# HoangGiang93/mujoco_sim

Hardware: AMD Instinct MI355X
Metric: env-steps/sec (whole node) at 4096 envs, 24-DoF/30-contact scene; 1/2/4/8 GPUs (higher is better)
Workload: dtype f32

## Files before the change

mujoco_sim_amd/csrc/dev_convex.h:

```cpp
#pragma once
#include "dev_math.h"

#define MPR_TOL 1e-6f
#define MPR_ITER 50
#define MPR_EPS_LEN2 1e-10f
#define MPR_EPS_VOL 1e-7f

struct CvxGeom { int type; float pos[3], mat[9], size[3], pad; const float* vert; int nvert; };
struct MprPt { float v[3], s[3]; };

DEV void mpr_tri_normal(float* n, const MprPt& p1, const MprPt& p2, const MprPt& p3) {
  const float e1[3] = {p2.v[0]-p1.v[0], p2.v[1]-p1.v[1], p2.v[2]-p1.v[2]}, e2[3] = {p3.v[0]-p1.v[0], p3.v[1]-p1.v[1], p3.v[2]-p1.v[2]};
  cross3(n, e1, e2); normalize3(n);
}
DEV bool mpr_converged(const MprPt& p1, const MprPt& p2, const MprPt& p3, const MprPt& p4, const float* n) {
  const float d4 = dot3(p4.v, n);
  const float m = fminf(d4 - dot3(p1.v, n), fminf(d4 - dot3(p2.v, n), d4 - dot3(p3.v, n)));
  return m <= MPR_TOL;
}
DEV void mpr_take(MprPt& q, const MprPt& p, bool take) {
#pragma unroll
  for (int k = 0; k < 3; k++) { q.v[k] = take ? p.v[k] : q.v[k]; q.s[k] = take ? p.s[k] : q.s[k]; }
}
DEV void mpr_expand(const MprPt& p0, MprPt& p1, MprPt& p2, MprPt& p3, const MprPt& p4) {
  float c[3];
  cross3(c, p4.v, p0.v);
  const bool a = dot3(p1.v, c) > 0, b = dot3(p2.v, c) > 0, d = dot3(p3.v, c) > 0;
  const bool r1 = a ? b : !d, r2 = !a && d, r3 = a && !b;
  mpr_take(p1, p4, r1); mpr_take(p2, p4, r2); mpr_take(p3, p4, r3);
}
DEV void tri_closest_to_origin(const float* a, const float* b, const float* c, float* out) {
  const float ab[3] = {b[0]-a[0], b[1]-a[1], b[2]-a[2]}, ac[3] = {c[0]-a[0], c[1]-a[1], c[2]-a[2]};
  const float d1 = -dot3(ab, a), d2 = -dot3(ac, a);
  if (d1 <= 0 && d2 <= 0) { out[0] = a[0]; out[1] = a[1]; out[2] = a[2]; return; }
  const float d3 = -dot3(ab, b), d4 = -dot3(ac, b);
  if (d3 >= 0 && d4 <= d3) { out[0] = b[0]; out[1] = b[1]; out[2] = b[2]; return; }
  const float vc = d1*d4 - d3*d2;
  if (vc <= 0 && d1 >= 0 && d3 <= 0) { const float t = d1 / (d1 - d3); out[0] = a[0] + t*ab[0]; out[1] = a[1] + t*ab[1]; out[2] = a[2] + t*ab[2]; return; }
  const float d5 = -dot3(ab, c), d6 = -dot3(ac, c);
  if (d6 >= 0 && d5 <= d6) { out[0] = c[0]; out[1] = c[1]; out[2] = c[2]; return; }
  const float vb = d5*d2 - d1*d6;
  if (vb <= 0 && d2 >= 0 && d6 <= 0) { const float t = d2 / (d2 - d6); out[0] = a[0] + t*ac[0]; out[1] = a[1] + t*ac[1]; out[2] = a[2] + t*ac[2]; return; }
  const float va = d3*d6 - d5*d4;
  if (va <= 0 && (d4 - d3) >= 0 && (d5 - d6) >= 0) {
    const float t = (d4 - d3) / ((d4 - d3) + (d5 - d6));
    out[0] = b[0] + t*(c[0]-b[0]); out[1] = b[1] + t*(c[1]-b[1]); out[2] = b[2] + t*(c[2]-b[2]); return;
  }
  const float den = 1.0f / (va + vb + vc), v = vb * den, w = vc * den;
  out[0] = a[0] + v*ab[0] + w*ac[0]; out[1] = a[1] + v*ab[1] + w*ac[1]; out[2] = a[2] + v*ab[2] + w*ac[2];
}

DEV void cvx_support_local(const CvxGeom& g, const float* dl, float* pl) {
  const float* s = g.size;
  pl[0] = pl[1] = pl[2] = 0;
  if (g.type == MJH_GEOM_SPHERE) { pl[0] = s[0]*dl[0]; pl[1] = s[0]*dl[1]; pl[2] = s[0]*dl[2]; }
  else if (g.type == MJH_GEOM_CAPSULE) { pl[0] = s[0]*dl[0]; pl[1] = s[0]*dl[1]; pl[2] = s[0]*dl[2] + (dl[2] >= 0 ? s[1] : -s[1]); }
  else if (g.type == MJH_GEOM_CYLINDER) {
    const float r2 = dl[0]*dl[0] + dl[1]*dl[1];
    if (r2 > MPR_EPS_LEN2) { const float sc = s[0] * rsqrtf(r2); pl[0] = dl[0]*sc; pl[1] = dl[1]*sc; }
    pl[2] = dl[2] >= 0 ? s[1] : -s[1];
  } else if (g.type == MJH_GEOM_BOX) { pl[0] = dl[0] >= 0 ? s[0] : -s[0]; pl[1] = dl[1] >= 0 ? s[1] : -s[1]; pl[2] = dl[2] >= 0 ? s[2] : -s[2]; }
  else if (g.type == MJH_GEOM_ELLIPSOID) {
    const float w0 = s[0]*s[0]*dl[0], w1 = s[1]*s[1]*dl[1], w2 = s[2]*s[2]*dl[2];
    const float den = sqrtf(w0*dl[0] + w1*dl[1] + w2*dl[2]);
    if (den > MJ_MINVAL) { const float inv = 1.0f / den; pl[0] = w0*inv; pl[1] = w1*inv; pl[2] = w2*inv; }
  }
}
DEV void mesh_support_wave(const bool want, const float* vert, const int nvert, const float* dl, float* pl, const int lane) {
  unsigned long long req = __ballot(want);
  const unsigned long long va = (unsigned long long)vert;
  const int valo = (int)(unsigned)va, vahi = (int)(unsigned)(va >> 32);
  while (req) {
    constexpr int NB = 4;
    int L[NB], nv[NB]; const float* vp[NB]; float d0[NB], d1[NB], d2[NB]; bool on[NB];
#pragma unroll
    for (int u = 0; u < NB; u++) {
      on[u] = req != 0;
      L[u] = on[u] ? __ffsll((long long)req) - 1 : 0;
      if (on[u]) req &= req - 1;
      const unsigned lo = (unsigned)__builtin_amdgcn_readlane(valo, L[u]), hi = (unsigned)__builtin_amdgcn_readlane(vahi, L[u]);
      vp[u] = (const float*)(((unsigned long long)hi << 32) | lo);
      nv[u] = on[u] ? __builtin_amdgcn_readlane(nvert, L[u]) : 0;
      d0[u] = readlane_f(dl[0], L[u]); d1[u] = readlane_f(dl[1], L[u]); d2[u] = readlane_f(dl[2], L[u]);
    }
    float bx[NB], by[NB], bz[NB], bd[NB]; int bi[NB];
#pragma unroll
    for (int u = 0; u < NB; u++) {
      bd[u] = -3.0e38f; bi[u] = 0x7fffffff; bx[u] = by[u] = bz[u] = 0;
      if (on[u]) { const int i = min(lane, nv[u] - 1); bx[u] = vp[u][3*i]; by[u] = vp[u][3*i+1]; bz[u] = vp[u][3*i+2]; }
    }
#pragma unroll
    for (int u = 0; u < NB; u++) {
      if (!on[u]) continue;
      if (lane < nv[u]) { bd[u] = bx[u]*d0[u] + by[u]*d1[u] + bz[u]*d2[u]; bi[u] = lane; }
      for (int i = lane + 64; i < nv[u]; i += 64) {
        const float x = vp[u][3*i], y = vp[u][3*i+1], z = vp[u][3*i+2], dp = x*d0[u] + y*d1[u] + z*d2[u];
        if (dp > bd[u]) { bd[u] = dp; bi[u] = i; bx[u] = x; by[u] = y; bz[u] = z; }
      }
      const float gmax = wave_max_f(bd[u]);
      const bool cand = bd[u] == gmax && bi[u] != 0x7fffffff;
      unsigned long long m = __ballot(cand);
      if (__popcll(m) > 1) { const int wi = wave_min_i(cand ? bi[u] : 0x7fffffff); m = __ballot(cand && bi[u] == wi); }
      const int wl = m ? __ffsll((long long)m) - 1 : 0;
      const float wx = readlane_f(bx[u], wl), wy = readlane_f(by[u], wl), wz = readlane_f(bz[u], wl);
      if (lane == L[u]) { pl[0] = wx; pl[1] = wy; pl[2] = wz; }
    }
  }
}
struct HfPrism { float x[3], y[3], top[3], bot; };
DEV void prism_support_local(const HfPrism& h, const float* dl, float* pl) {
  const bool up = dl[2] >= 0;
  float bd = -3.0e38f;
  pl[0] = h.x[0]; pl[1] = h.y[0]; pl[2] = up ? h.top[0] : h.bot;
#pragma unroll
  for (int i = 0; i < 3; i++) {
    const float z = up ? h.top[i] : h.bot, d = h.x[i]*dl[0] + h.y[i]*dl[1] + z*dl[2];
    const bool take = d > bd;
    bd = take ? d : bd; pl[0] = take ? h.x[i] : pl[0]; pl[1] = take ? h.y[i] : pl[1]; pl[2] = take ? z : pl[2];
  }
}
DEV void mesh_support_lane(const float* vert, const int nvert, const float* dl, float* pl) {
  float bd = -3.0e38f;
  for (int i = 0; i < nvert; i++) {
    const float x = vert[3*i], y = vert[3*i+1], z = vert[3*i+2], dp = x*dl[0] + y*dl[1] + z*dl[2];
    if (dp > bd) { bd = dp; pl[0] = x; pl[1] = y; pl[2] = z; }
  }
}
template <bool PRISM = false>
DEV void mpr_support_wave(const CvxGeom& g1, const CvxGeom& g2, const float* dir, MprPt& p, const bool act, const int lane, const HfPrism* h = nullptr) {
  const float nd[3] = {-dir[0], -dir[1], -dir[2]};
  float dl1[3], dl2[3], pl1[3], pl2[3], a[3], b[3];
  rotvecT(dl1, g1.mat, dir); rotvecT(dl2, g2.mat, nd);
  if constexpr (PRISM) prism_support_local(*h, dl1, pl1); else cvx_support_local(g1, dl1, pl1);
  cvx_support_local(g2, dl2, pl2);
  if constexpr (!PRISM) mesh_support_wave(act && g1.type == MJH_GEOM_MESH, g1.vert, g1.nvert, dl1, pl1, lane);
  if constexpr (PRISM) { if (g2.type == MJH_GEOM_MESH) mesh_support_lane(g2.vert, g2.nvert, dl2, pl2); }
  else mesh_support_wave(act && g2.type == MJH_GEOM_MESH, g2.vert, g2.nvert, dl2, pl2, lane);
  rotvec(a, g1.mat, pl1); rotvec(b, g2.mat, pl2);
#pragma unroll
  for (int k = 0; k < 3; k++) {
    a[k] += g1.pos[k] + g1.pad*dir[k]; b[k] += g2.pos[k] + g2.pad*nd[k];
    p.v[k] = a[k] - b[k]; p.s[k] = a[k] + b[k];
  }
}

template <bool PRISM = false>
DEV int c_convex_wave(CvxGeom& g1, CvxGeom& g2, float margin, float* st, const bool act, const int lane, const HfPrism* h = nullptr) {
  g1.pad = g2.pad = 0.5f * margin;
  MprPt p0, p1, p2, p3, p4;
  float n[3], c[3];
#pragma unroll
  for (int k = 0; k < 3; k++) { p0.v[k] = g1.pos[k] - g2.pos[k]; p0.s[k] = g1.pos[k] + g2.pos[k]; p1.v[k] = p2.v[k] = p3.v[k] = 0; p1.s[k] = p2.s[k] = p3.s[k] = 0; }
  if (dot3(p0.v, p0.v) < MPR_EPS_LEN2) p0.v[0] += 1e-4f;
  n[0] = -p0.v[0]; n[1] = -p0.v[1]; n[2] = -p0.v[2];
  normalize3(n);
  enum { PH_FIRST, PH_SECOND, PH_DISCOVER, PH_REFINE, PH_PUSH };
  int phase = PH_FIRST, it = 0;
  bool live = act;
  int res = 0;
  while (__ballot(live) != 0) {
    mpr_support_wave<PRISM>(g1, g2, n, p4, live, lane, h);
    if (live) {
    const float d4 = dot3(p4.v, n);
    if (phase == PH_FIRST) {
      if (d4 <= 0) live = false;
      else {
      p1 = p4;
      cross3(n, p0.v, p1.v);
      if (dot3(n, n) < 1e-12f * dot3(p0.v, p0.v) * dot3(p1.v, p1.v)) {
        const float depth = norm3(p1.v);
        float dir[3] = {p1.v[0], p1.v[1], p1.v[2]}; normalize3(dir);
        const float pos[3] = {0.5f * p1.s[0], 0.5f * p1.s[1], 0.5f * p1.s[2]};
        raw_emit(st, 0, margin - depth, pos, dir);
        res = 1; live = false;
      } else {
      normalize3(n);
      phase = PH_SECOND;
      } }
    } else if (phase == PH_SECOND) {
      if (d4 <= 0) live = false;
      else {
      p2 = p4;
      const float e1[3] = {p1.v[0]-p0.v[0], p1.v[1]-p0.v[1], p1.v[2]-p0.v[2]}, e2[3] = {p2.v[0]-p0.v[0], p2.v[1]-p0.v[1], p2.v[2]-p0.v[2]};
      cross3(n, e1, e2); normalize3(n);
      const bool sw = dot3(n, p0.v) > 0;
      const MprPt t = p1;
      mpr_take(p1, p2, sw); mpr_take(p2, t, sw);
      n[0] = sw ? -n[0] : n[0]; n[1] = sw ? -n[1] : n[1]; n[2] = sw ? -n[2] : n[2];
      phase = PH_DISCOVER; it = 0;
      }
    } else if (phase == PH_DISCOVER) {
      if (d4 <= 0 || it > MPR_ITER) live = false;
      else {
      it++;
      cross3(c, p1.v, p4.v);
      const bool t2 = dot3(c, p0.v) < -MPR_EPS_VOL;
      cross3(c, p4.v, p2.v);
      const bool t1 = !t2 && dot3(c, p0.v) < -MPR_EPS_VOL;
      if (t1 || t2) {
        mpr_take(p2, p4, t2); mpr_take(p1, p4, t1);
        const float e1[3] = {p1.v[0]-p0.v[0], p1.v[1]-p0.v[1], p1.v[2]-p0.v[2]}, e2[3] = {p2.v[0]-p0.v[0], p2.v[1]-p0.v[1], p2.v[2]-p0.v[2]};
        cross3(n, e1, e2); normalize3(n);
      } else {
        p3 = p4;
        mpr_tri_normal(n, p1, p2, p3);
        phase = dot3(n, p1.v) >= -MPR_EPS_VOL ? PH_PUSH : PH_REFINE; it = 0;
      }
      }
    } else if (phase == PH_REFINE) {
      if (d4 < -MPR_EPS_VOL || mpr_converged(p1, p2, p3, p4, n) || it > MPR_ITER) live = false;
      else {
      it++;
      mpr_expand(p0, p1, p2, p3, p4);
      mpr_tri_normal(n, p1, p2, p3);
      if (dot3(n, p1.v) >= -MPR_EPS_VOL) { phase = PH_PUSH; it = 0; }
      }
    } else {
      if (mpr_converged(p1, p2, p3, p4, n) || it > MPR_ITER) { res = 2; live = false; }
      else {
      it++;
      mpr_expand(p0, p1, p2, p3, p4);
      mpr_tri_normal(n, p1, p2, p3);
      }
    }
    }
  }
  if (res != 2) return res;
  float depth, dir[3], pos[3];
  tri_closest_to_origin(p1.v, p2.v, p3.v, c);
  depth = norm3(c);
  if (depth < 1e-7f) { dir[0] = n[0]; dir[1] = n[1]; dir[2] = n[2]; } else { const float inv = 1.0f / depth; dir[0] = c[0]*inv; dir[1] = c[1]*inv; dir[2] = c[2]*inv; }
  float b0, b1, b2, b3, x[3];
  cross3(x, p1.v, p2.v); b0 = dot3(x, p3.v);
  cross3(x, p3.v, p2.v); b1 = dot3(x, p0.v);
  cross3(x, p0.v, p1.v); b2 = dot3(x, p3.v);
  cross3(x, p2.v, p1.v); b3 = dot3(x, p0.v);
  float sum = b0 + b1 + b2 + b3;
  if (sum <= 0) {
    b0 = 0;
    cross3(x, p2.v, p3.v); b1 = dot3(x, n);
    cross3(x, p3.v, p1.v); b2 = dot3(x, n);
    cross3(x, p1.v, p2.v); b3 = dot3(x, n);
    sum = b1 + b2 + b3;
  }
// ... 14 lines not shown
```

mujoco_sim_amd/csrc/dev_math.h:

```cpp
#pragma once
#include <hip/hip_runtime.h>

#define DEV __device__ __forceinline__
#define HDEV __host__ __device__ __forceinline__
#if !defined(__HIP_DEVICE_COMPILE__)
static inline float rsqrtf(float x) { return 1.0f / sqrtf(x); }
#endif
#define MJ_MINVAL 1e-15f
#define MJ_MAXVAL 1e10f

HDEV float dot3(const float* a, const float* b) { return a[0]*b[0] + a[1]*b[1] + a[2]*b[2]; }
HDEV void cross3(float* r, const float* a, const float* b) {
  float x = a[1]*b[2] - a[2]*b[1], y = a[2]*b[0] - a[0]*b[2], z = a[0]*b[1] - a[1]*b[0];
  r[0] = x; r[1] = y; r[2] = z;
}
HDEV float norm3(const float* a) { return sqrtf(dot3(a, a)); }
DEV float normalize3(float* a) {
  float n = norm3(a);
  if (n < MJ_MINVAL) { a[0] = 1; a[1] = 0; a[2] = 0; } else { float s = 1.0f / n; a[0] *= s; a[1] *= s; a[2] *= s; }
  return n;
}
DEV void normalize4(float* q) {
  const float n2 = q[0]*q[0] + q[1]*q[1] + q[2]*q[2] + q[3]*q[3];
  if (fabsf(n2 - 1.0f) <= 4.8e-7f) return;
  const float n = sqrtf(n2);
  if (n < MJ_MINVAL) { q[0] = 1; q[1] = q[2] = q[3] = 0; } else { float s = 1.0f / n; q[0] *= s; q[1] *= s; q[2] *= s; q[3] *= s; }
}
DEV void mulquat(float* r, const float* a, const float* b) {
  float w = a[0]*b[0] - a[1]*b[1] - a[2]*b[2] - a[3]*b[3];
  float x = a[0]*b[1] + a[1]*b[0] + a[2]*b[3] - a[3]*b[2];
  float y = a[0]*b[2] - a[1]*b[3] + a[2]*b[0] + a[3]*b[1];
  float z = a[0]*b[3] + a[1]*b[2] - a[2]*b[1] + a[3]*b[0];
  r[0] = w; r[1] = x; r[2] = y; r[3] = z;
}
DEV void quat2mat(float* m, const float* q) {
  float w = q[0], x = q[1], y = q[2], z = q[3];
  m[0] = w*w + x*x - y*y - z*z; m[1] = 2*(x*y - w*z);         m[2] = 2*(x*z + w*y);
  m[3] = 2*(x*y + w*z);         m[4] = w*w - x*x + y*y - z*z; m[5] = 2*(y*z - w*x);
  m[6] = 2*(x*z - w*y);         m[7] = 2*(y*z + w*x);         m[8] = w*w - x*x - y*y + z*z;
}
HDEV void rotvec(float* r, const float* m, const float* v) {
  float x = m[0]*v[0] + m[1]*v[1] + m[2]*v[2], y = m[3]*v[0] + m[4]*v[1] + m[5]*v[2], z = m[6]*v[0] + m[7]*v[1] + m[8]*v[2];
  r[0] = x; r[1] = y; r[2] = z;
}
HDEV void rotvecT(float* r, const float* m, const float* v) {
  float x = m[0]*v[0] + m[3]*v[1] + m[6]*v[2], y = m[1]*v[0] + m[4]*v[1] + m[7]*v[2], z = m[2]*v[0] + m[5]*v[1] + m[8]*v[2];
  r[0] = x; r[1] = y; r[2] = z;
}
DEV void axisangle2quat(float* q, const float* axis, float angle) {
  float s, c; __sincosf(0.5f * angle, &s, &c);
  q[0] = c; q[1] = axis[0]*s; q[2] = axis[1]*s; q[3] = axis[2]*s;
}
DEV void quat_integrate(float* q, const float* w, float h) {
  float ax[3] = {w[0], w[1], w[2]};
  float n = norm3(ax);
  if (n < MJ_MINVAL) { normalize4(q); return; }
  float inv = 1.0f / n; ax[0] *= inv; ax[1] *= inv; ax[2] *= inv;
  float dq[4], r[4];
  float s = sinf(0.5f * h * n), c = cosf(0.5f * h * n);
  dq[0] = c; dq[1] = ax[0]*s; dq[2] = ax[1]*s; dq[3] = ax[2]*s;
  normalize4(q); mulquat(r, q, dq); normalize4(r);
  q[0] = r[0]; q[1] = r[1]; q[2] = r[2]; q[3] = r[3];
}
DEV void cross_motion(float* r, const float* v, const float* x) {
  float a[3], b[3], c[3];
  cross3(a, v, x); cross3(b, v, x + 3); cross3(c, v + 3, x);
  r[0] = a[0]; r[1] = a[1]; r[2] = a[2]; r[3] = b[0] + c[0]; r[4] = b[1] + c[1]; r[5] = b[2] + c[2];
}
DEV void cross_force(float* r, const float* v, const float* f) {
  float a[3], b[3], c[3];
  cross3(a, v, f); cross3(b, v + 3, f + 3); cross3(c, v, f + 3);
  r[0] = a[0] + b[0]; r[1] = a[1] + b[1]; r[2] = a[2] + b[2]; r[3] = c[0]; r[4] = c[1]; r[5] = c[2];
}
DEV void inert_com(float* res, const float* diagI, const float* mat, const float* off, float mass) {
  float I[9];
#pragma unroll
  for (int r = 0; r < 3; r++)
#pragma unroll
    for (int c = 0; c < 3; c++) I[3*r+c] = mat[3*r]*diagI[0]*mat[3*c] + mat[3*r+1]*diagI[1]*mat[3*c+1] + mat[3*r+2]*diagI[2]*mat[3*c+2];
  float d2 = dot3(off, off);
  res[0] = I[0] + mass * (d2 - off[0]*off[0]); res[1] = I[4] + mass * (d2 - off[1]*off[1]); res[2] = I[8] + mass * (d2 - off[2]*off[2]);
  res[3] = I[1] - mass * off[0]*off[1]; res[4] = I[2] - mass * off[0]*off[2]; res[5] = I[5] - mass * off[1]*off[2];
  res[6] = mass * off[0]; res[7] = mass * off[1]; res[8] = mass * off[2]; res[9] = mass;
}
DEV void mul_inert_vec(float* res, const float* i, const float* v) {
  float r0 = i[0]*v[0] + i[3]*v[1] + i[4]*v[2] - i[8]*v[4] + i[7]*v[5];
// ... 104 lines not shown
```

mujoco_sim_amd/csrc/dev_types.h:

```cpp
#pragma once

#define MJH_INT_TABLES(X)                                                                          \
  X(body_parentid) X(body_rootid) X(body_jntadr) X(body_jntnum) X(body_dofadr) X(body_dofnum)      \
  X(body_level) X(body_subtreesize) X(body_treeid) X(body_lastdof) X(jnt_type) X(jnt_qposadr)      \
  X(jnt_dofadr) X(jnt_bodyid) X(jnt_limited) X(dof_bodyid) X(dof_jntid) X(dof_parentid)            \
  X(dof_Madr) X(dof_treeid) X(tree_dofadr) X(tree_dofnum) X(geom_type) X(geom_bodyid)              \
  X(geom_condim) X(pair_geom1) X(pair_geom2) X(pair_stageadr) X(eq_obj1id) X(eq_obj2id)            \
  X(eq_active) X(fl_dof) X(gc_body) X(controlled) X(odom)

#define MJH_FLT_TABLES(X)                                                                          \
  X(body_pos) X(body_quat) X(body_ipos) X(body_iquat) X(body_mass) X(body_inertia)                 \
  X(body_gravcomp) X(body_invweight0) X(jnt_pos) X(jnt_axis) X(jnt_stiffness) X(jnt_range)         \
  X(jnt_margin) X(jnt_solref) X(jnt_solimp) X(qpos0) X(qpos_spring) X(dof_armature)                \
  X(dof_damping) X(dof_frictionloss) X(dof_invweight0) X(dof_solref) X(dof_solimp) X(geom_pos)     \
  X(geom_quat) X(geom_size) X(geom_rbound) X(geom_friction) X(geom_solmix) X(geom_solref)          \
  X(geom_solimp) X(geom_margin) X(geom_gap) X(eq_data) X(eq_solref) X(eq_solimp)

struct DModel {
  const int* I;
  const float* F;
#define X(n) int o_##n;
  MJH_INT_TABLES(X)
  MJH_FLT_TABLES(X)
#undef X
  int nq, nv, nbody, njnt, ngeom, neq, npair, nM, ntree, maxcon, maxefc;
  int nqp, nvp;
  int maxlevel, nfl, ngc, rowW, nstage, has_damping, has_limits, diagM, maxblk, maxbrow, has_dim4, big, k1_floats, has_convex;
  int iterations, disableflags;
  float timestep, gravity[3], tolerance, impratio, meaninertia;
  int o_geom_dataid, o_mesh_vertadr, o_mesh_vertnum, o_mesh_vert;
  int noslip_iterations; float noslip_tolerance;
  double timestep_d;
  int nsite, nsensor, nmocap, has_weld;
  int group_max;
  int scratch_off;
  int o_site_bodyid, o_site_pos, o_site_quat, o_sensor_type, o_sensor_objid, o_body_mocapid, o_eq_type;
  int patch, pool, pool_floats, pdesc, pslot;
  int window, win_nvt, win_maxw, win_jsz;
  int pgs_row_order;
  int dense, dense_cap, dense_nvs;
  int dense_min_iter;
};

#ifdef MJH_COLLIDE_PROBE
#define PROF_STRIDE 24
#else
#define PROF_STRIDE 20
#endif
struct DState {
  float *qpos, *qvel, *qacc, *qacc_ws, *qvel_ref, *qfrc_applied, *ddq, *dq, *qfrc_inverse;
  double* time;
  float *initial_qpos, *odom_vel;
  int* stats;
  const int* env_order;
  unsigned* slot_mask;
  float *x_xpos, *x_xquat, *x_gpos, *x_gmat;
  float *x_bias, *x_passive, *x_smooth, *x_constraint, *x_energy;
  float *x_contacts;
  float *x_vec, *x_res;
  long long* x_prof;
  const float *p_geom_size, *p_geom_rbound, *p_body_mass, *p_body_inertia, *p_body_invweight0, *p_dof_invweight0;
  int p_stride;
  float *xfrc_applied, *mocap, *sensordata; int xfrc_stride;
  const float* pd_target; float pd_kp, pd_kd;
  float* gscratch; long long gstride;
  int win32;
  int win64;
  int probe_slices;
  float* wbuf; long long wstride; long long wj_off;
};

#define MJH_LDS_SMALL(X)                                                                           \
  X(qpos) X(qvel) X(qvref) X(ws) X(qacc) X(smooth) X(asmooth) X(passive) X(bias) X(applied)        \
  X(tmpv) X(tmpv2) X(xpos) X(xquat) X(xmat) X(xipos) X(ximat) X(com) X(cinert) X(crb) X(cvel)      \
  X(cacc) X(cfrc) X(cfrcsub) X(xanchor) X(xaxis) X(cdof) X(cdofdot) X(qM) X(qLD) X(qLDinv)          \
  X(gpos) X(gmat) X(zero) X(dofpar) X(dofMadr) X(anc) X(p_gsize) X(p_rbound) X(p_mass) X(p_inertia) X(site) X(fext)
#define MJH_LDS_POOLS(X) X(con) X(blki) X(blkf) X(blkq) X(bv) X(phi) X(sched) X(order) X(J) X(B) X(ext)
#define MJH_LDS_ARRAYS(X) MJH_LDS_SMALL(X) MJH_LDS_POOLS(X)

struct Lay {
#define X(n) int n;
  MJH_LDS_ARRAYS(X)
#undef X
  int total;
  int g_a0, g_minv, g_qvel, g_smooth, g_qacc, g_meta, g_qM;
  int g_qLD, g_anc;
  int g_dense;
};

struct DHField { int has_hfield, o_hfield_nrow, o_hfield_ncol, o_hfield_adr, o_hfield_size, o_hfield_data; };

struct DWpre { int slim, J; };

#define CREP_STRIDE 20
#define CREP_FORCE 13
#define CREP_GEOM1 17
#define CREP_GEOM2 18
#define CREP_DIM 19
struct DReport { int on, maxcon; int* ncon; float* rec; float* cfrc; };

struct DConst { DModel M; Lay L; DHField H; DWpre W; DReport R; };

enum { PH_STEP1 = 1, PH_INV = 2, PH_STEP2 = 4, PH_NOINT = 8, PH_FKONLY = 16, PH_MULM = 32, PH_RESET = 64,
       PH_PRE = 128, PH_POST = 256 };
enum { XF_BODY = 1, XF_GEOM = 2, XF_CON = 4, XF_FORCE = 8, XF_PROF = 16,
       XF_NOSTORE = 32,
       XF_DENSE = 64,
       XF_SPLIT2 = 256,
       XF_WSTRAIGHT = 512,
       XF_DEFER = 128 };

#define CON_STRIDE 16
#define CON_GEOMS 13
#define CON_MARGIN 14
#define CON_G1(c) (__float_as_int((c)[CON_GEOMS]) & 0xfff)
#define CON_G2(c) ((__float_as_int((c)[CON_GEOMS]) >> 12) & 0xfff)
#define CON_DIM(c) (__float_as_int((c)[CON_GEOMS]) >> 24)
#define BLKI_STRIDE 4
#define BLKF_STRIDE 16
#define BLKQ_STRIDE 16
#define BF_AREF 4
#define BF_F 8
#define BF_LO 14
enum { BK_SINGLE = 0, BK_PYR3 = 3, BK_PYR4 = 4 };
enum { RT_EQ = 0, RT_FL = 1, RT_LIMIT = 2, RT_CONTACT = 3, RT_WELD = 4 };
```

mujoco_sim_amd/csrc/engine.hip:

```cpp
#include <hip/hip_runtime.h>

#include <algorithm>
#include <cmath>
#include <cstddef>
#include <cstdio>
#include <cstdlib>
#include <cstring>
#include <string>
#include <vector>

#include "../../include/mjhip.h"
#include "step_kernel.h"
#include "dev_ray.h"
#include "dev_depth.h"
#include "dev_scan.h"
#include "dev_heightscan.h"
#include "dev_contact.h"
#include "dev_frame.h"
#include "dev_render.h"
#include "dev_light.h"
#include "dev_texture.h"
#include "ray_tables.h"

void mjh_set_error(const std::string& s);
hipError_t mjh_launch_window(hipStream_t st, int nvt, int grid, size_t lds, const DConst* dC, const DState& S, int env0, int n, int nl, int wxf, int n32, int n64);
hipError_t mjh_dense_attributes(size_t build_lds, size_t solve_lds);
hipError_t mjh_launch_step_hf(hipStream_t st, int nr, bool diag, int wpre, int grid, size_t lds, const DConst* dC, const DState& S,
                              int env0, int nsteps, int ph, int xflags);
hipError_t mjh_step_hf_attributes(size_t lds);
hipError_t mjh_launch_dense(hipStream_t st, int n, size_t build_lds, size_t solve_lds, const DConst* dC, const DState& S, int env0);
#define DN_CAP_MAX 256

#define HIPCHK(call)                                                                             \
  do {                                                                                           \
    hipError_t e_ = (call);                                                                      \
    if (e_ != hipSuccess) {                                                                      \
      mjh_set_error(std::string(#call) + ": " + hipGetErrorString(e_));                          \
      return MJH_ERR_NO_DEVICE;                                                                  \
    }                                                                                            \
  } while (0)

struct StateGuard {
  DState* where; DState saved;
  explicit StateGuard(DState* w) : where(w), saved(*w) {}
  ~StateGuard() { *where = saved; }
  StateGuard(const StateGuard&) = delete; StateGuard& operator=(const StateGuard&) = delete;
};
struct DevBuf {
  void* p = nullptr;
  ~DevBuf() { if (p) (void)hipFree(p); }
};

#define MJH_MAX_COHORTS 8
#define MJH_IO_SLOTS 8
#define MJH_IO_PUT_FLOATS 4096
#define MJH_IO_GET_FLOATS 16384
__attribute__((constructor)) static void mjh_library_init() { setenv("GPU_MAX_HW_QUEUES", "8", 0); }
struct mjh_engine {
  const mjh_model* model = nullptr;
  int nenv = 0, device = 0;
  hipStream_t stream = nullptr;
  DModel M{};
  DState S{};
  Lay L{};
  int lds_bytes = 0, lds_bytes_pre = 0;
  DHField H{};
  bool report = false; DReport R{};
  int2* csel_tab = nullptr; int2* csel_host = nullptr; int csel_cap = 0; hipEvent_t csel_up = nullptr; std::vector<int> csel_have; float* csel_io = nullptr; size_t csel_io_words = 0;
  DWpre W{};
  size_t dense_lds = 0, dense_solve_lds = 0;
  float* h_io = nullptr; float* d_io = nullptr; hipEvent_t io_ev[MJH_IO_SLOTS] = {}; bool io_used[MJH_IO_SLOTS] = {}; unsigned io_next = 0;
  int win_lean = -1;
  bool win_straight = true;
  int* h_wn = nullptr; int* d_wn = nullptr; int cur_cohort = -1;
  int* h_dense = nullptr; int* d_dense = nullptr; hipEvent_t ev_dense[MJH_MAX_COHORTS][4] = {}; unsigned dense_epoch[MJH_MAX_COHORTS] = {}; bool dense_now[MJH_MAX_COHORTS];
  int* dI = nullptr; float* dF = nullptr; DConst* dC = nullptr;
  std::vector<int> hI;
  int o_controlled = 0, o_odom = 0;
  std::vector<void*> allocs;
  float* scratch = nullptr; size_t scratch_floats = 0;
  float* p_tables[MJH_EP_COUNT] = {nullptr};
  int* d_order = nullptr;
  bool lpt = true;
  bool split3 = true;
  bool order_valid = false;
  struct ChainGraph { hipGraphExec_t exec = nullptr; unsigned char S[sizeof(DState)]; int g0 = -1, n = -1, key = -1; bool nocap = false; };
  int last_launches = 0;
  ChainGraph cgraph[MJH_MAX_COHORTS][8];
  int steps_per_launch = 8;
  long order_age = 0; int order_G = 0; int last_chunk = 1;
  int ncohort = 1;
  hipStream_t cstream[MJH_MAX_COHORTS] = {nullptr};
  hipEvent_t ev_fork = nullptr, ev_join[MJH_MAX_COHORTS] = {nullptr};
  bool forked = false;
  bool timing = false; int timing_stride = 1; long timing_count = 0;
  std::vector<std::pair<hipEvent_t, hipEvent_t>> tev; size_t tev_used = 0;
  bool step1_done = false;
  bool handover = false;
  bool step1_pending = false;
  float pd_kp = 0, pd_kd = 0; float* pd_target = nullptr; bool pd_on = false;
  int4* ray_ginfo = nullptr; RayHField* ray_hf = nullptr; float* ray_hfdata = nullptr; bool ray_ready = false;
  int ray_mesh_mode = 0; int4* ray_ginfo_mesh = nullptr; RayMesh* ray_mesh = nullptr; float4* ray_planes = nullptr;
  int ray_mesh_surface = 0; bool ray_tri_ready = false; std::vector<int4> ray_gi_mesh_host;
  int4* ray_ginfo_tri = nullptr; RayTriMesh* ray_trimesh = nullptr; RayNode* ray_nodes = nullptr; float4* ray_tris = nullptr;
  float* ray_io = nullptr; size_t ray_io_floats = 0;
  float4* ray_color = nullptr; float* render_io = nullptr; size_t render_io_floats = 0;
  int light_mode = 0; mjh_light_options light_opt = {1, 1, 1e-3f};
  bool lights_ready = false; int nlight = 0; LightRec lights[MJH_MAXLIGHT]; int light_on[MJH_MAXLIGHT];
  int tex_mode = 0; TexRec* tex_rec = nullptr; unsigned* tex_data = nullptr; float* tex_io = nullptr; size_t tex_io_floats = 0;
  float* scan_tab = nullptr; size_t scan_tab_floats = 0; float* scan_host = nullptr; size_t scan_host_floats = 0; hipEvent_t scan_up = nullptr;
  bool scan_have = false; int scan_w = 0, scan_h = 0; double scan_az[2] = {0, 0}, scan_el[2] = {0, 0}; bool scan_table = false; std::vector<double> scan_elev;
  int* hscan_root = nullptr;
  bool frame_ready = false; FrameModel frame_model{};
  FrameRec* frame_tab = nullptr; FrameRec* frame_host = nullptr; int frame_cap = 0; hipEvent_t frame_up = nullptr; std::vector<int> frame_have;
  float* frame_io = nullptr; size_t frame_io_floats = 0;
};

static int pad32(int n) { return ((n + 31) / 32) * 32; }

template <class T> static int dev_alloc(mjh_engine* e, T** p, size_t n, bool zero = true) {
  void* q = nullptr;
  HIPCHK(hipMalloc(&q, std::max<size_t>(n, 1) * sizeof(T)));
  if (zero) HIPCHK(hipMemsetAsync(q, 0, std::max<size_t>(n, 1) * sizeof(T), e->stream));
  e->allocs.push_back(q);
  *p = (T*)q;
  return MJH_OK;
}

static int g_chain_graph = getenv("MJH_CHAIN_GRAPH") ? atoi(getenv("MJH_CHAIN_GRAPH")) : 1;
extern "C" void mjh_set_chain_graph(int mode) { g_chain_graph = mode < 0 ? 0 : (mode > 2 ? 2 : mode); }

static int ensure_scratch(mjh_engine* e, size_t floats) {
  if (floats <= e->scratch_floats) return MJH_OK;
  if (e->scratch) { HIPCHK(hipStreamSynchronize(e->stream)); HIPCHK(hipFree(e->scratch)); }
  HIPCHK(hipMalloc((void**)&e->scratch, floats * sizeof(float)));
  e->scratch_floats = floats;
  return MJH_OK;
}

static bool extra_instance(const DModel& M) { return M.has_convex || M.noslip_iterations > 0 || M.nsensor > 0 || M.nmocap > 0 || M.has_weld; }

static int window_tier(const mjh_engine* e) {
  static const int nl_env = getenv("MJH_WN_NL") ? atoi(getenv("MJH_WN_NL")) : -1;
  const int nwreg = e->M.win_nvt == 24 ? WN_NW24 : WN_NW32;
  const int seen = (e->h_wn && e->cur_cohort >= 0) ? *(volatile int*)(e->h_wn + e->cur_cohort) : (1 << 20);
  const int nl_full = std::min(WN_MAXW, (int)((40 * 1024 - 1024) / (4 * WN_XREC(e->M.win_nvt) * 16 * sizeof(float))));
  const bool sec32 = e->S.win32 > 0 && e->M.win_nvt == 24 && e->S.win32 <= 16 * nwreg;
  const bool tier = sec32 ? seen > 32 * WN32_NW : seen + 16 > 16 * nwreg;
  if (nl_env < 0 && e->win_lean >= 0 && e->M.win_maxw <= 16) return e->win_lean ? 0 : nl_full;
// ... 5 lines not shown
  const bool window = snap || (e->M.window && e->S.wbuf && (ph & PH_STEP2) && !(ph & (PH_NOINT | PH_PRE | PH_POST)) && !(xflags & ~(XF_FORCE | XF_DEFER | (wmode == 1 ? XF_PROF : 0))));
  if (window && !snap) ph |= PH_PRE;
  if (wmode && !window) { mjh_set_error("internal: window-chain launch mode on a launch that is not one"); return MJH_ERR_STATE; }
  if (wmode == 1) xflags |= XF_DEFER;
  if (wmode != 2) {
#define MJH_LAUNCH2(NR, DG, CX) do { if (e->H.has_hfield) HIPCHK(mjh_launch_step_hf(st, NR, DG, 0, n, (size_t)e->lds_bytes, e->dC, e->S, env0, nsteps, ph, xflags)); \
                                   else hipLaunchKernelGGL((mjh_step_kernel<NR, DG, CX>), dim3(n), dim3(64), (size_t)e->lds_bytes, st, e->dC, e->S, env0, nsteps, ph, xflags); } while (0)
#define MJH_LAUNCH(NR, DG) do { if (extra_instance(e->M) || e->S.xfrc_applied || e->report) MJH_LAUNCH2(NR, DG, true); else MJH_LAUNCH2(NR, DG, false); } while (0)
  const int nr = e->M.big ? 8 : (e->M.nv <= 16 ? 1 : (e->M.nv <= 32 ? 2 : 4));
  static const bool slim = !(getenv("MJH_WINDOW_SLIM") && atoi(getenv("MJH_WINDOW_SLIM")) == 0);
  if (window && slim) {
    const bool cx = extra_instance(e->M) || e->S.xfrc_applied || e->report;
    static const bool slim_lds = !(getenv("MJH_WINDOW_SLIM_LDS") && atoi(getenv("MJH_WINDOW_SLIM_LDS")) == 0);
    static const int wpad = getenv("MJH_WPRE_LDS_PAD") ? std::max(0, atoi(getenv("MJH_WPRE_LDS_PAD"))) : 0;
    const size_t wlds = (size_t)((slim_lds && e->lds_bytes_pre > 0) ? e->lds_bytes_pre : e->lds_bytes) + (size_t)wpad;
#define MJH_LAUNCHW(NR, CX, GJ) do { if (e->H.has_hfield) HIPCHK(mjh_launch_step_hf(st, NR, true, GJ, n, wlds, e->dC, e->S, env0, nsteps, ph, xflags)); \
                                   else hipLaunchKernelGGL((mjh_step_kernel<NR, true, CX, GJ>), dim3(n), dim3(64), wlds, st, e->dC, e->S, env0, nsteps, ph, xflags); } while (0)
#define MJH_LAUNCHW2(NR, CX) do { if (e->M.patch) MJH_LAUNCHW(NR, CX, 1); else MJH_LAUNCHW(NR, CX, 2); } while (0)
    if (nr == 1) { if (cx) MJH_LAUNCHW2(1, true); else MJH_LAUNCHW2(1, false); } else { if (cx) MJH_LAUNCHW2(2, true); else MJH_LAUNCHW2(2, false); }
#undef MJH_LAUNCHW2
#undef MJH_LAUNCHW
  } else
  if (e->M.diagM) { if (nr == 1) MJH_LAUNCH(1, true); else if (nr == 2) MJH_LAUNCH(2, true); else if (nr == 4) MJH_LAUNCH(4, true); else MJH_LAUNCH(8, true); }
  else { if (nr == 1) MJH_LAUNCH(1, false); else if (nr == 2) MJH_LAUNCH(2, false); else if (nr == 4) MJH_LAUNCH(4, false); else MJH_LAUNCH(8, false); }
#undef MJH_LAUNCH2
#undef MJH_LAUNCH
  HIPCHK(hipGetLastError());
  }
  if (window && wmode != 1 && wmode != 3) {
    const int nl = tier_nl >= 0 ? tier_nl : window_tier(e);
    const size_t lds = (size_t)4 * nl * WN_XREC(e->M.win_nvt) * 16 * sizeof(float);
    const int n32 = (e->S.win32 && e->M.win_nvt == 24) ? (n + 1) / 2 : 0;
    const int wxf = (xflags & ~XF_DEFER) | ((ph & PH_STEP1) ? 0 : XF_SPLIT2) | (e->win_straight ? XF_WSTRAIGHT : 0);
    const int n64 = (e->S.win64 && e->M.win_nvt == 24 && e->S.win64 < 16 * e->M.win_maxw) ? n : 0;
    HIPCHK(mjh_launch_window(st, e->M.win_nvt, n64 + (e->M.win_nvt == 24 ? n32 : 0) + (n + 3) / 4, lds, e->dC, e->S, env0, n, nl, wxf, n32, n64));
  }
  return MJH_OK;
}

static int launch(mjh_engine* e, int env0, int n, int nsteps, int ph, int xflags, int wmode = 0) { return launch_on(e, e->stream, env0, n, nsteps, ph, xflags, wmode); }

static int fork_cohorts(mjh_engine* e) {
  if (e->forked || e->ncohort <= 1) return MJH_OK;
  HIPCHK(hipEventRecord(e->ev_fork, e->stream));
  for (int g = 0; g < e->ncohort; g++) HIPCHK(hipStreamWaitEvent(e->cstream[g], e->ev_fork, 0));
  e->forked = true;
  return MJH_OK;
}
static int join_cohorts(mjh_engine* e) {
  if (!e->forked) return MJH_OK;
  for (int g = 0; g < e->ncohort; g++) {
    HIPCHK(hipEventRecord(e->ev_join[g], e->cstream[g]));
    HIPCHK(hipStreamWaitEvent(e->stream, e->ev_join[g], 0));
  }
  e->forked = false;
  return MJH_OK;
}
static int set_cohorts(mjh_engine* e, int n) {
  n = std::max(1, std::min(n, MJH_MAX_COHORTS));
  int rc = join_cohorts(e);
  if (rc) return rc;
  if (n > 1) {
    if (!e->ev_fork) HIPCHK(hipEventCreateWithFlags(&e->ev_fork, hipEventDisableTiming));
    for (int g = 0; g < n; g++) {
      if (!e->cstream[g]) HIPCHK(hipStreamCreateWithFlags(&e->cstream[g], hipStreamNonBlocking));
      if (!e->ev_join[g]) HIPCHK(hipEventCreateWithFlags(&e->ev_join[g], hipEventDisableTiming));
    }
  }
  e->ncohort = n;
  return MJH_OK;
}

static int pair_cap(int t1, int t2) {
  if (t1 > t2) std::swap(t1, t2);
  if (t1 == MJH_GEOM_PLANE && t2 == MJH_GEOM_BOX) return 4;
  if (t1 == MJH_GEOM_PLANE && t2 == MJH_GEOM_CAPSULE) return 2;
  if (t1 == MJH_GEOM_PLANE && t2 == MJH_GEOM_CYLINDER) return 4;
  if (t1 == MJH_GEOM_PLANE && t2 == MJH_GEOM_MESH) return 4;
  if (t1 == MJH_GEOM_BOX && t2 == MJH_GEOM_BOX) return 8;
  if (t1 == MJH_GEOM_HFIELD) return MJH_HFIELD_MAXCON;
  return 1;
}

struct HostPack { DModel M{}; Lay L{}; DHField H{}; DWpre W{}; bool report = false; std::vector<int> I; std::vector<float> F; int o_controlled = 0, o_odom = 0, lds_bytes = 0, lds_bytes_pre = 0, lds_bytes_wpre = 0; long long gstride = 0; };
#define MJH_WINDOW_MAXCON 128
static int g_window_solver = getenv("MJH_WINDOW") ? (atoi(getenv("MJH_WINDOW")) != 0) : 1;
extern "C" void mjh_set_window_solver(int on) { g_window_solver = on ? 1 : 0; }
static int g_pgs_row_order = 1;
static int g_contact_report = getenv("MJH_CONTACT_REPORT") ? (atoi(getenv("MJH_CONTACT_REPORT")) != 0) : 0;
extern "C" void mjh_set_contact_report(int on) { g_contact_report = on ? 1 : 0; }
extern "C" void mjh_set_pgs_row_order(int mode) { g_pgs_row_order = mode < 0 || mode > 2 ? 1 : mode; }
static void derive_device_model(const mjh_model* m, HostPack& hp, bool force_big = false, bool allow_patch = true) {
  DModel& M = hp.M; std::vector<int>& I = hp.I; std::vector<float>& F = hp.F;
  const bool report = g_contact_report != 0;
  hp.report = report;
  const int nb = m->nbody, nv = m->nv, nj = m->njnt, ng = m->ngeom;
  std::vector<int> subtreesize(nb, 1), lastdof(nb, -1), stageadr(m->npair, 0), fl_dof, gc_body, controlled(std::max(nv, 1), 0), odom(10, -1);
  odom[9] = 0;
  for (int b = nb - 1; b > 0; b--) subtreesize[m->body_parentid[b]] += subtreesize[b];
  for (int b = 1; b < nb; b++) lastdof[b] = m->body_dofnum[b] ? m->body_dofadr[b] + m->body_dofnum[b] - 1 : lastdof[m->body_parentid[b]];
  int nstage = 0, maxlevel = 0, rowW = 1;
  for (int b = 0; b < nb; b++) maxlevel = std::max(maxlevel, m->body_level[b]);
  auto treenum = [&](int b) { int t = m->body_treeid[b]; return t >= 0 ? m->tree_dofnum[t] : 0; };
  for (int i = 0; i < m->npair; i++) {
    int g1 = m->pair_geom1[i], g2 = m->pair_geom2[i];
    stageadr[i] = nstage; nstage += pair_cap(m->geom_type[g1], m->geom_type[g2]);
    int b1 = m->geom_bodyid[g1], b2 = m->geom_bodyid[g2];
    int w = treenum(b1) + ((m->body_treeid[b1] != m->body_treeid[b2]) ? treenum(b2) : 0);
    rowW = std::max(rowW, w);
  }
  for (int t = 0; t < m->ntree; t++) rowW = std::max(rowW, m->tree_dofnum[t]);
  int neqrow = 0; bool has_weld = false;
  for (int q = 0; q < m->neq; q++) {
    if (m->eq_type[q] != MJH_EQ_JOINT) {
      has_weld = true; neqrow += m->eq_type[q] == MJH_EQ_WELD ? 6 : 3;
      rowW = std::max(rowW, treenum(m->eq_obj1id[q]) + ((m->body_treeid[m->eq_obj1id[q]] != m->body_treeid[m->eq_obj2id[q]]) ? treenum(m->eq_obj2id[q]) : 0));
      continue;
    }
    neqrow++;
    int j1 = m->eq_obj1id[q], j2 = m->eq_obj2id[q];
    int t1 = m->dof_treeid[m->jnt_dofadr[j1]], w = m->tree_dofnum[t1];
    if (j2 >= 0) { int t2 = m->dof_treeid[m->jnt_dofadr[j2]]; if (t2 != t1) w += m->tree_dofnum[t2]; }
    rowW = std::max(rowW, w);
  }
  rowW = ((rowW + 3) / 4) * 4;
  bool diagM = m->ntree > 0 && m->neq == 0 && m->nsensor == 0 && m->nmocap == 0 && !report;
  for (int t = 0; t < m->ntree && diagM; t++) {
    const int b = m->tree_bodyid[t];
    diagM = m->tree_dofnum[t] == 6 && m->body_jntnum[b] == 1 && m->jnt_type[m->body_jntadr[b]] == MJH_JNT_FREE && subtreesize[b] == 1 &&
            m->body_ipos[3*b] == 0 && m->body_ipos[3*b+1] == 0 && m->body_ipos[3*b+2] == 0 && m->body_iquat[4*b] == 1;
  }
  bool has_damping = false, has_limits = false;
  for (int d = 0; d < nv; d++) { if (m->dof_frictionloss[d] > 0) { fl_dof.push_back(d); diagM = false; } if (m->dof_damping[d] > 0) has_damping = true; }
  for (int j = 0; j < nj; j++) if (m->jnt_limited[j]) has_limits = true;
  for (int b = 1; b < nb; b++) if (m->body_gravcomp[b] != 0) gc_body.push_back(b);

  auto addI = [&](const int* p, size_t n) { int o = (int)I.size(); I.insert(I.end(), p, p + n); while (I.size() % 4) I.push_back(0); return o; };
  auto addF = [&](const double* p, size_t n) { int o = (int)F.size(); for (size_t i = 0; i < n; i++) F.push_back((float)p[i]); while (F.size() % 4) F.push_back(0); return o; };
#define PI(name, n) M.o_##name = addI(m->name, (size_t)(n))
#define PF(name, n) M.o_##name = addF(m->name, (size_t)(n))
  PI(body_parentid, nb); PI(body_rootid, nb); PI(body_jntadr, nb); PI(body_jntnum, nb); PI(body_dofadr, nb); PI(body_dofnum, nb);
  PI(body_level, nb); M.o_body_subtreesize = addI(subtreesize.data(), nb); PI(body_treeid, nb); M.o_body_lastdof = addI(lastdof.data(), nb);
  PI(jnt_type, nj); PI(jnt_qposadr, nj); PI(jnt_dofadr, nj); PI(jnt_bodyid, nj); PI(jnt_limited, nj);
  PI(dof_bodyid, nv); PI(dof_jntid, nv); PI(dof_parentid, nv); PI(dof_Madr, nv); PI(dof_treeid, nv);
  PI(tree_dofadr, m->ntree); PI(tree_dofnum, m->ntree);
  PI(geom_type, ng); PI(geom_bodyid, ng); PI(geom_condim, ng);
  PI(pair_geom1, m->npair); PI(pair_geom2, m->npair); M.o_pair_stageadr = addI(stageadr.data(), m->npair);
  PI(eq_obj1id, m->neq); PI(eq_obj2id, m->neq); PI(eq_active, m->neq);
  M.o_fl_dof = addI(fl_dof.data(), fl_dof.size()); M.o_gc_body = addI(gc_body.data(), gc_body.size());
  M.o_controlled = hp.o_controlled = addI(controlled.data(), controlled.size());
  M.o_odom = hp.o_odom = addI(odom.data(), odom.size());
  PF(body_pos, 3*nb); PF(body_quat, 4*nb); PF(body_ipos, 3*nb); PF(body_iquat, 4*nb); PF(body_mass, nb); PF(body_inertia, 3*nb);
  PF(body_gravcomp, nb); PF(body_invweight0, 2*nb);
  PF(jnt_pos, 3*nj); PF(jnt_axis, 3*nj); PF(jnt_stiffness, nj); PF(jnt_range, 2*nj); PF(jnt_margin, nj); PF(jnt_solref, 2*nj); PF(jnt_solimp, 5*nj);
  PF(qpos0, m->nq); PF(qpos_spring, m->nq);
  PF(dof_armature, nv); PF(dof_damping, nv); PF(dof_frictionloss, nv); PF(dof_invweight0, nv); PF(dof_solref, 2*nv); PF(dof_solimp, 5*nv);
  PF(geom_pos, 3*ng); PF(geom_quat, 4*ng); PF(geom_size, 3*ng); PF(geom_rbound, ng); PF(geom_friction, 3*ng); PF(geom_solmix, ng);
  PF(geom_solref, 2*ng); PF(geom_solimp, 5*ng); PF(geom_margin, ng); PF(geom_gap, ng);
  PF(eq_data, 11*m->neq); PF(eq_solref, 2*m->neq); PF(eq_solimp, 5*m->neq);
  PI(geom_dataid, ng); PI(mesh_vertadr, m->nmesh); PI(mesh_vertnum, m->nmesh); PF(mesh_vert, 3 * (size_t)m->nmeshvert);
  PI(eq_type, m->neq);
  if (m->nsite > 0) { PI(site_bodyid, m->nsite); PF(site_pos, 3 * (size_t)m->nsite); PF(site_quat, 4 * (size_t)m->nsite); }
  if (m->nsensor > 0) { PI(sensor_type, m->nsensor); PI(sensor_objid, m->nsensor); }
  {
    std::vector<int> mocapid(nb, -1);
    if (m->body_mocapid) for (int b = 0; b < nb; b++) mocapid[b] = m->body_mocapid[b];
    M.o_body_mocapid = addI(mocapid.data(), nb);
  }
  M.nsite = m->nsite; M.nsensor = m->nsensor; M.nmocap = m->nmocap; M.has_weld = has_weld ? 1 : 0;
  {
    DHField& H = hp.H;
    H.has_hfield = 0;
    for (int i = 0; i < m->npair; i++) if (m->geom_type[m->pair_geom1[i]] == MJH_GEOM_HFIELD) H.has_hfield = 1;
    if (H.has_hfield) {
      H.o_hfield_nrow = addI(m->hfield_nrow, m->nhfield); H.o_hfield_ncol = addI(m->hfield_ncol, m->nhfield); H.o_hfield_adr = addI(m->hfield_adr, m->nhfield);
      H.o_hfield_size = addF(m->hfield_size, 4 * (size_t)m->nhfield); H.o_hfield_data = addF(m->hfield_data, (size_t)m->nhfielddata);
    }
  }
  M.group_max = m->ntree <= 64 ? 16 : 4;
  for (int t = 0; t < m->ntree; t++) if (m->tree_dofnum[t] > 8) M.group_max = 4;
#undef PI
#undef PF
  M.nq = m->nq; M.nv = nv; M.nbody = nb; M.njnt = nj; M.ngeom = ng; M.neq = m->neq; M.npair = m->npair; M.nM = m->nM; M.ntree = m->ntree;
  M.maxcon = std::max(m->maxcon, 1); M.maxefc = std::max(m->maxefc, 1);
  M.nqp = M.nvp = pad32(m->nq + 4 * std::max(nv, 1));
  M.maxlevel = maxlevel; M.nfl = (int)fl_dof.size(); M.ngc = (int)gc_body.size(); M.rowW = rowW; M.nstage = nstage;
  M.has_damping = has_damping; M.has_limits = has_limits; M.diagM = diagM;
  M.has_dim4 = 0;
  for (int g = 0; g < ng; g++) if (m->geom_condim[g] == 4) M.has_dim4 = 1;
  M.has_convex = 0;
  for (int i = 0; i < m->npair; i++) {
    const int t1 = m->geom_type[m->pair_geom1[i]], t2 = m->geom_type[m->pair_geom2[i]];
    if (t2 == MJH_GEOM_MESH) M.has_convex = 1;
    if (t1 != MJH_GEOM_PLANE && (t1 == MJH_GEOM_ELLIPSOID || t2 == MJH_GEOM_ELLIPSOID || t1 == MJH_GEOM_CYLINDER || t2 == MJH_GEOM_CYLINDER ||
                                 t2 == MJH_GEOM_MESH || (t1 == MJH_GEOM_CAPSULE && t2 == MJH_GEOM_BOX))) M.has_convex = 1;
  }
  {
    int nlim = 0; for (int j = 0; j < nj; j++) if (m->jnt_limited[j]) nlim += (m->jnt_range[2*j+1] - m->jnt_range[2*j] <= 2 * m->jnt_margin[j]) ? 2 : 1;
    const int nfix = neqrow + (int)fl_dof.size() + nlim;
    M.maxblk = nfix + M.maxcon; M.maxbrow = nfix + 4 * M.maxcon;
  }
  M.iterations = m->opt.iterations; M.disableflags = m->opt.disableflags;
  M.timestep = (float)m->opt.timestep; M.timestep_d = m->opt.timestep; for (int k = 0; k < 3; k++) M.gravity[k] = (float)m->opt.gravity[k];
  M.tolerance = (float)m->opt.tolerance; M.impratio = (float)m->opt.impratio; M.meaninertia = (float)m->meaninertia;
  M.noslip_iterations = m->opt.noslip_iterations; M.noslip_tolerance = (float)m->opt.noslip_tolerance;
  {
    Lay& L = hp.L; int off = 0; long long goff = 0;
    auto put = [&](int n) { int o = off; off += ((std::max(n, 1) + 3) / 4) * 4; return o; };
    const bool big = force_big || nv > 64;
    M.big = big;
    const bool keep = m->nsensor > 0 || report;
    auto gput = [&](long long n) { long long o = goff; goff += ((std::max<long long>(n, 1) + 3) / 4) * 4; return (int)(-1 - o); };
    const int nblkcap = std::max(M.maxblk, 1);
    long long jsz = std::max<long long>((long long)(M.maxblk - M.maxcon) * rowW + (long long)M.maxcon * rowW * 4, 4);
    const long long need = (long long)nstage * RAW_STRIDE;
    if ((diagM ? 1 : 2) * jsz < need) jsz = diagM ? need : (need + 1) / 2;
    M.pgs_row_order = g_pgs_row_order;
    if (!M.pgs_row_order && nv > 32) for (int t = 0; t < m->ntree; t++) if (m->tree_dofnum[t] > 16) M.pgs_row_order = 1;
    const bool small_free = allow_patch && diagM && !big && nv <= 32 && M.noslip_iterations == 0 && !keep;
    const bool patch = small_free && M.maxcon <= 64;
    M.patch = patch ? 1 : 0;
    M.window = (small_free && M.maxcon <= MJH_WINDOW_MAXCON && M.pgs_row_order != 0 && g_window_solver && nv <= 32 && m->njnt <= 16 && m->nq <= 40) ? 1 : 0;
    M.win_nvt = nv <= 24 ? 24 : 32;
    M.win_maxw = std::max(1, std::min(WN_MAXW, (M.maxefc + 15) / 16));
    if (const char* v = getenv("MJH_WINDOW_MAXW")) M.win_maxw = std::max(1, std::min(M.win_maxw, atoi(v)));
    L.qpos = put(m->nq);
    L.qvel = put(nv); L.qvref = put(nv); L.ws = put(nv); L.qacc = put(nv); L.smooth = put(nv); L.asmooth = put(nv); L.passive = put(nv);
    L.bias = put(nv); L.applied = put(nv); L.tmpv = put(nv); L.tmpv2 = put(nv);
    if (patch) {
      L.qM = put(m->nM); L.qLD = L.qM; L.qLDinv = put(nv); L.dofpar = 0; L.dofMadr = 0; L.anc = 0;
      L.p_gsize = put(3*ng); L.p_rbound = put(ng); L.p_mass = put(nb); L.p_inertia = put(3*nb);
      L.zero = put(PP_ZERO);
    }
    const int k1 = off;
    const int unused = diagM ? put(4) : 0;
    L.xpos = put(3*nb); L.xquat = put(4*nb); L.xmat = put(9*nb); L.ximat = put(9*nb); L.crb = diagM ? unused : put(10*nb);
    L.xanchor = put(3*nj); L.xaxis = put(3*nj); L.gpos = put(3*ng); L.gmat = put(9*ng);
    const int k1_size = off - k1;
    M.k1_floats = k1_size;
    M.scratch_off = (big && keep) ? put(k1_size) : k1;
    L.xipos = put(3*nb); L.com = put(3*nb); L.cinert = diagM ? unused : put(10*nb); L.cdof = diagM ? unused : put(6*nv);
    const int k2_size = off - k1;
    if (!patch) {
      L.qM = put(m->nM); L.qLD = (diagM || big) ? L.qM : put(m->nM); L.qLDinv = put(nv);
      if (diagM) { L.dofpar = 0; L.dofMadr = 0; L.anc = 0; }
      else { L.dofpar = put(nv); L.dofMadr = put(nv); L.anc = put(m->nM); }
      const bool nopairs = m->npair == 0;
      L.p_gsize = nopairs ? L.gpos : put(3*ng); L.p_rbound = nopairs ? L.gmat : put(ng); L.p_mass = put(nb); L.p_inertia = put(3*nb);
    }
    {
      const int a4 = [](int n) { return ((std::max(n, 1) + 3) / 4) * 4; }(6*nb);
      const int velsz = diagM ? 4 : 4 * a4 + ((6*nv + 3) / 4) * 4;
      int vel;
      if (big) { L.con = gput((long long)M.maxcon * CON_STRIDE); L.blkq = gput((long long)nblkcap * BLKQ_STRIDE); vel = (!keep && !diagM && velsz <= k1_size) ? k1 : put(velsz); }
      else if (keep) { L.con = put(M.maxcon * CON_STRIDE); L.blkq = put(nblkcap * BLKQ_STRIDE); vel = put(velsz); }
      else {
        L.con = put(std::max(std::max(M.maxcon * CON_STRIDE, velsz), nblkcap * BLKQ_STRIDE));
        L.blkq = L.con; vel = L.con;
      }
      if (diagM) { L.cvel = unused; L.cacc = unused; L.cfrc = unused; L.cfrcsub = unused; L.cdofdot = unused; }
      else { L.cvel = vel; L.cacc = vel + a4; L.cfrc = vel + 2*a4; L.cfrcsub = vel + 3*a4; L.cdofdot = vel + 4*a4; }
// ... 42 lines not shown
      L.g_a0 = graw(nv); L.g_minv = graw(nv); L.g_qvel = graw(nv); L.g_smooth = graw(nv); L.g_qacc = graw(nv); L.g_meta = graw(8); L.g_qM = graw(m->nM);
      const bool dense_on = !(getenv("MJH_DENSE") && atoi(getenv("MJH_DENSE")) == 0);
      M.dense = (dense_on && !diagM && M.noslip_iterations == 0 && nv <= 128 && nv >= 1) ? 1 : 0;
      M.dense_cap = std::min(256, ((std::max(M.maxefc, 1) + 63) / 64) * 64); M.dense_nvs = ((nv + 15) / 16) * 16;
      if (const char* dc = getenv("MJH_DENSE_CAP")) M.dense_cap = std::max(64, std::min(M.dense_cap, (atoi(dc) / 64) * 64));
      M.dense_min_iter = getenv("MJH_DENSE_MIN_ITER") ? std::max(0, atoi(getenv("MJH_DENSE_MIN_ITER"))) : 32;
      L.g_dense = 0; L.g_qLD = 0; L.g_anc = 0;
      if (M.dense) { L.g_qLD = graw(m->nM); L.g_anc = graw(m->nM); }
      if (M.dense) { long long o = goff; goff += (long long)M.dense_cap * M.dense_cap + (long long)M.dense_cap * M.dense_nvs + 6LL * M.dense_cap; L.g_dense = (int)o; }
    }
    hp.gstride = goff;
    if (const char* pad = getenv("MJH_LDS_PAD")) off += std::max(0, atoi(pad));
    L.total = off;
    hp.lds_bytes = off * (int)sizeof(float);
  }
}

#define MJH_LDS_RESIDENT_MAX (24 * 1024)
#define MJH_ORDER_EVERY 32
static int order_every_of(const mjh_engine* e);
static int g_layout_policy = 0;
extern "C" void mjh_set_layout_policy(int policy) { g_layout_policy = policy < 0 || policy > 2 ? 0 : policy; }
static int order_every_of(const mjh_engine* e) {
  static const int env = getenv("MJH_ORDER_EVERY") ? std::max(1, atoi(getenv("MJH_ORDER_EVERY"))) : 0;
  return env ? env : ((e->M.window && e->M.win_maxw > 16) ? 16 : MJH_ORDER_EVERY);
}
static void derive_fitting(const mjh_model* m, HostPack& hp) {
  derive_device_model(m, hp);
  int policy = g_layout_policy;
  if (const char* fb = getenv("MJH_FORCE_BIG")) policy = atoi(fb) ? 2 : 1;
  const int limit = policy == 1 ? 160 * 1024 : (policy == 2 ? 0 : MJH_LDS_RESIDENT_MAX);
  if ((hp.M.patch || hp.M.window) && policy == 0 && hp.lds_bytes <= 64 * 1024) return;
  if (hp.M.patch && hp.lds_bytes > 64 * 1024 && hp.lds_bytes <= limit) { HostPack np; derive_device_model(m, np, false, false); hp = np; }
  if ((hp.lds_bytes > 160 * 1024 || hp.lds_bytes > limit) && !hp.M.big && hp.M.rowW <= 64) { HostPack big; derive_device_model(m, big, true); hp = big; }
}

extern "C" int mjh_query_lds_bytes(const mjh_model* m) {
  if (!m) return MJH_ERR_ARG;
  HostPack hp; derive_fitting(m, hp);
  return hp.lds_bytes;
}
extern "C" int mjh_debug_lds_layout(const mjh_model* m, char* out, int cap) {
  if (!m || !out || cap <= 0) return MJH_ERR_ARG;
  HostPack hp; derive_fitting(m, hp);
  std::string t;
#define X(n) t += std::string(#n) + " " + std::to_string(hp.L.n) + "\n";
  MJH_LDS_ARRAYS(X)
#undef X
  t += "total " + std::to_string(hp.L.total) + "\nlds_bytes " + std::to_string(hp.lds_bytes) + "\nlds_bytes_pre " + std::to_string(hp.lds_bytes_pre) +
       "\nk1_floats " + std::to_string(hp.M.k1_floats) + "\nmaxcon " + std::to_string(hp.M.maxcon) + "\nmaxblk " + std::to_string(hp.M.maxblk) +
       "\nrowW " + std::to_string(hp.M.rowW) + "\nnstage " + std::to_string(hp.M.nstage) + "\nbig " + std::to_string((int)hp.M.big) +
       "\nlds_bytes_wpre " + std::to_string(hp.M.window ? hp.lds_bytes_wpre : 0) + "\n";
  const int n = std::min((int)t.size(), cap - 1);
  std::memcpy(out, t.data(), (size_t)n); out[n] = 0;
  return n;
}
extern "C" int mjh_query_lds_bytes_assemble(const mjh_model* m) {
  if (!m) return MJH_ERR_ARG;
  HostPack hp; derive_fitting(m, hp);
  return hp.M.window ? hp.lds_bytes_pre : 0;
}

extern "C" int mjh_create(const mjh_model* m, int nenv, int device, void* stream, mjh_engine** out) {
  if (!m || nenv <= 0 || !out) { mjh_set_error("mjh_create: bad argument"); return MJH_ERR_ARG; }
  int ndev = 0;
  if (hipGetDeviceCount(&ndev) != hipSuccess || ndev <= 0) {
    mjh_set_error("mjh_create: no HIP device visible (this engine has no CPU fallback)");
    return MJH_ERR_NO_DEVICE;
  }
  if (device < 0 || device >= ndev) { mjh_set_error("mjh_create: bad device index"); return MJH_ERR_ARG; }

  if (m->ngeom > 4095) { mjh_set_error("mjh_create: more than 4095 geoms (contact records pack the geom ids in 12 bits)"); return MJH_ERR_CAPACITY; }
  for (int g = 0; g < m->ngeom; g++) if (m->geom_condim[g] != 1 && m->geom_condim[g] != 3 && m->geom_condim[g] != 4) {
    mjh_set_error("mjh_create: condim must be 1, 3 or 4 (rolling friction, condim 6, is not implemented)"); return MJH_ERR_UNSUPPORTED; }
  HIPCHK(hipSetDevice(device));
  mjh_engine* e = new mjh_engine();
#undef HIPCHK
#define HIPCHK(call) do { hipError_t e_ = (call); if (e_ != hipSuccess) { mjh_set_error(std::string(#call) + ": " + hipGetErrorString(e_)); mjh_destroy(e); return MJH_ERR_NO_DEVICE; } } while (0)
  if (const char* v = getenv("MJH_LPT")) e->lpt = atoi(v) != 0;
  if (const char* v = getenv("MJH_SPLIT3")) e->split3 = atoi(v) != 0;
  e->model = m; e->nenv = nenv; e->device = device; e->stream = (hipStream_t)stream;

  HostPack hp; derive_fitting(m, hp);
  e->M = hp.M; e->L = hp.L; e->H = hp.H; e->W = hp.W; e->report = hp.report; e->lds_bytes = hp.lds_bytes; e->lds_bytes_pre = hp.lds_bytes_wpre; e->o_controlled = hp.o_controlled; e->o_odom = hp.o_odom;
  DModel& M = e->M; std::vector<int>& I = hp.I; std::vector<float>& F = hp.F;
  e->hI = I;
  if (dev_alloc(e, &e->dI, I.size(), false) || dev_alloc(e, &e->dF, F.size(), false)) { mjh_destroy(e); return MJH_ERR_NO_DEVICE; }
  HIPCHK(hipMemcpyAsync(e->dI, I.data(), I.size() * sizeof(int), hipMemcpyHostToDevice, e->stream));
  HIPCHK(hipMemcpyAsync(e->dF, F.data(), F.size() * sizeof(float), hipMemcpyHostToDevice, e->stream));
  HIPCHK(hipStreamSynchronize(e->stream));
  M.I = e->dI; M.F = e->dF;

  if (e->report) {
    DReport& R = e->R;
    R.on = 1; R.maxcon = e->M.maxcon; e->split3 = false;
    if (dev_alloc(e, &R.ncon, (size_t)nenv) || dev_alloc(e, &R.rec, (size_t)nenv * R.maxcon * CREP_STRIDE) || dev_alloc(e, &R.cfrc, (size_t)nenv * 6 * e->M.nbody)) { mjh_destroy(e); return MJH_ERR_NO_DEVICE; }
  }
  {
    DConst hc; hc.M = e->M; hc.L = e->L; hc.H = e->H; hc.W = e->W; hc.R = e->R;
    if (dev_alloc(e, &e->dC, 1, false)) { mjh_destroy(e); return MJH_ERR_NO_DEVICE; }
    HIPCHK(hipMemcpyAsync(e->dC, &hc, sizeof hc, hipMemcpyHostToDevice, e->stream));
    HIPCHK(hipStreamSynchronize(e->stream));
  }
  if ((long long)(e->M.maxblk - e->M.maxcon) * e->M.rowW + (long long)e->M.maxcon * e->M.rowW * 4 >= 4LL * 65536) {
    mjh_set_error("mjh_create: Jacobian pool too large for the 16-bit block offsets (lower the contact capacity)");
    mjh_destroy(e); return MJH_ERR_CAPACITY;
  }
  if (e->M.big && e->M.rowW > 64) {
    mjh_set_error("mjh_create: nv > 64 needs every constraint to touch at most 64 dofs (this model: " + std::to_string(e->M.rowW) + "); the solver maps one dof of a block per lane");
    mjh_destroy(e); return MJH_ERR_CAPACITY;
  }
  if (e->lds_bytes > 160 * 1024) {
    mjh_set_error("mjh_create: per-env working set exceeds the 160 KiB LDS of one CU (" + std::to_string(e->lds_bytes) + " B)");
    mjh_destroy(e); return MJH_ERR_CAPACITY;
  }
#define MJH_ATTR(NR, DG) do { HIPCHK(hipFuncSetAttribute((const void*)mjh_step_kernel<NR, DG, false>, hipFuncAttributeMaxDynamicSharedMemorySize, e->lds_bytes)); \
                              HIPCHK(hipFuncSetAttribute((const void*)mjh_step_kernel<NR, DG, true>, hipFuncAttributeMaxDynamicSharedMemorySize, e->lds_bytes)); } while (0)
  if (e->M.dense) {
    e->dense_lds = ((size_t)e->M.dense_nvs + 5 * (size_t)e->M.dense_cap + (size_t)std::max(e->M.maxblk, 1) + 8) * sizeof(float);
    e->dense_solve_lds = (DN_CAP_MAX + 128 + 2 * (size_t)e->M.nM) * sizeof(float);
    if (e->dense_lds > 160 * 1024 || e->dense_solve_lds > 160 * 1024) { e->M.dense = 0; }
    else {
      HIPCHK(mjh_dense_attributes(e->dense_lds, e->dense_solve_lds));
    }
  }
  MJH_ATTR(1, true); MJH_ATTR(2, true); MJH_ATTR(4, true); MJH_ATTR(8, true); MJH_ATTR(1, false); MJH_ATTR(2, false); MJH_ATTR(4, false); MJH_ATTR(8, false);
#undef MJH_ATTR
  if (e->H.has_hfield) HIPCHK(mjh_step_hf_attributes((size_t)e->lds_bytes));
  if (e->M.window) {
#define MJH_ATTRW(NR, CX, GJ) HIPCHK(hipFuncSetAttribute((const void*)mjh_step_kernel<NR, true, CX, GJ>, hipFuncAttributeMaxDynamicSharedMemorySize, e->lds_bytes))
    MJH_ATTRW(1, false, 1); MJH_ATTRW(1, true, 1); MJH_ATTRW(2, false, 1); MJH_ATTRW(2, true, 1);
    MJH_ATTRW(1, false, 2); MJH_ATTRW(1, true, 2); MJH_ATTRW(2, false, 2); MJH_ATTRW(2, true, 2);
#undef MJH_ATTRW
  }

  DState& S = e->S;
  const size_t nq_all = (size_t)nenv * M.nqp, nv_all = (size_t)nenv * M.nvp;
  int rc = 0;
  rc |= dev_alloc(e, &S.qpos, nq_all); rc |= dev_alloc(e, &S.initial_qpos, nq_all);
  {
    const int nvc = std::max(M.nv, 1);
    S.qvel = S.qpos + M.nq; S.qacc_ws = S.qvel + nvc; S.ddq = S.qacc_ws + nvc; S.dq = S.ddq + nvc;
  }
  S.qacc = S.qacc_ws;
  rc |= dev_alloc(e, &S.qvel_ref, nv_all); rc |= dev_alloc(e, &S.qfrc_applied, nv_all);
  rc |= dev_alloc(e, &S.qfrc_inverse, nv_all);
  S.gscratch = nullptr; S.gstride = hp.gstride;
  if (M.big) rc |= dev_alloc(e, &S.gscratch, (size_t)nenv * (size_t)hp.gstride, false);
  S.wbuf = nullptr; S.wstride = 0;
  S.win32 = getenv("MJH_WINDOW32") ? std::max(0, atoi(getenv("MJH_WINDOW32"))) : (M.win_maxw > 16 ? 0 : WN32_MIN_ROWS);
  S.win64 = getenv("MJH_WINDOW64") ? std::max(0, atoi(getenv("MJH_WINDOW64"))) : (M.win_maxw > 16 ? WN64_MIN_ROWS : WN32_MIN_ROWS);
  if (S.win64 > 0 && S.win64 < S.win32) S.win64 = S.win32;
  if (getenv("MJH_WN_NL") && atoi(getenv("MJH_WN_NL")) < 3) S.win64 = 0;
  if (M.window) {
    S.wj_off = ((WN_ROWS + M.win_maxw * WN_NK * 16 + M.win_maxw * WN_XREC(M.win_nvt) * 16 + (M.win_maxw / 2 + 1) * WN_XPAIR * 16 + 63) / 64) * 64;
    S.wstride = S.wj_off + ((M.win_jsz + 63) / 64) * 64;
    if (((S.wstride / 64) & 1) == 0) S.wstride += 64;
    rc |= dev_alloc(e, &S.wbuf, (size_t)nenv * (size_t)S.wstride, true);
  }
  if (const char* v = getenv("MJH_WINDOW_LEAN")) e->win_lean = atoi(v) != 0;
  if (const char* v = getenv("MJH_WINDOW_STRAIGHT")) e->win_straight = atoi(v) != 0;
  if (M.window && e->lpt && nenv >= 1024) {
    HIPCHK(hipHostMalloc((void**)&e->h_wn, MJH_MAX_COHORTS * sizeof(int), hipHostMallocMapped));
    for (int g = 0; g < MJH_MAX_COHORTS; g++) e->h_wn[g] = 1 << 20;
    HIPCHK(hipHostGetDevicePointer((void**)&e->d_wn, e->h_wn, 0));
  }
  if (M.big && M.dense && e->lpt && nenv >= 1024) {
    HIPCHK(hipHostMalloc((void**)&e->h_dense, MJH_MAX_COHORTS * 4 * sizeof(int), hipHostMallocMapped));
    for (int g = 0; g < MJH_MAX_COHORTS * 4; g++) e->h_dense[g] = 1;
    for (int g = 0; g < MJH_MAX_COHORTS; g++) e->dense_now[g] = true;
    HIPCHK(hipHostGetDevicePointer((void**)&e->d_dense, e->h_dense, 0));
    for (int g = 0; g < MJH_MAX_COHORTS; g++) for (int k = 0; k < 4; k++) HIPCHK(hipEventCreateWithFlags(&e->ev_dense[g][k], hipEventDisableTiming));
  }
  rc |= dev_alloc(e, &S.time, (size_t)nenv); rc |= dev_alloc(e, &S.odom_vel, (size_t)nenv * 6); rc |= dev_alloc(e, &S.stats, (size_t)nenv * 4);
  rc |= dev_alloc(e, &S.x_bias, nv_all); rc |= dev_alloc(e, &S.x_passive, nv_all); rc |= dev_alloc(e, &S.x_smooth, nv_all);
  rc |= dev_alloc(e, &S.x_constraint, nv_all); rc |= dev_alloc(e, &S.x_energy, (size_t)nenv * 2);
  if (M.nsensor > 0) { rc |= dev_alloc(e, &S.sensordata, (size_t)nenv * 3 * M.nsensor); e->split3 = false; }
  if (M.nmocap > 0) rc |= dev_alloc(e, &S.mocap, (size_t)nenv * 7 * M.nmocap, false);
  if (rc) { mjh_destroy(e); return MJH_ERR_NO_DEVICE; }
  if (M.nmocap > 0) {
    std::vector<float> mp((size_t)nenv * 7 * M.nmocap);
    for (int b = 0; b < m->nbody; b++) if (m->body_mocapid && m->body_mocapid[b] >= 0)
// ... 1857 lines not shown
```

mujoco_sim_amd/csrc/step_kernel.h:

```cpp
#pragma once
#include "dev_collide.h"
#include "dev_convex.h"
#include "dev_types.h"

#define WSYNC() __syncthreads()
#define PROF(k) do { if ((xflags & XF_PROF) && lane == 0) S.x_prof[(size_t)blockIdx.x * PROF_STRIDE + (k)] = (long long)__builtin_amdgcn_s_memtime(); \
                     if (((xflags >> 8) & 15) == (k) && (k) > 0) return; } while (0)
#ifdef MJH_ASM_PROBE
#define ASM_PROBE_BEGIN() const long long asm_probe_t0 = (long long)__builtin_amdgcn_s_memrealtime()
#define ASM_PROBE_STORE() do { if (WPRE != 0 && lane == 0) { \
    const int hw = (int)__builtin_amdgcn_s_getreg(63492), xcc = (int)__builtin_amdgcn_s_getreg(63508) & 7; \
    const long long dt = (long long)__builtin_amdgcn_s_memrealtime() - asm_probe_t0; \
    S.stats[4*env] = (int)(asm_probe_t0 & 0x7fffffff); \
    S.stats[4*env+2] = ((hw >> 4) & 3) | (((hw >> 8) & 0xff) << 2) | (xcc << 10) | ((int)(dt < 0 ? 0 : (dt > 0x3ffff ? 0x3ffff : dt)) << 13); } } while (0)
#else
#define ASM_PROBE_BEGIN() do {} while (0)
#define ASM_PROBE_STORE() do {} while (0)
#endif
#ifdef MJH_COLLIDE_PROBE
#define CPROF(k) do { if ((xflags & XF_PROF) && lane == 0) S.x_prof[(size_t)blockIdx.x * PROF_STRIDE + 20 + (k)] = (long long)__builtin_amdgcn_s_memtime(); } while (0)
#else
#define CPROF(k) do {} while (0)
#endif
#define MINIMP 0.0001f
#define MAXIMP 0.9999f

DEV float get_impedance(const float* si, float pos, float margin) {
  float s0 = fminf(MAXIMP, fmaxf(MINIMP, si[0])), s1 = fminf(MAXIMP, fmaxf(MINIMP, si[1]));
  float s2 = fmaxf(0.0f, si[2]), s3 = fminf(MAXIMP, fmaxf(MINIMP, si[3])), s4 = fmaxf(1.0f, si[4]);
  if (s0 == s1 || s2 <= MJ_MINVAL) return 0.5f * (s0 + s1);
  float x = fabsf((pos - margin) / s2);
  if (x >= 1) return s1;
  if (x <= 0) return s0;
  float y;
  if (s4 == 1) y = x;
  else if (x <= s3) y = powf(x, s4) / powf(s3, s4 - 1);
  else y = 1 - powf(1 - x, s4) / powf(1 - s3, s4 - 1);
  return s0 + y * (s1 - s0);
}

template <class T> struct Tab {
  const T* base; int off;
  DEV T operator[](int i) const { return base[off + i]; }
  DEV const T* operator+(int k) const { return base + off + k; }
};
template <bool LAZY, class T, int DModel::*OFF> struct XTab {
  const DModel* m; const T* base; int off;
  DEV explicit XTab(const DModel& M) : m(&M), base(nullptr), off(0) { if constexpr (!LAZY) { base = tb(); off = M.*OFF; } }
  DEV const T* tb() const { if constexpr (T(1.5) == T(1)) return (const T*)m->I; else return (const T*)m->F; }
#ifdef MJH_TAB_PROBE_L2
  DEV T operator[](int i) const { if constexpr (LAZY) return *(volatile const T*)(tb() + (m->*OFF + i)); else return base[off + i]; }
#else
  DEV T operator[](int i) const { if constexpr (LAZY) return tb()[m->*OFF + i]; else return base[off + i]; }
#endif
  DEV const T* operator+(int k) const { if constexpr (LAZY) return tb() + (m->*OFF + k); else return base + off + k; }
};

template <bool LAZY, int Lay::*OFF> struct XArr {
  float* p; const Lay* l; float* b;
  DEV XArr(float* lds, const Lay& L) : p(nullptr), l(&L), b(lds) { if constexpr (!LAZY) p = lds + L.*OFF; }
  DEV float* get() const { if constexpr (LAZY) return b + l->*OFF; else return p; }
  DEV operator float*() const { return get(); }
  template <class U> DEV explicit operator U*() const { return (U*)get(); }
};

DEV void solve_tree(float* x, const float* qLD, const float* qLDinv, const int* dof_parentid, const int* dof_Madr, int adr, int num, const int STRIDE = 1) {
  for (int k = adr + num - 1; k >= adr; k--) {
    float xk = x[k * STRIDE];
    if (xk == 0) continue;
    int a = dof_Madr[k] + 1;
    for (int i = dof_parentid[k]; i >= 0; i = dof_parentid[i]) x[i * STRIDE] -= qLD[a++] * xk;
  }
  for (int k = adr; k < adr + num; k++) x[k * STRIDE] *= qLDinv[k];
  for (int k = adr; k < adr + num; k++) {
    int a = dof_Madr[k] + 1; float xk = x[k * STRIDE];
    for (int i = dof_parentid[k]; i >= 0; i = dof_parentid[i]) xk -= qLD[a++] * x[i * STRIDE];
    x[k * STRIDE] = xk;
  }
}
DEV void solve_tree_lt(float* x, const float* qLD, const int* dof_parentid, const int* dof_Madr, int adr, int num, const int STRIDE = 1) {
  for (int k = adr + num - 1; k >= adr; k--) {
    float xk = x[k * STRIDE];
    if (xk == 0) continue;
    int a = dof_Madr[k] + 1;
    for (int i = dof_parentid[k]; i >= 0; i = dof_parentid[i]) x[i * STRIDE] -= qLD[a++] * xk;
  }
}
DEV void factor_tree(float* qLD, float* qLDinv, const int* dof_parentid, const int* dof_Madr, int adr, int num) {
  for (int k = adr + num - 1; k >= adr; k--) {
    int Mkk_a = dof_Madr[k], Mki = Mkk_a + 1;
    float Mkk = qLD[Mkk_a];
    float inv = 1.0f / Mkk;
    for (int i = dof_parentid[k]; i >= 0; i = dof_parentid[i]) {
      float tmp = qLD[Mki] * inv;
      int cnt = 0, ai = dof_Madr[i];
      for (int j = i; j >= 0; j = dof_parentid[j]) { qLD[ai + cnt] -= tmp * qLD[Mki + cnt]; cnt++; }
      qLD[Mki] = tmp;
      Mki++;
    }
    qLDinv[k] = inv;
  }
}

#define MJH_WAVE_TREE_MIN 12
#define ANC_DOF(w) ((w) & 0xffff)
#define ANC_MADR(w) ((int)((unsigned)(w) >> 16))
template <int NP, int NQ>
DEV void factor_dof_pairs(float* qLD, float* qLDinv, const int* anc, const int Mk, const int d, const int k, const int lane) {
  const int q = 1 + (lane & 15), pr = lane >> 4;
  const float dk = qLD[Mk];
  float aq[NQ], ap[NP], tg[NP][NQ]; int am[NP];
#pragma unroll
  for (int c = 0; c < NQ; c++) aq[c] = qLD[Mk + min(q + 16 * c, d)];
#pragma unroll
  for (int it = 0; it < NP; it++) { const int pp = min(1 + 4 * it + pr, d); ap[it] = qLD[Mk + pp]; am[it] = ANC_MADR(anc[Mk + pp]); }
  const float inv = 1.0f / dk;
#pragma unroll
  for (int it = 0; it < NP; it++)
#pragma unroll
    for (int c = 0; c < NQ; c++) {
      tg[it][c] = 0.0f;
      if (16 * c + 16 > 4 * it) {
        const int pp = 1 + 4 * it + pr, qq = q + 16 * c; const bool v = pp <= d && qq >= pp && qq <= d;
        tg[it][c] = qLD[v ? am[it] + (qq - pp) : Mk];
      }
    }
#pragma unroll
  for (int it = 0; it < NP; it++)
#pragma unroll
    for (int c = 0; c < NQ; c++)
      if (16 * c + 16 > 4 * it) {
        const int pp = 1 + 4 * it + pr, qq = q + 16 * c; const bool v = pp <= d && qq >= pp && qq <= d;
        if (v) qLD[am[it] + (qq - pp)] = tg[it][c] - ap[it] * inv * aq[c];
      }
#pragma unroll
  for (int c = 0; c < NQ; c++) if (pr == 0 && q + 16 * c <= d) qLD[Mk + q + 16 * c] = aq[c] * inv;
  if (lane == 0) qLDinv[k] = inv;
}
// ... 638 lines not shown
      while (true) {
        o2 = nextFetch(); processQ(o0, impl); stepDone(); if (done) break;
        o0 = nextFetch(); processQ(o1, impl); stepDone(); if (done) break;
        o1 = nextFetch(); processQ(o2, impl); stepDone(); if (done) break;
      }
    } else {
      QOp o0 = nextFetch(), o1;
      while (true) {
        o1 = nextFetch(); processQ(o0, impl); stepDone(); if (done) break;
        o0 = nextFetch(); processQ(o1, impl); stepDone(); if (done) break;
      }
    }
  } else
  if (c.nblk < 3) {
    for (int it = 0; it < itmax; it++) {
      float improvement = 0;
      for (int k = 0; k < c.nblk; k++) { MOp op = fetch8(blockAt(k)); process8(op, improvement); if (!solo) __syncthreads(); }
      niter = it + 1;
      if (improvement * c.scale < tol) break;
    }
  } else {
    MOp opA = fetch8(blockAt(0)), opB;
    for (int it = 0; it < itmax; it++) {
      float improvement = 0;
      for (int k = 0; k < c.nblk; k += 2) {
        opB = fetch8(blockAt(k + 1 < c.nblk ? k + 1 : 0));
        process8(opA, improvement);
        if (k + 1 < c.nblk) {
          opA = fetch8(blockAt(k + 2 < c.nblk ? k + 2 : 0));
          process8(opB, improvement);
        } else opA = opB;
      }
      niter = it + 1;
      if (improvement * c.scale < tol) break;
    }
  }
  }
  return niter + nmain;
}

DEV void contact_frame_force(const int hd0, const float* f, const float mu1, const float mu3, float cf[4]) {
  float ph[4] = {0, 0, 0, 0};
  const int kind = hd0 & 15, nr = (hd0 >> 4) & 15;
  for (int r = 0; r < nr; r++) {
    const float fr = f[r];
    ph[0] += fr;
    if (kind != BK_SINGLE) { const int kk = 1 + (r >> 1); ph[kk] += (r & 1) ? -fr : fr; }
  }
  cf[0] = ph[0]; cf[1] = mu1 * ph[1]; cf[2] = mu1 * ph[2]; cf[3] = mu3 * ph[3];
}

#include "patch_pgs.h"
#include "window_pgs.h"

template <int NROW, bool DIAGM, bool EXTRA, int WPRE = 0, bool HF = false>
#ifndef MJH_STEP_WAVES
#define MJH_STEP_WAVES ((!DIAGM && NROW <= 4) ? 3 : 2)
#endif
#ifndef MJH_WPRE_WAVES
#define MJH_WPRE_WAVES 2
#endif
#define MJH_STEP_WAVES_T (WPRE ? MJH_WPRE_WAVES : MJH_STEP_WAVES)
__global__ __launch_bounds__(64, MJH_STEP_WAVES_T) void mjh_step_kernel(const DConst* __restrict__ C, const DState S_arg, int env0, int nsteps, int ph, int xflags) {
#ifndef MJH_LAZY_STATE
#define MJH_LAZY_STATE true
#endif
  static_assert(alignof(DState) <= alignof(const DConst*), "the descriptor follows the first argument in the kernel-argument segment without padding");
  const DState& S = MJH_LAZY_STATE ? *(const DState*)((const char*)__builtin_amdgcn_kernarg_segment_ptr() + sizeof(const DConst*)) : S_arg;
  ASM_PROBE_BEGIN();
#ifdef MJH_WPRE_PRIO
  if constexpr (WPRE != 0) __builtin_amdgcn_s_setprio(MJH_WPRE_PRIO);
#endif
  const DModel& M = C->M;
  const Lay& L = C->L;
  extern __shared__ float lds[];
  const int lane = threadIdx.x;
  const int env = S.env_order ? S.env_order[env0 + blockIdx.x] : env0 + (int)blockIdx.x;
  const int xrow = env - env0;
  const int nq = M.nq, nv = M.nv, nbody = M.nbody, njnt = M.njnt, ngeom = M.ngeom;

#ifndef MJH_LAZY_TABLES
#define MJH_LAZY_TABLES (WPRE != 0 || (!DIAGM && NROW <= 4 && EXTRA))
#endif
#define IT(n) const XTab<MJH_LAZY_TABLES, int, &DModel::o_##n> n(M);
  MJH_INT_TABLES(IT)
#undef IT
#define FT(n) const XTab<MJH_LAZY_TABLES, float, &DModel::o_##n> n(M);
  MJH_FLT_TABLES(FT)
#undef FT
  float* const gs = NROW == 8 ? S.gscratch + (size_t)env * (size_t)S.gstride : nullptr;
#ifndef MJH_LAZY_LDS
#define MJH_LAZY_LDS (WPRE != 0)
#endif
#ifndef MJH_COLLIDE_LANES
#define MJH_COLLIDE_LANES 1
#endif
  constexpr bool COLLIDE_LANES = MJH_COLLIDE_LANES != 0 && WPRE != 0;
  constexpr bool REPORT = EXTRA && !DIAGM && WPRE == 0;
#define LA(n) const XArr<MJH_LAZY_LDS, &Lay::n> s_##n(lds, L);
  MJH_LDS_SMALL(LA)
#undef LA
#define LA(n) float* s_##n = NROW == 8 ? gs + (-1 - L.n) : lds + L.n;
  MJH_LDS_POOLS(LA)
#undef LA
  int* s_blki_i = (int*)s_blki; int* s_sched_i = (int*)s_sched; int* s_order_i = (int*)s_order; 
  const int* s_dofpar_i = DIAGM ? (dof_parentid + 0) : (const int*)s_dofpar; const int* s_dofMadr_i = DIAGM ? (dof_Madr + 0) : (const int*)s_dofMadr;
  int* s_anc_i = (int*)s_anc;
  const bool level_solves = !DIAGM && nv <= 128;
  const bool short_rows = level_solves && M.ntree <= 4;
  const float* qM_ro = (NROW == 8 && !DIAGM) ? gs + L.g_qM : s_qM;
  if constexpr (WPRE == 2) { s_J = S.wbuf + (size_t)env * (size_t)S.wstride + S.wj_off; s_B = s_J; }
  if constexpr (WPRE == 2) if (8 * max(M.maxblk, 1) <= M.maxcon * CON_STRIDE) { s_bv = s_con; s_phi = s_con + 4 * max(M.maxblk, 1); }
  if constexpr (WPRE == 1) if (C->W.slim) { s_bv = s_con; s_phi = s_con + 4 * max(M.maxblk, 1); s_J = lds + C->W.J; s_B = s_J; }
  float* s_stage = s_J;
  const int rowW = M.rowW;

  const size_t qrow = (size_t)env * M.nqp, vrow = (size_t)env * M.nvp;
  const float h = M.timestep;
  const float grav[3] = {(M.disableflags & MJH_DSBL_GRAVITY) ? 0.0f : M.gravity[0], (M.disableflags & MJH_DSBL_GRAVITY) ? 0.0f : M.gravity[1],
                         (M.disableflags & MJH_DSBL_GRAVITY) ? 0.0f : M.gravity[2]};

  if (ph & PH_RESET) {
    for (int i = lane; i < nq; i += 64) S.qpos[qrow + i] = S.initial_qpos[qrow + i];
    for (int i = lane; i < nv; i += 64) { S.qvel[vrow+i] = 0; S.qacc_ws[vrow+i] = 0; S.qvel_ref[vrow+i] = 0; S.qfrc_applied[vrow+i] = 0; S.ddq[vrow+i] = 0; S.dq[vrow+i] = 0; }
    if (lane == 0) { S.time[env] = 0; S.stats[4*env] = 0; S.stats[4*env+1] = 0; S.stats[4*env+2] = 0; S.stats[4*env+3] = 0; }
    if constexpr (REPORT) if (C->R.on) {
      const DReport& R = C->R;
      float* const rec = R.rec + (size_t)env * (size_t)R.maxcon * CREP_STRIDE;
      for (int i = lane; i < R.maxcon * CREP_STRIDE; i += 64) rec[i] = 0;
      for (int i = lane; i < 6 * nbody; i += 64) R.cfrc[(size_t)env * (size_t)(6 * nbody) + i] = 0;
      if (lane == 0) R.ncon[env] = 0;
    }
    return;
  }
  for (int i = lane; i < nq; i += 64) s_qpos[i] = S.qpos[qrow + i];
  for (int i = lane; i < nv; i += 64) {
    s_qvel[i] = S.qvel[vrow + i]; s_ws[i] = S.qacc_ws[vrow + i];
    s_qacc[i] = ((ph & PH_INV) || !(ph & PH_STEP2)) ? S.qacc[vrow + i] : 0.0f;
    if (!(ph & PH_STEP1)) { s_qvref[i] = S.qvel_ref[vrow + i]; s_applied[i] = S.qfrc_applied[vrow + i]; }
  }
  if (lane < (M.patch ? PP_ZERO : 4)) s_zero[lane] = 0;
  if (!DIAGM) {
    for (int i = lane; i < nv; i += 64) { ((int*)s_dofpar)[i] = dof_parentid[i]; ((int*)s_dofMadr)[i] = dof_Madr[i]; }
    WSYNC();
    for (int i = lane; i < nv; i += 64) {
      int a = s_dofMadr_i[i]; s_anc_i[a] = i | (a << 16);
      for (int j = s_dofpar_i[i]; j >= 0; j = s_dofpar_i[j]) s_anc_i[++a] = j | (s_dofMadr_i[j] << 16);
    }
  }
  for (int i = lane; i < 3 * ngeom; i += 64) s_p_gsize[i] = S.p_geom_size ? S.p_geom_size[(size_t)env * S.p_stride + i] : geom_size[i];
  for (int i = lane; i < ngeom; i += 64) s_p_rbound[i] = S.p_geom_rbound ? S.p_geom_rbound[(size_t)env * S.p_stride + i] : geom_rbound[i];
  for (int i = lane; i < nbody; i += 64) s_p_mass[i] = S.p_body_mass ? S.p_body_mass[(size_t)env * S.p_stride + i] : body_mass[i];
  for (int i = lane; i < 3 * nbody; i += 64) s_p_inertia[i] = S.p_body_inertia ? S.p_body_inertia[(size_t)env * S.p_stride + i] : body_inertia[i];
  const bool pre = NROW == 8 && (ph & PH_PRE), post = NROW == 8 && (ph & PH_POST);
  bool wpre = false;
  if constexpr (DIAGM && NROW <= 2) wpre = M.window != 0 && (ph & PH_PRE) && S.wbuf != nullptr;
  if (wpre && lane == 0) { int* wh0 = (int*)(S.wbuf + (size_t)env * (size_t)S.wstride); wh0[0] = 0; wh0[4] = 0; wh0[5] = 0; }
  if (post) for (int i = lane; i < nv; i += 64) s_qvel[i] = gs[L.g_qvel + i];
  double time = S.time[env];
  const unsigned slotmask = S.slot_mask ? (unsigned)__builtin_amdgcn_readfirstlane((int)S.slot_mask[env]) : 0u;
  const int sbase = nbody > 32 ? nbody - 32 : 0;
  int flags = 0, ncon = 0, nefc = 0, niter = 0, cost_hint = 0;
  PROF(0);
  if ((xflags & XF_PROF) && lane == 0) {
    S.x_prof[(size_t)blockIdx.x * PROF_STRIDE + 16] = (long long)__builtin_amdgcn_s_memrealtime();
    S.x_prof[(size_t)blockIdx.x * PROF_STRIDE + 19] = env;
    S.x_prof[(size_t)blockIdx.x * PROF_STRIDE + 18] = (long long)__builtin_amdgcn_s_getreg(63492) | ((long long)__builtin_amdgcn_s_getreg(63508) << 32);
  }
  WSYNC();
  PROF(1);

  constexpr bool LOOP = !DIAGM && NROW <= 4;
  int step = 0;
step_again:
  {
    int lane_it = (int)threadIdx.x;
    if constexpr (LOOP) asm volatile("" : "+v"(lane_it));
    const int lane = lane_it;
    cost_hint = 0;
    {
      bool badv = false;
      for (int i = lane; i < nq; i += 64) { float x = s_qpos[i]; badv |= !(x == x) || fabsf(x) > MJ_MAXVAL; }
      for (int i = lane; i < nv; i += 64) { float x = s_qvel[i], y = s_qacc[i]; badv |= !(x == x) || fabsf(x) > MJ_MAXVAL || !(y == y) || fabsf(y) > MJ_MAXVAL; }
      if (wave_any(badv)) {
        for (int i = lane; i < nq; i += 64) s_qpos[i] = S.initial_qpos[qrow + i];
        for (int i = lane; i < nv; i += 64) { s_qvel[i] = 0; s_qacc[i] = 0; s_ws[i] = 0; s_applied[i] = 0; }
        flags |= 4;
        WSYNC();
      }
    }
    if (post) {
      for (int j = lane; j < njnt; j += 64) {
        const int jt = jnt_type[j], qa = jnt_qposadr[j] + (jt == MJH_JNT_FREE ? 3 : 0);
        if (jt == MJH_JNT_FREE || jt == MJH_JNT_BALL) {
          float q[4] = {s_qpos[qa], s_qpos[qa+1], s_qpos[qa+2], s_qpos[qa+3]};
          normalize4(q);
          s_qpos[qa] = q[0]; s_qpos[qa+1] = q[1]; s_qpos[qa+2] = q[2]; s_qpos[qa+3] = q[3];
        }
      }
      for (int i = lane; i < M.nM; i += 64) s_qM[i] = gs[L.g_qM + i];
      WSYNC();
    } else {
    if (lane == 0) {
      s_xpos[0] = s_xpos[1] = s_xpos[2] = 0; s_xquat[0] = 1; s_xquat[1] = s_xquat[2] = s_xquat[3] = 0;
      for (int k = 0; k < 9; k++) { s_xmat[k] = (k % 4 == 0) ? 1.0f : 0.0f; s_ximat[k] = s_xmat[k]; }
      s_xipos[0] = s_xipos[1] = s_xipos[2] = 0;
    }
    WSYNC();
    for (int lev = 1; lev <= M.maxlevel; lev++) {
      for (int b = lane; b < nbody; b += 64) {
        if (body_level[b] != lev) continue;
        float xpos[3], xquat[4], mat[9];
        const int jn = body_jntnum[b], ja = body_jntadr[b];
        if (jn == 1 && jnt_type[ja] == MJH_JNT_FREE) {
          const int qa = jnt_qposadr[ja];
          xpos[0] = s_qpos[qa]; xpos[1] = s_qpos[qa+1]; xpos[2] = s_qpos[qa+2];
          xquat[0] = s_qpos[qa+3]; xquat[1] = s_qpos[qa+4]; xquat[2] = s_qpos[qa+5]; xquat[3] = s_qpos[qa+6];
          normalize4(xquat);
          s_qpos[qa+3] = xquat[0]; s_qpos[qa+4] = xquat[1]; s_qpos[qa+5] = xquat[2]; s_qpos[qa+6] = xquat[3];
          s_xanchor[3*ja] = xpos[0]; s_xanchor[3*ja+1] = xpos[1]; s_xanchor[3*ja+2] = xpos[2];
          s_xaxis[3*ja] = 0; s_xaxis[3*ja+1] = 0; s_xaxis[3*ja+2] = 1;
        } else if (EXTRA && M.nmocap > 0 && M.I[M.o_body_mocapid + b] >= 0) {
          const float* mp = S.mocap + ((size_t)env * M.nmocap + M.I[M.o_body_mocapid + b]) * 7;
          xpos[0] = mp[0]; xpos[1] = mp[1]; xpos[2] = mp[2]; xquat[0] = mp[3]; xquat[1] = mp[4]; xquat[2] = mp[5]; xquat[3] = mp[6];
        } else {
          const int p = body_parentid[b];
          float t[3]; rotvec(t, s_xmat + 9*p, body_pos + 3*b);
          xpos[0] = s_xpos[3*p] + t[0]; xpos[1] = s_xpos[3*p+1] + t[1]; xpos[2] = s_xpos[3*p+2] + t[2];
          mulquat(xquat, s_xquat + 4*p, body_quat + 4*b);
          for (int j = ja; j < ja + jn; j++) {
            const int qa = jnt_qposadr[j], jt = jnt_type[j];
            float vec[3], anchor[3], axis[3];
            quat2mat(mat, xquat);
            rotvec(vec, mat, jnt_pos + 3*j);
            anchor[0] = xpos[0] + vec[0]; anchor[1] = xpos[1] + vec[1]; anchor[2] = xpos[2] + vec[2];
            rotvec(axis, mat, jnt_axis + 3*j);
            if (jt == MJH_JNT_SLIDE) {
              float dq = s_qpos[qa] - qpos0[qa];
              xpos[0] += axis[0]*dq; xpos[1] += axis[1]*dq; xpos[2] += axis[2]*dq;
            } else if (jt == MJH_JNT_BALL || jt == MJH_JNT_HINGE) {
              float ql[4], r[4];
              if (jt == MJH_JNT_BALL) {
                ql[0] = s_qpos[qa]; ql[1] = s_qpos[qa+1]; ql[2] = s_qpos[qa+2]; ql[3] = s_qpos[qa+3];
                normalize4(ql);
                s_qpos[qa] = ql[0]; s_qpos[qa+1] = ql[1]; s_qpos[qa+2] = ql[2]; s_qpos[qa+3] = ql[3];
              } else axisangle2quat(ql, jnt_axis + 3*j, s_qpos[qa] - qpos0[qa]);
              mulquat(r, xquat, ql);
              xquat[0] = r[0]; xquat[1] = r[1]; xquat[2] = r[2]; xquat[3] = r[3];
              quat2mat(mat, xquat); rotvec(vec, mat, jnt_pos + 3*j);
              xpos[0] = anchor[0] - vec[0]; xpos[1] = anchor[1] - vec[1]; xpos[2] = anchor[2] - vec[2];
            }
            s_xanchor[3*j] = anchor[0]; s_xanchor[3*j+1] = anchor[1]; s_xanchor[3*j+2] = anchor[2];
            s_xaxis[3*j] = axis[0]; s_xaxis[3*j+1] = axis[1]; s_xaxis[3*j+2] = axis[2];
          }
        }
        normalize4(xquat);
        quat2mat(mat, xquat);
        float t[3], qi[4], imat[9];
        rotvec(t, mat, body_ipos + 3*b);
        mulquat(qi, xquat, body_iquat + 4*b); quat2mat(imat, qi);
#pragma unroll
        for (int k = 0; k < 3; k++) { s_xpos[3*b+k] = xpos[k]; s_xipos[3*b+k] = xpos[k] + t[k]; }
#pragma unroll
        for (int k = 0; k < 4; k++) s_xquat[4*b+k] = xquat[k];
#pragma unroll
        for (int k = 0; k < 9; k++) { s_xmat[9*b+k] = mat[k]; s_ximat[9*b+k] = imat[k]; }
      }
      WSYNC();
    }
    for (int g = lane; g < ngeom; g += 64) {
      const int b = geom_bodyid[g];
      float t[3], q[4], mat[9];
      rotvec(t, s_xmat + 9*b, geom_pos + 3*g);
      mulquat(q, s_xquat + 4*b, geom_quat + 4*g); quat2mat(mat, q);
#pragma unroll
      for (int k = 0; k < 3; k++) s_gpos[3*g+k] = s_xpos[3*b+k] + t[k];
#pragma unroll
      for (int k = 0; k < 9; k++) s_gmat[9*g+k] = mat[k];
    }
    if (EXTRA && M.nsite > 0) {
      for (int si = lane; si < M.nsite; si += 64) {
        const int b = M.I[M.o_site_bodyid + si];
        float t[3], q[4], mat[9];
        rotvec(t, s_xmat + 9*b, M.F + M.o_site_pos + 3*si);
        mulquat(q, s_xquat + 4*b, M.F + M.o_site_quat + 4*si); quat2mat(mat, q);
#pragma unroll
        for (int k = 0; k < 3; k++) s_site[12*si+k] = s_xpos[3*b+k] + t[k];
#pragma unroll
        for (int k = 0; k < 9; k++) s_site[12*si+3+k] = mat[k];
      }
    }
    if (xflags & (XF_BODY | XF_GEOM)) {
      WSYNC();
      const size_t e = xrow;
      if (S.x_xpos) for (int i = lane; i < 3*nbody; i += 64) S.x_xpos[e*3*nbody + i] = s_xpos[i];
      if (S.x_xquat) for (int i = lane; i < 4*nbody; i += 64) S.x_xquat[e*4*nbody + i] = s_xquat[i];
      if (S.x_gpos) for (int i = lane; i < 3*ngeom; i += 64) S.x_gpos[e*3*ngeom + i] = s_gpos[i];
      if (S.x_gmat) for (int i = lane; i < 9*ngeom; i += 64) S.x_gmat[e*9*ngeom + i] = s_gmat[i];
    }
    if (ph & PH_FKONLY) return;
    PROF(2);

    for (int r = lane; r < nbody; r += 64) {
      if (r == 0 || body_parentid[r] != 0) continue;
      float sm = 0, c[3] = {0, 0, 0};
      for (int b = r; b < r + body_subtreesize[r]; b++) {
        float m = s_p_mass[b]; sm += m;
        c[0] += m * s_xipos[3*b]; c[1] += m * s_xipos[3*b+1]; c[2] += m * s_xipos[3*b+2];
      }
      if (sm < MJ_MINVAL) { c[0] = s_xipos[3*r]; c[1] = s_xipos[3*r+1]; c[2] = s_xipos[3*r+2]; }
      else { float inv = 1.0f / sm; c[0] *= inv; c[1] *= inv; c[2] *= inv; }
      s_com[3*r] = c[0]; s_com[3*r+1] = c[1]; s_com[3*r+2] = c[2];
    }
    WSYNC();
    if constexpr (DIAGM) {
      for (int i = lane; i < M.nM; i += 64) { s_qM[i] = 0; }
      WSYNC();
      for (int d = lane; d < nv; d += 64) {
        const int b = dof_bodyid[d], k = d - body_dofadr[b];
        s_qM[s_dofMadr_i[d]] = (k < 3 ? s_p_mass[b] : s_p_inertia[3*b + k - 3]) + dof_armature[d];
      }
      WSYNC();
    } else {
    for (int b = lane; b < nbody; b += 64) {
      float ci[10];
      if (b == 0) { for (int k = 0; k < 10; k++) ci[k] = 0; }
      else {
        const float* com = s_com + 3*body_rootid[b];
        float off[3] = {s_xipos[3*b] - com[0], s_xipos[3*b+1] - com[1], s_xipos[3*b+2] - com[2]};
        inert_com(ci, s_p_inertia + 3*b, s_ximat + 9*b, off, s_p_mass[b]);
      }
#pragma unroll
      for (int k = 0; k < 10; k++) s_cinert[10*b+k] = ci[k];
    }
    for (int d = lane; d < nv; d += 64) {
      const int j = dof_jntid[d], b = dof_bodyid[d], jt = jnt_type[j];
      int k = d - jnt_dofadr[j];
      const float* com = s_com + 3*body_rootid[b];
      float off[3] = {com[0] - s_xanchor[3*j], com[1] - s_xanchor[3*j+1], com[2] - s_xanchor[3*j+2]};
      float cd[6];
      if (jt == MJH_JNT_FREE && k < 3) { cd[0] = cd[1] = cd[2] = 0; cd[3] = (k == 0); cd[4] = (k == 1); cd[5] = (k == 2); }
      else if (jt == MJH_JNT_FREE || jt == MJH_JNT_BALL) {
        if (jt == MJH_JNT_FREE) k -= 3;
        float ax[3] = {s_xmat[9*b + k], s_xmat[9*b + 3 + k], s_xmat[9*b + 6 + k]};
        cd[0] = ax[0]; cd[1] = ax[1]; cd[2] = ax[2]; cross3(cd + 3, ax, off);
      } else if (jt == MJH_JNT_SLIDE) { cd[0] = cd[1] = cd[2] = 0; cd[3] = s_xaxis[3*j]; cd[4] = s_xaxis[3*j+1]; cd[5] = s_xaxis[3*j+2]; }
      else { float ax[3] = {s_xaxis[3*j], s_xaxis[3*j+1], s_xaxis[3*j+2]}; cd[0] = ax[0]; cd[1] = ax[1]; cd[2] = ax[2]; cross3(cd + 3, ax, off); }
#pragma unroll
      for (int q = 0; q < 6; q++) s_cdof[6*d+q] = cd[q];
    }
    WSYNC();
    for (int b = lane; b < nbody; b += 64) {
      float acc[10];
#pragma unroll
      for (int k = 0; k < 10; k++) acc[k] = 0;
      if (b > 0) for (int c = b; c < b + body_subtreesize[b]; c++)
#pragma unroll
        for (int k = 0; k < 10; k++) acc[k] += s_cinert[10*c+k];
#pragma unroll
      for (int k = 0; k < 10; k++) s_crb[10*b+k] = acc[k];
    }
    WSYNC();
    for (int i = lane; i < nv; i += 64) {
      float buf[6], cd[6];
#pragma unroll
      for (int q = 0; q < 6; q++) cd[q] = s_cdof[6*i+q];
      mul_inert_vec(buf, s_crb + 10*dof_bodyid[i], cd);
      int adr = s_dofMadr_i[i];
      for (int j = i; j >= 0; j = s_dofpar_i[j]) {
        float v = 0;
#pragma unroll
        for (int q = 0; q < 6; q++) v += s_cdof[6*j+q] * buf[q];
        if (j == i) v += dof_armature[i];
        s_qM[adr] = v; s_qLD[adr] = v;
        if (NROW == 8) gs[L.g_qM + adr] = v;
        adr++;
      }
    }
    WSYNC();
    }
    if (ph & PH_MULM) {
      for (int i = lane; i < nv; i += 64) { s_tmpv[i] = S.x_vec[(size_t)blockIdx.x * M.nvp + i]; s_tmpv2[i] = 0; }
      WSYNC();
      for (int i = lane; i < nv; i += 64) {
        int adr = s_dofMadr_i[i]; float vi = s_tmpv[i], acc = s_qM[adr] * vi; int k = 1;
        for (int j = s_dofpar_i[i]; j >= 0; j = s_dofpar_i[j]) { float mij = s_qM[adr + k]; acc += mij * s_tmpv[j]; atomicAdd(&s_tmpv2[j], mij * vi); k++; }
        atomicAdd(&s_tmpv2[i], acc);
      }
      WSYNC();
      for (int i = lane; i < nv; i += 64) S.x_res[(size_t)blockIdx.x * M.nvp + i] = s_tmpv2[i];
      return;
    }
    PROF(3);
    if (DIAGM) { for (int d = lane; d < nv; d += 64) s_qLDinv[d] = 1.0f / s_qM[s_dofMadr_i[d]]; }
    else {
      for (int t = 0; t < M.ntree; t++) if (tree_dofnum[t] >= MJH_WAVE_TREE_MIN) factor_tree_wave(s_qLD, s_qLDinv, s_anc_i, s_dofMadr_i, tree_dofadr[t], tree_dofnum[t], M.nM, nv, lane);
      if (short_rows) factor_trees_short(s_qLD, s_qLDinv, s_anc_i, s_dofMadr_i, tree_dofadr, tree_dofnum, M.ntree, M.nM, nv, lane);
      else for (int t = lane; t < M.ntree; t += 64) if (tree_dofnum[t] < MJH_WAVE_TREE_MIN) factor_tree(s_qLD, s_qLDinv, s_dofpar_i, s_dofMadr_i, tree_dofadr[t], tree_dofnum[t]);
    }
    WSYNC();
    }

    PROF(4);
    ncon = 0;
    if (!post && !(M.disableflags & (MJH_DSBL_CONTACT | MJH_DSBL_CONSTRAINT))) {
      int conbase = 0;
      auto hfield_pair = [&](const auto ipu) __attribute__((always_inline)) {
        const Tab<int> geom_dataid{M.I, M.o_geom_dataid}, mesh_vertadr{M.I, M.o_mesh_vertadr}, mesh_vertnum{M.I, M.o_mesh_vertnum};
        const DHField& H = C->H;
        const int g1 = pair_geom1[ipu], g2 = pair_geom2[ipu], t2 = geom_type[g2];
        float* const stp = s_stage + pair_stageadr[ipu] * RAW_STRIDE;
        const int hid = geom_dataid[g1];
        const int hnr = M.I[H.o_hfield_nrow + hid], hnc = M.I[H.o_hfield_ncol + hid];
        const float* const hdat = M.F + H.o_hfield_data + M.I[H.o_hfield_adr + hid];
        const float hsx = M.F[H.o_hfield_size + 4*hid], hsy = M.F[H.o_hfield_size + 4*hid + 1], hsz = M.F[H.o_hfield_size + 4*hid + 2], hsb = M.F[H.o_hfield_size + 4*hid + 3];
        const float hmargin = fmaxf(geom_margin[g1], geom_margin[g2]);
        CvxGeom P1, P2;
        P1.type = MJH_GEOM_HFIELD; P1.vert = nullptr; P1.nvert = 0; P1.pad = P2.pad = 0;
        P2.type = t2; P2.vert = nullptr; P2.nvert = 0;
        if (t2 == MJH_GEOM_MESH) { const int id = geom_dataid[g2]; P2.vert = M.F + M.o_mesh_vert + 3 * mesh_vertadr[id]; P2.nvert = mesh_vertnum[id]; }
        float lp[3];
#pragma unroll
        for (int k = 0; k < 9; k++) { P1.mat[k] = s_gmat[9*g1+k]; P2.mat[k] = s_gmat[9*g2+k]; }
#pragma unroll
        for (int k = 0; k < 3; k++) { P1.size[k] = 0; P2.pos[k] = s_gpos[3*g2+k]; P2.size[k] = s_p_gsize[3*g2+k]; lp[k] = P2.pos[k] - s_gpos[3*g1+k]; }
        { float t[3]; rotvecT(t, P1.mat, lp); lp[0] = t[0]; lp[1] = t[1]; lp[2] = t[2]; }
        const float rb2 = s_p_rbound[g2], R = rb2 + hmargin;
        const float dxc = 2.0f * hsx / (float)(hnc - 1), dyc = 2.0f * hsy / (float)(hnr - 1);
        const bool outside = lp[0] + R < -hsx || lp[0] - R > hsx || lp[1] + R < -hsy || lp[1] - R > hsy || lp[2] - R > hsz || lp[2] + R < -hsb;
        const int c0 = (int)fminf(fmaxf(floorf((lp[0] - R + hsx) / dxc), 0.0f), (float)(hnc - 2)), c1 = (int)fminf(fmaxf(floorf((lp[0] + R + hsx) / dxc), 0.0f), (float)(hnc - 2));
        const int r0 = (int)fminf(fmaxf(floorf((lp[1] - R + hsy) / dyc), 0.0f), (float)(hnr - 2)), r1 = (int)fminf(fmaxf(floorf((lp[1] + R + hsy) / dyc), 0.0f), (float)(hnr - 2));
        const int ncell = c1 - c0 + 1, nprism = outside ? 0 : 2 * ncell * (r1 - r0 + 1);
        const float low = lp[2] - rb2 - hmargin;
        int cnt = 0;
        for (int base = 0; base < nprism && cnt < MJH_HFIELD_MAXCON; base += 64) {
          const int k = min(base + lane, nprism - 1), cell = k >> 1, r = r0 + cell / ncell, c = c0 + cell % ncell;
          const int rc = (k & 1) ? r + 1 : r, cc = (k & 1) ? c : c + 1;
          const float xa = -hsx + dxc * (float)c, xb = -hsx + dxc * (float)(c + 1), xc = -hsx + dxc * (float)cc;
          const float ya = -hsy + dyc * (float)r, yb = -hsy + dyc * (float)(r + 1), yc = -hsy + dyc * (float)rc;
          const float ta = hdat[r * hnc + c] * hsz, tb = hdat[(r + 1) * hnc + c + 1] * hsz, tcc = hdat[rc * hnc + cc] * hsz;
          const bool act = base + lane < nprism && fmaxf(ta, fmaxf(tb, tcc)) >= low;
          const float cx = (xa + xb + xc) * (1.0f / 3.0f), cy = (ya + yb + yc) * (1.0f / 3.0f), cz = (ta + tb + tcc - 3.0f * hsb) * (1.0f / 6.0f);
          HfPrism hp;
          hp.x[0] = xa - cx; hp.x[1] = xb - cx; hp.x[2] = xc - cx; hp.y[0] = ya - cy; hp.y[1] = yb - cy; hp.y[2] = yc - cy;
          hp.top[0] = ta - cz; hp.top[1] = tb - cz; hp.top[2] = tcc - cz; hp.bot = -hsb - cz;
          { const float cl[3] = {cx, cy, cz}; float cw[3]; rotvec(cw, P1.mat, cl);
#pragma unroll
            for (int q = 0; q < 3; q++) P1.pos[q] = s_gpos[3*g1+q] + cw[q]; }
          float rbuf[RAW_STRIDE];
#pragma unroll
          for (int q = 0; q < RAW_STRIDE; q++) rbuf[q] = 0;
          bool got = false;
          if (wave_any(act)) got = c_convex_wave<true>(P1, P2, hmargin, rbuf, act, lane, &hp) != 0 && act;
          const unsigned long long gm = __ballot(got);
          const int idx = cnt + __popcll(gm & ((1ull << lane) - 1ull));
          if (got && idx < MJH_HFIELD_MAXCON) {
#pragma unroll
            for (int q = 0; q < RAW_STRIDE; q++) stp[idx * RAW_STRIDE + q] = rbuf[q];
          }
          cnt += __popcll(gm);
        }
        return min(cnt, MJH_HFIELD_MAXCON);
      };
      auto collide_round = [&](const int ip) __attribute__((always_inline)) {
        int n = 0, g1 = 0, g2 = 0; float margin = 0, gap = 0;
        float* st = s_stage;
        CvxGeom G1, G2; bool cvx = false, hf = false;
        G1.type = G2.type = 0; G1.vert = G2.vert = nullptr; G1.nvert = G2.nvert = 0; G1.pad = G2.pad = 0;
#pragma unroll
        for (int k = 0; k < 9; k++) { G1.mat[k] = G2.mat[k] = 0; if (k < 3) { G1.pos[k] = G2.pos[k] = 0; G1.size[k] = G2.size[k] = 0; } }
        if (ip >= 0) {
          g1 = pair_geom1[ip]; g2 = pair_geom2[ip];
          st = s_stage + pair_stageadr[ip] * RAW_STRIDE;
          const int t1 = geom_type[g1], t2 = geom_type[g2];
          margin = fmaxf(geom_margin[g1], geom_margin[g2]); gap = fmaxf(geom_gap[g1], geom_gap[g2]);
          float p1[3], p2[3], m1[9], m2[9], z1[3], z2[3];
#pragma unroll
          for (int k = 0; k < 3; k++) { p1[k] = s_gpos[3*g1+k]; p2[k] = s_gpos[3*g2+k]; z1[k] = s_p_gsize[3*g1+k]; z2[k] = s_p_gsize[3*g2+k]; }
#pragma unroll
          for (int k = 0; k < 9; k++) { m1[k] = s_gmat[9*g1+k]; m2[k] = s_gmat[9*g2+k]; }
          bool cull;
          const int sb1 = geom_bodyid[g1], sb2 = geom_bodyid[g2];
          const unsigned r1 = (unsigned)(sb1 - sbase), r2 = (unsigned)(sb2 - sbase);
          const bool parked = ((r1 < 32u && ((slotmask >> r1) & 1u)) || (r2 < 32u && ((slotmask >> r2) & 1u)));
          float tt[3] = {p2[0]-p1[0], p2[1]-p1[1], p2[2]-p1[2]};
          if (t1 == MJH_GEOM_PLANE) { float nn[3] = {m1[2], m1[5], m1[8]}; cull = dot3(tt, nn) > s_p_rbound[g2] + margin; }
          else { float bound = s_p_rbound[g1] + s_p_rbound[g2] + margin; cull = dot3(tt, tt) > bound * bound; }
          if (!cull && !parked) {
            if (t1 == MJH_GEOM_PLANE && t2 == MJH_GEOM_BOX) n = c_plane_box(p1, m1, p2, m2, z2, margin, st);
            else if (t1 == MJH_GEOM_BOX && t2 == MJH_GEOM_BOX) n = c_box_box(p1, m1, z1, p2, m2, z2, margin, st);
            else if (t1 == MJH_GEOM_PLANE && t2 == MJH_GEOM_SPHERE) n = c_plane_sphere(p1, m1, p2, z2[0], margin, st, 0);
            else if (t1 == MJH_GEOM_PLANE && t2 == MJH_GEOM_CAPSULE) n = c_plane_capsule(p1, m1, p2, m2, z2, margin, st);
            else if (t1 == MJH_GEOM_PLANE && t2 == MJH_GEOM_CYLINDER) n = c_plane_cylinder(p1, m1, p2, m2, z2, margin, st);
            else if (t1 == MJH_GEOM_SPHERE && t2 == MJH_GEOM_SPHERE) n = c_sphere_sphere(p1, z1[0], p2, z2[0], margin, st);
            else if (t1 == MJH_GEOM_SPHERE && t2 == MJH_GEOM_CAPSULE) n = c_sphere_capsule(p1, z1[0], p2, m2, z2, margin, st);
            else if (t1 == MJH_GEOM_CAPSULE && t2 == MJH_GEOM_CAPSULE) n = c_capsule_capsule(p1, m1, z1, p2, m2, z2, margin, st);
            else if (t1 == MJH_GEOM_SPHERE && t2 == MJH_GEOM_BOX) n = c_sphere_box(p1, z1[0], p2, m2, z2, margin, st);
            else if (t1 == MJH_GEOM_PLANE && t2 == MJH_GEOM_ELLIPSOID) n = c_plane_ellipsoid(p1, m1, p2, m2, z2, margin, st);
            else if (EXTRA && t2 == MJH_GEOM_MESH && t1 == MJH_GEOM_PLANE) {
              const Tab<int> geom_dataid{M.I, M.o_geom_dataid}, mesh_vertadr{M.I, M.o_mesh_vertadr}, mesh_vertnum{M.I, M.o_mesh_vertnum};
              const Tab<float> mesh_vert{M.F, M.o_mesh_vert};
              const int id = geom_dataid[g2];
              n = c_plane_mesh(p1, m1, p2, m2, mesh_vert + 3 * mesh_vertadr[id], mesh_vertnum[id], margin, st);
            } else if (EXTRA && pair_is_convex(t1, t2)) {
              const Tab<int> geom_dataid{M.I, M.o_geom_dataid}, mesh_vertadr{M.I, M.o_mesh_vertadr}, mesh_vertnum{M.I, M.o_mesh_vertnum};
              const Tab<float> mesh_vert{M.F, M.o_mesh_vert};
              cvx = true;
              G1.type = t1; G2.type = t2; G1.vert = G2.vert = nullptr; G1.nvert = G2.nvert = 0;
              if (t1 == MJH_GEOM_MESH) { const int id = geom_dataid[g1]; G1.vert = mesh_vert + 3 * mesh_vertadr[id]; G1.nvert = mesh_vertnum[id]; }
              if (t2 == MJH_GEOM_MESH) { const int id = geom_dataid[g2]; G2.vert = mesh_vert + 3 * mesh_vertadr[id]; G2.nvert = mesh_vertnum[id]; }
#pragma unroll
              for (int k = 0; k < 3; k++) { G1.pos[k] = p1[k]; G2.pos[k] = p2[k]; G1.size[k] = z1[k]; G2.size[k] = z2[k]; }
#pragma unroll
              for (int k = 0; k < 9; k++) { G1.mat[k] = m1[k]; G2.mat[k] = m2[k]; }
            } else if (HF && t1 == MJH_GEOM_HFIELD) hf = true;
          }
        }
        if constexpr (EXTRA) { if (wave_any(cvx)) { const int nc = c_convex_wave(G1, G2, margin, st, cvx, lane); if (cvx) n = nc; } }
        if constexpr (HF) {
          unsigned long long req = __ballot(hf);
          while (req) {
            const int owner = __ffsll((long long)req) - 1; req &= req - 1;
            const int nh = hfield_pair(__builtin_amdgcn_readlane(ip, owner));
            if (lane == owner) n = nh;
          }
          WSYNC();
        }
        CPROF(0);
        const int incl = wave_incl_scan_i(n, lane);
        const int total = wave_last_i(incl);
        const int first = conbase + incl - n;
        CPROF(1);
        if constexpr (COLLIDE_LANES) {
          const int exst = (incl - n) | ((int)(st - s_stage) << 10);
          const int gw = g1 | (g2 << 12) | (max(geom_condim[g1], geom_condim[g2]) << 24);
          const float mg = margin - gap;
          WSYNC();
          for (int c0 = 0; c0 < total; c0 += 64) {
            const int c = min(c0 + lane, total - 1), idx = conbase + c;
            const bool live = c0 + lane < total && idx < M.maxcon;
            int pl = 0;
#pragma unroll
            for (int stp = 32; stp > 0; stp >>= 1) { if (__builtin_amdgcn_ds_bpermute((pl + stp - 1) << 2, incl) <= c) pl += stp; }
            const int es = __builtin_amdgcn_ds_bpermute(pl << 2, exst);
            const float* r = s_stage + (es >> 10) + (c - (es & 1023)) * RAW_STRIDE;
            float* cc = s_con + min(idx, M.maxcon - 1) * CON_STRIDE;
            float fr[9]; fr[0] = r[4]; fr[1] = r[5]; fr[2] = r[6];
            const float r0 = r[0], r1 = r[1], r2 = r[2], r3 = r[3];
            if (live) { cc[0] = r0; cc[1] = r1; cc[2] = r2; cc[3] = r3; }
            make_frame(fr);
            if (live) {
#pragma unroll
              for (int k = 0; k < 9; k++) cc[4+k] = fr[k];
            }
            const int gwp = __builtin_amdgcn_ds_bpermute(pl << 2, gw);
            if (live) cc[CON_GEOMS] = __int_as_float(gwp);
            const int mgp = __builtin_amdgcn_ds_bpermute(pl << 2, __builtin_bit_cast(int, mg));
            if (live) cc[CON_MARGIN] = __int_as_float(mgp);
          }
        } else
        for (int q = 0; q < n; q++) {
          const int idx = first + q;
          if (idx >= M.maxcon) break;
          const float* r = st + q * RAW_STRIDE;
          float fr[9]; fr[0] = r[4]; fr[1] = r[5]; fr[2] = r[6];
          make_frame(fr);
          float* c = s_con + idx * CON_STRIDE;
          c[0] = r[0]; c[1] = r[1]; c[2] = r[2]; c[3] = r[3];
#pragma unroll
          for (int k = 0; k < 9; k++) c[4+k] = fr[k];
          c[CON_GEOMS] = __int_as_float(g1 | (g2 << 12) | (max(geom_condim[g1], geom_condim[g2]) << 24)); c[CON_MARGIN] = margin - gap;
        }
        CPROF(2);
        conbase += total;
      };
      auto survives = [&](const int ip) __attribute__((always_inline)) {
        const int g1 = pair_geom1[ip], g2 = pair_geom2[ip];
        const float margin = fmaxf(geom_margin[g1], geom_margin[g2]);
        const int sb1 = geom_bodyid[g1], sb2 = geom_bodyid[g2];
        const unsigned r1 = (unsigned)(sb1 - sbase), r2 = (unsigned)(sb2 - sbase);
        const bool parked = (r1 < 32u && ((slotmask >> (r1 & 31u)) & 1u)) | (r2 < 32u && ((slotmask >> (r2 & 31u)) & 1u));
        const float tt[3] = {s_gpos[3*g2] - s_gpos[3*g1], s_gpos[3*g2+1] - s_gpos[3*g1+1], s_gpos[3*g2+2] - s_gpos[3*g1+2]};
        const float nn[3] = {s_gmat[9*g1+2], s_gmat[9*g1+5], s_gmat[9*g1+8]};
        const float rb2 = s_p_rbound[g2], bound = s_p_rbound[g1] + rb2 + margin;
        const bool far_plane = dot3(tt, nn) > rb2 + margin, far_sphere = dot3(tt, tt) > bound * bound;
        return !parked & !(geom_type[g1] == MJH_GEOM_PLANE ? far_plane : far_sphere);
      };
      const int poolcap = NROW == 8 ? (max(M.maxblk, 1) * BLKQ_STRIDE) & ~63 : 0;
      const bool pool_list = NROW == 8 && poolcap >= M.npair;
      const int listcap = pool_list ? poolcap : (4 * (((nv + 3) / 4) * 4)) & ~63;
      if (M.npair > 64 && listcap >= 64) {
        int* list = pool_list ? (int*)s_blkq : (int*)s_smooth;
        for (int c0 = 0; c0 < M.npair; c0 += listcap) {
          const int c1 = min(c0 + listcap, M.npair);
          int cnt = 0;
          for (int base = c0; base < c1; base += 256) {
            bool sv[4];
#pragma unroll
            for (int u = 0; u < 4; u++) { const int ip = base + 64 * u + lane; sv[u] = survives(min(ip, c1 - 1)) & (ip < c1); }
#pragma unroll
            for (int u = 0; u < 4; u++) {
              const unsigned long long mk = __ballot(sv[u]);
              if (sv[u]) list[cnt + __popcll(mk & ((1ull << lane) - 1ull))] = base + 64 * u + lane;
              cnt += __popcll(mk);
            }
          }
          WSYNC();
          for (int b2 = 0; b2 < cnt; b2 += 64) collide_round(b2 + lane < cnt ? list[b2 + lane] : -1);
          WSYNC();
        }
      } else {
        for (int base = 0; base < M.npair; base += 64) collide_round(base + lane < M.npair ? base + lane : -1);
      }
      if (conbase > M.maxcon) { flags |= 1; conbase = M.maxcon; }
      ncon = __builtin_amdgcn_readfirstlane(conbase);
    }
    WSYNC();
    if ((xflags & XF_CON) && S.x_contacts) {
      float* o = S.x_contacts + (size_t)blockIdx.x * ((size_t)M.maxcon * CON_STRIDE + 4);
      for (int i = lane; i < ncon * CON_STRIDE; i += 64) o[i] = s_con[i];
      if (lane == 0) { o[(size_t)M.maxcon * CON_STRIDE] = __int_as_float(ncon); o[(size_t)M.maxcon * CON_STRIDE + 1] = __int_as_float(flags); }
      if (xflags & XF_NOSTORE) return;
      WSYNC();
    }

    PROF(5);
    nefc = 0;
    int nblk = 0, nbrow = 0, nfixblk = 0;
    if (!post && !(M.disableflags & MJH_DSBL_CONSTRAINT)) {
      auto put_block = [&](int b, int kind, int nrows, int nb, int clamp, int joff4, int id, int rtype, int side) __attribute__((always_inline)) {
        int* hd = s_blki_i + b * BLKI_STRIDE;
        hd[0] = kind | (nrows << 4) | (nb << 8) | (clamp << 12) | (joff4 << 16); hd[1] = id | (rtype << 24) | (side << 28);
      };
      const int w4 = rowW >> 2;
      if (!(M.disableflags & MJH_DSBL_EQUALITY))
        for (int e = 0; e < M.neq; e++) if (eq_active[e]) {
          const int et = (EXTRA && M.has_weld) ? M.I[M.o_eq_type + e] : MJH_EQ_JOINT;
          const int nr = et == MJH_EQ_WELD ? 6 : (et == MJH_EQ_CONNECT ? 3 : 1);
          if (lane < nr) put_block(nblk + lane, BK_SINGLE, 1, 1, 0, (nblk + lane) * w4, et == MJH_EQ_JOINT ? e : (e | (lane << 16)), et == MJH_EQ_JOINT ? RT_EQ : RT_WELD, 0);
          nblk += nr; nbrow += nr; nefc += nr;
        }
      if (!(M.disableflags & MJH_DSBL_FRICTIONLOSS)) {
        for (int f = lane; f < M.nfl; f += 64) put_block(nblk + f, BK_SINGLE, 1, 1, 2, (nblk + f) * w4, fl_dof[f], RT_FL, 0);
        nblk += M.nfl; nbrow += M.nfl; nefc += M.nfl;
      }
      if (M.has_limits && !(M.disableflags & MJH_DSBL_LIMIT)) {
        for (int base = 0; base < njnt; base += 64) {
          const int j = base + lane; int lo = 0, hi = 0;
          if (j < njnt && jnt_limited[j] && (jnt_type[j] == MJH_JNT_HINGE || jnt_type[j] == MJH_JNT_SLIDE)) {
            float val = s_qpos[jnt_qposadr[j]], mg = jnt_margin[j];
            lo = (val - jnt_range[2*j]) < mg; hi = (jnt_range[2*j+1] - val) < mg;
          }
          const int n = lo + hi, incl = wave_incl_scan_i(n, lane);
          int r = incl - n;
          if (lo) { put_block(nblk + r, BK_SINGLE, 1, 1, 1, (nblk + r) * w4, j, RT_LIMIT, 0); r++; }
          if (hi) put_block(nblk + r, BK_SINGLE, 1, 1, 1, (nblk + r) * w4, j, RT_LIMIT, 1);
          const int tot = wave_last_i(incl);
          nblk += tot; nbrow += tot; nefc += tot;
        }
      }
      const int nfix = nblk; nfixblk = nblk;
      bool stop = false;
      for (int base = 0; base < ncon && !stop; base += 64) {
        const int ic = base + lane; int nr = 0, nb = 0, dim = 0;
        if (ic < ncon) {
          const float* c = s_con + ic * CON_STRIDE;
          dim = CON_DIM(c);
          if (c[0] < c[CON_MARGIN]) { nr = dim == 1 ? 1 : 2 * (dim - 1); nb = dim == 1 ? 1 : (dim == 3 ? 3 : 4); }
        }
        const int inc = nr > 0;
        const int sr = wave_incl_scan_i(nr, lane), sb = wave_incl_scan_i(nb, lane), sc = wave_incl_scan_i(inc, lane);
        const unsigned long long over = __ballot(inc && nefc + sr > M.maxefc);
        const int firstover = over ? __ffsll((long long)over) - 1 : 64;
        if (inc && lane < firstover)
          put_block(nblk + sc - 1, dim == 1 ? BK_SINGLE : (dim == 3 ? BK_PYR3 : BK_PYR4), nr, nb, 1, (nfix + 4 * (nblk + sc - 1 - nfix)) * w4, ic, RT_CONTACT, 0);
        int last = 63;
        if (over) { flags |= 2; stop = true; last = firstover - 1; }
        if (last >= 0) { const int ul = __builtin_amdgcn_readfirstlane(last); nefc += __builtin_amdgcn_readlane(sr, ul); nbrow += __builtin_amdgcn_readlane(sb, ul); nblk += __builtin_amdgcn_readlane(sc, ul); }
      }
    }
    nefc = __builtin_amdgcn_readfirstlane(nefc); nblk = __builtin_amdgcn_readfirstlane(nblk); nbrow = __builtin_amdgcn_readfirstlane(nbrow);
    const bool dense_pre = NROW == 8 && !DIAGM && pre && (xflags & XF_DENSE) && nefc > 0 && nefc <= M.dense_cap;
    WSYNC();
    PROF(6);
    for (int t = lane; t < 4 * nblk; t += 64) {
      const int b = t >> 2, jb = t & 3;
      int* hd = s_blki_i + b * BLKI_STRIDE;
      const int nb = (hd[0] >> 8) & 15;
      const int SL = BLK_SLOTS(hd[1]);
      if (jb >= SL) continue;
      float* J = s_J + BLK_JOFF(hd[0]) + jb;
      for (int k = 0; k < rowW; k++) J[SL*k] = 0;
      if (jb >= nb) continue;
      const int id = hd[1] & 0xffffff, rtype = (hd[1] >> 24) & 15, side = (hd[1] >> 28) & 1;
      int t1 = -1, t2 = -1;
      if (rtype == RT_EQ) {
        const int j1 = eq_obj1id[id], j2 = eq_obj2id[id];
        const float* dat = eq_data + 11*id;
        const int d1 = jnt_dofadr[j1];
        t1 = dof_treeid[d1];
        J[SL*(d1 - tree_dofadr[t1])] = 1;
        if (j2 >= 0) {
          const int d2 = jnt_dofadr[j2];
          const float p2 = s_qpos[jnt_qposadr[j2]] - qpos0[jnt_qposadr[j2]];
          const float deriv = dat[1] + p2*(2*dat[2] + p2*(3*dat[3] + p2*4*dat[4]));
          const int tt = dof_treeid[d2];
          if (tt == t1) J[SL*(d2 - tree_dofadr[t1])] += -deriv;
          else { t2 = tt; J[SL*(tree_dofnum[t1] + d2 - tree_dofadr[t2])] = -deriv; }
        }
      } else if (rtype == RT_FL) { t1 = dof_treeid[id]; J[SL*(id - tree_dofadr[t1])] = 1; }
      else if (rtype == RT_LIMIT) { const int d = jnt_dofadr[id]; t1 = dof_treeid[d]; J[SL*(d - tree_dofadr[t1])] = side ? -1.0f : 1.0f; }
      else if (EXTRA && rtype == RT_WELD) {
        const int e = id & 0xffff, r = id >> 16;
        const int b1 = eq_obj1id[e], b2 = eq_obj2id[e];
        const bool weld = M.I[M.o_eq_type + e] == MJH_EQ_WELD;
        const float* dat = eq_data + 11*e;
        t1 = body_treeid[b1]; t2 = body_treeid[b2];
        if (t1 < 0) { t1 = t2; t2 = -1; }
        if (t2 == t1) t2 = -1;
        float q1i[4] = {s_xquat[4*b1], -s_xquat[4*b1+1], -s_xquat[4*b1+2], -s_xquat[4*b1+3]}, q2r[4];
        { const float rel[4] = {dat[6], dat[7], dat[8], dat[9]}; mulquat(q2r, s_xquat + 4*b2, rel); }
        const float ts = dat[10];
#pragma unroll
        for (int sd = 0; sd < 2; sd++) {
          const int bd = sd ? b2 : b1; const float ss = sd ? -1.0f : 1.0f;
          int i = bd > 0 ? body_lastdof[bd] : -1;
          if (i < 0 || t1 < 0) continue;
          const float* an = weld ? (sd ? dat : dat + 3) : (sd ? dat + 3 : dat);
          float pw[3]; rotvec(pw, s_xmat + 9*bd, an);
          const float* com = s_com + 3*body_rootid[bd];
          const float off[3] = {s_xpos[3*bd] + pw[0] - com[0], s_xpos[3*bd+1] + pw[1] - com[1], s_xpos[3*bd+2] + pw[2] - com[2]};
          const int tr = dof_treeid[i];
          const int o = (tr == t1) ? -tree_dofadr[t1] : tree_dofnum[t1] - tree_dofadr[t2];
          for (; i >= 0; i = s_dofpar_i[i]) {
            const float* cd = s_cdof + 6*i;
            float v;
            if (r < 3) { float cr[3]; cross3(cr, cd, off); v = ss * (cd[3 + r] + cr[r]); }
            else {
              const float w[4] = {0.0f, -ss * cd[0], -ss * cd[1], -ss * cd[2]};
              float u[4], vv[4]; mulquat(u, q1i, w); mulquat(vv, u, q2r);
              v = 0.5f * ts * vv[1 + (r - 3)];
            }
            J[SL*(o + i)] += v;
          }
        }
      }
      else {
        const float* c = s_con + id * CON_STRIDE;
        const int g1 = CON_G1(c), g2 = CON_G2(c);
        const int b1 = geom_bodyid[g1], b2 = geom_bodyid[g2];
        t1 = body_treeid[b1]; t2 = body_treeid[b2];
        const int t1raw = t1, t2raw = t2;
        if (t1 < 0) { t1 = t2; t2 = -1; }
        if (t2 == t1) t2 = -1;
        const float* dir = c + 4 + 3 * (jb < 3 ? jb : 0);
        const float musc = jb == 0 ? 1.0f : (jb < 3 ? fmaxf(geom_friction[3*g1], geom_friction[3*g2]) : fmaxf(geom_friction[3*g1+1], geom_friction[3*g2+1]));
#pragma unroll
        for (int sd = 0; sd < 2; sd++) {
          const int bd = sd ? b2 : b1; const float ss = (sd ? 1.0f : -1.0f) * musc;
          if constexpr (DIAGM) {
            const int tr = sd ? t2raw : t1raw;
            if (tr < 0) continue;
            const int o = (tr == t1) ? 0 : 6;
            const float* com = s_com + 3*bd;
            const float off[3] = {c[1] - com[0], c[2] - com[1], c[3] - com[2]};
            const float* xm = s_xmat + 9*bd;
            float tq[3];
            if (jb < 3) { cross3(tq, off, dir); J[SL*o] = ss * dir[0]; J[SL*(o+1)] = ss * dir[1]; J[SL*(o+2)] = ss * dir[2]; }
            else { tq[0] = dir[0]; tq[1] = dir[1]; tq[2] = dir[2]; }
#pragma unroll
            for (int k = 0; k < 3; k++) J[SL*(o+3+k)] = ss * (xm[k] * tq[0] + xm[3+k] * tq[1] + xm[6+k] * tq[2]);
            continue;
          }
          int i = body_lastdof[bd];
          if (i < 0) continue;
          const float* com = s_com + 3*body_rootid[bd];
          const float off[3] = {c[1] - com[0], c[2] - com[1], c[3] - com[2]};
          const int tr = dof_treeid[i];
          const int o = (tr == t1) ? -tree_dofadr[t1] : tree_dofnum[t1] - tree_dofadr[t2];
          for (; i >= 0; i = s_dofpar_i[i]) {
            const float* cd = s_cdof + 6*i;
            float v;
            if (jb < 3) { float cr[3]; cross3(cr, cd, off); const float jp[3] = {cd[3] + cr[0], cd[4] + cr[1], cd[5] + cr[2]}; v = dot3(dir, jp); }
            else v = dot3(dir, cd);
            J[SL*(o + i)] += ss * v;
          }
        }
      }
      if (jb == 0) {
        if (EXTRA && t1 < 0) { hd[2] = 0xffff; hd[3] = 0xffff; }
        else { hd[2] = tree_dofadr[t1] | (tree_dofnum[t1] << 16); hd[3] = t2 >= 0 ? (tree_dofadr[t2] | (tree_dofnum[t2] << 16)) : 0xffff; }
      }
    }
    auto p_dinv = [&](int d) __attribute__((always_inline)) { return S.p_dof_invweight0 ? S.p_dof_invweight0[(size_t)env * S.p_stride + d] : dof_invweight0[d]; };
    auto p_binv = [&](int i) __attribute__((always_inline)) { return S.p_body_invweight0 ? S.p_body_invweight0[(size_t)env * S.p_stride + i] : body_invweight0[i]; };
    for (int b = lane; b < nblk; b += 64) {
      const int* hd = s_blki_i + b * BLKI_STRIDE;
      const int id = hd[1] & 0xffffff, rtype = (hd[1] >> 24) & 15, side = (hd[1] >> 28) & 1;
      float* bf = s_blkf + b * BLKF_STRIDE;
      for (int k = 0; k < BLKF_STRIDE; k++) bf[k] = 0;
      float pos = 0, margin = 0, diagA = 0, fl = 0, mu1 = 0, mu3 = 0, rscale = -1, sr[2], si[5];
      if (rtype == RT_EQ) {
        const int j1 = eq_obj1id[id], j2 = eq_obj2id[id];
        const float* dat = eq_data + 11*id;
        const float pos1 = s_qpos[jnt_qposadr[j1]] - qpos0[jnt_qposadr[j1]];
        diagA = p_dinv(jnt_dofadr[j1]);
        if (j2 >= 0) {
          const float p2 = s_qpos[jnt_qposadr[j2]] - qpos0[jnt_qposadr[j2]];
          pos = pos1 - (dat[0] + p2*(dat[1] + p2*(dat[2] + p2*(dat[3] + p2*dat[4]))));
          diagA += p_dinv(jnt_dofadr[j2]);
        } else pos = pos1 - dat[0];
        sr[0] = eq_solref[2*id]; sr[1] = eq_solref[2*id+1];
#pragma unroll
        for (int q = 0; q < 5; q++) si[q] = eq_solimp[5*id+q];
      } else if (rtype == RT_FL) {
        diagA = p_dinv(id); fl = dof_frictionloss[id];
        sr[0] = dof_solref[2*id]; sr[1] = dof_solref[2*id+1];
#pragma unroll
        for (int q = 0; q < 5; q++) si[q] = dof_solimp[5*id+q];
      } else if (rtype == RT_LIMIT) {
        const float val = s_qpos[jnt_qposadr[id]];
        pos = side ? jnt_range[2*id+1] - val : val - jnt_range[2*id];
        margin = jnt_margin[id]; diagA = p_dinv(jnt_dofadr[id]);
        sr[0] = jnt_solref[2*id]; sr[1] = jnt_solref[2*id+1];
#pragma unroll
        for (int q = 0; q < 5; q++) si[q] = jnt_solimp[5*id+q];
      } else if (EXTRA && rtype == RT_WELD) {
        const int e = id & 0xffff, r = id >> 16;
        const int b1 = eq_obj1id[e], b2 = eq_obj2id[e];
        const bool weld = M.I[M.o_eq_type + e] == MJH_EQ_WELD;
        const float* dat = eq_data + 11*e;
        if (r < 3) {
          float p1[3], p2[3];
          rotvec(p1, s_xmat + 9*b1, weld ? dat + 3 : dat); rotvec(p2, s_xmat + 9*b2, weld ? dat : dat + 3);
          pos = (s_xpos[3*b1 + r] + p1[r]) - (s_xpos[3*b2 + r] + p2[r]);
          diagA = p_binv(2*b1) + p_binv(2*b2);
        } else {
          const float q1i[4] = {s_xquat[4*b1], -s_xquat[4*b1+1], -s_xquat[4*b1+2], -s_xquat[4*b1+3]}, rel[4] = {dat[6], dat[7], dat[8], dat[9]};
          float q2r[4], qe[4]; mulquat(q2r, s_xquat + 4*b2, rel); mulquat(qe, q1i, q2r);
          pos = dat[10] * qe[1 + (r - 3)];
          diagA = p_binv(2*b1+1) + p_binv(2*b2+1);
        }
        sr[0] = eq_solref[2*e]; sr[1] = eq_solref[2*e+1];
#pragma unroll
        for (int q = 0; q < 5; q++) si[q] = eq_solimp[5*e+q];
      } else {
        const float* c = s_con + id * CON_STRIDE;
        const int g1 = CON_G1(c), g2 = CON_G2(c), dim = CON_DIM(c);
        const int b1 = geom_bodyid[g1], b2 = geom_bodyid[g2];
        pos = c[0]; margin = c[CON_MARGIN];
        const float f0 = fmaxf(geom_friction[3*g1], geom_friction[3*g2]), f1 = fmaxf(geom_friction[3*g1+1], geom_friction[3*g2+1]);
        mu1 = f0; mu3 = f1;
        const float tran = p_binv(2*b1) + p_binv(2*b2);
        if (dim == 1) diagA = tran;
        else { diagA = tran + f0*f0*tran; const float mu0 = f0 * rsqrtf(M.impratio); rscale = 2 * mu0 * mu0; }
        const float a = geom_solmix[g1], bq = geom_solmix[g2];
        const float mix = (a >= MJ_MINVAL && bq >= MJ_MINVAL) ? a / (a + bq) : ((a < MJ_MINVAL && bq < MJ_MINVAL) ? 0.5f : (a < MJ_MINVAL ? 0.0f : 1.0f));
        sr[0] = mix*geom_solref[2*g1] + (1-mix)*geom_solref[2*g2]; sr[1] = mix*geom_solref[2*g1+1] + (1-mix)*geom_solref[2*g2+1];
#pragma unroll
        for (int q = 0; q < 5; q++) si[q] = mix*geom_solimp[5*g1+q] + (1-mix)*geom_solimp[5*g2+q];
      }
      const float imp = get_impedance(si, pos, margin);
      float R = fmaxf(MJ_MINVAL, (1 - imp) * diagA / imp);
      if (rscale > 0) R = fmaxf(MJ_MINVAL, rscale * R);
      float sr0 = sr[0], K, Bc; const float sr1 = sr[1], dmax = fminf(MAXIMP, fmaxf(MINIMP, si[1]));
      if (sr0 > 0) {
        if (!(M.disableflags & MJH_DSBL_REFSAFE)) sr0 = fmaxf(sr0, 2 * h);
        K = 1 / fmaxf(MJ_MINVAL, dmax*dmax * sr0*sr0 * sr1*sr1); Bc = 2 / fmaxf(MJ_MINVAL, dmax * sr0);
      } else { K = -sr0 / fmaxf(MJ_MINVAL, dmax*dmax); Bc = -sr1 / fmaxf(MJ_MINVAL, dmax); }
      if (rtype == RT_FL) K = 0;
      (void)mu1; (void)mu3;
      bf[0] = R; bf[1] = fl; bf[2] = K * imp * (pos - margin); bf[3] = Bc;
    }
    WSYNC();
    PROF(7);
    if (!DIAGM && NROW == 8 && M.k1_floats >= 16 * rowW) {
      const int P = min(64, M.k1_floats / rowW);
      for (int t0 = 0; t0 < 4 * nblk; t0 += P) {
        const int t = t0 + lane;
        if (lane >= P || t >= 4 * nblk) continue;
        const int b = t >> 2, jb = t & 3;
        const int* hd = s_blki_i + b * BLKI_STRIDE;
        const int SL = BLK_SLOTS(hd[1]);
        if (jb >= SL) continue;
        const float* J = s_J + BLK_JOFF(hd[0]) + jb; float* B = s_B + BLK_JOFF(hd[0]) + jb;
        if (jb >= ((hd[0] >> 8) & 15)) { for (int k = 0; k < rowW; k++) B[SL*k] = 0; continue; }
        ROW_TREES(hd[2], hd[3]);
        float* x = lds + M.scratch_off + lane;
        for (int k = 0; k < rowW; k++) x[k * P] = J[SL*k];
        if (dense_pre) {
          solve_tree_lt(x - a1 * P, s_qLD, s_dofpar_i, s_dofMadr_i, a1, n1, P);
          if (n2 > 0) solve_tree_lt(x + (n1 - a2) * P, s_qLD, s_dofpar_i, s_dofMadr_i, a2, n2, P);
        } else {
          solve_tree(x - a1 * P, s_qLD, s_qLDinv, s_dofpar_i, s_dofMadr_i, a1, n1, P);
          if (n2 > 0) solve_tree(x + (n1 - a2) * P, s_qLD, s_qLDinv, s_dofpar_i, s_dofMadr_i, a2, n2, P);
        }
        for (int k = 0; k < rowW; k++) B[SL*k] = x[k * P];
      }
      WSYNC();
    } else if (!DIAGM) {
      for (int t = lane; t < 4 * nblk; t += 64) {
        const int b = t >> 2, jb = t & 3;
        const int* hd = s_blki_i + b * BLKI_STRIDE;
        const int SL = BLK_SLOTS(hd[1]);
        if (jb >= SL) continue;
        const float* J = s_J + BLK_JOFF(hd[0]) + jb; float* B = s_B + BLK_JOFF(hd[0]) + jb;
        if (jb >= ((hd[0] >> 8) & 15)) { for (int k = 0; k < rowW; k++) B[SL*k] = 0; continue; }
        ROW_TREES(hd[2], hd[3]);
        for (int k = 0; k < rowW; k++) B[SL*k] = J[SL*k];
        if (dense_pre) {
          solve_tree_lt(B - SL*a1, s_qLD, s_dofpar_i, s_dofMadr_i, a1, n1, SL);
          if (n2 > 0) solve_tree_lt(B + SL*(n1 - a2), s_qLD, s_dofpar_i, s_dofMadr_i, a2, n2, SL);
          continue;
        }
        solve_tree(B - SL*a1, s_qLD, s_qLDinv, s_dofpar_i, s_dofMadr_i, a1, n1, SL);
        if (n2 > 0) solve_tree(B + SL*(n1 - a2), s_qLD, s_qLDinv, s_dofpar_i, s_dofMadr_i, a2, n2, SL);
      }
      WSYNC();
    }
    int ngrp = 0;
    bool patch_order = false;
    if constexpr (DIAGM && NROW <= 2) patch_order = M.patch != 0;
    if constexpr (WPRE != 0) patch_order = true;
    if (!patch_order && M.pgs_row_order) {
      bool listed = false;
      auto tree_of = [&](const int adr) __attribute__((always_inline)) { if constexpr (DIAGM) return adr / 6; else return (int)dof_treeid[adr]; };
      if constexpr (NROW <= 2) {
        if (M.pgs_row_order == 1 && nblk <= 64 && M.ntree <= 64) {
          listed = true;
          int t1 = -1, t2 = -1;
          if (lane < nblk) {
            const int* hd = s_blki_i + lane * BLKI_STRIDE;
            const int a = hd[2] & 0xffff;
            if (a != 0xffff) t1 = tree_of(a);
            if ((hd[3] >> 16) != 0) t2 = tree_of(hd[3] & 0xffff);
          }
          int lastv = 0, cntv = 0, mygrp = 0, myrank = 0;
          for (int i = 0; i < nblk; i++) {
            const int a = __builtin_amdgcn_readlane(t1, i), b = __builtin_amdgcn_readlane(t2, i);
            const int ea = a >= 0 ? __builtin_amdgcn_readlane(lastv, a) : 0, eb = b >= 0 ? __builtin_amdgcn_readlane(lastv, b) : 0;
            const int e = max(ea, eb);
            const unsigned long long bal = __ballot(cntv < 2 && lane >= e);
            const int g = __ffsll((long long)bal) - 1;
// ... 924 lines not shown
          const float R = op.P.x, lo = op.r2.z, hi = op.r2.w;
          if (kind == BK_PYR4) pgs_block<4, 6, NROW, EXTRA>(ns, R, lo, hi, aref, f, Q, X, Jd, Bp, bs, a, improvement);
          else if (kind == BK_PYR3) pgs_block<3, 4, NROW, EXTRA>(ns, R, lo, hi, aref, f, Q, X, Jd, Bp, bs, a, improvement);
          else pgs_block<1, 1, NROW, EXTRA>(ns, R, lo, hi, aref, f, Q, X, Jd, Bp, bs, a, improvement);
          if (lane == 0) {
            float* bf = s_blkf + b * BLKF_STRIDE + BF_F;
            *(float4*)(bf) = make_float4(f[0], f[1], f[2], f[3]);
            *(float2*)(bf + 4) = make_float2(f[4], f[5]);
          }
        };
        for (int mode = 0; mode < nmode; mode++) {
        if (mode == 1) { ns = true; nmain = niter; niter = 0; itmax = M.noslip_iterations; tol = M.noslip_tolerance; WSYNC(); }
        for (int it = 0; it < itmax; it++) {
          float improvement = 0;
          BlkOp opA = fetch(s_order_i[0]), opB;
          for (int k = 0; k < nblk; k += 2) {
            const int b0 = s_order_i[k], b1 = s_order_i[k + 1 < nblk ? k + 1 : k], b2 = s_order_i[k + 2 < nblk ? k + 2 : k];
            opB = fetch(b1);
            process(opA, b0, improvement);
            if (k + 1 < nblk) {
              opA = fetch(b2);
              process(opB, b1, improvement);
            }
          }
          niter = it + 1;
          if (improvement * scale < tol) break;
          WSYNC();
        }
        }
        niter += nmain;
        }
        WSYNC();
        if (NROW != 8 && d0 < nv && lane < 64 / (NROW <= 2 ? 2 : 1)) { s_qacc[d0] = a; s_ws[d0] = a; }
        PROF(13);
        WSYNC();
        if (xflags & XF_FORCE) { phi_from_forces(); accum_T(false, s_phi, s_tmpv2); }
        }
      }
      }
      if (xflags & XF_FORCE) {
        const size_t e = (size_t)xrow * M.nvp;
        for (int d = lane; d < nv; d += 64) { if (S.x_smooth) S.x_smooth[e + d] = s_asmooth[d]; if (S.x_constraint) S.x_constraint[e + d] = s_tmpv2[d]; }
      }
      if constexpr (EXTRA) {
      bool report = false;
      if constexpr (REPORT) report = C->R.on != 0;
      const bool sensors = M.nsensor > 0 && S.sensordata;
      if ((sensors || report) && !post) {
        WSYNC();
        const float* xf = S.xfrc_applied ? S.xfrc_applied + (size_t)env * S.xfrc_stride : nullptr;
        for (int b = lane; b < nbody; b += 64) {
          float F[6] = {0, 0, 0, 0, 0, 0};
          if (b > 0) {
            const float* com = s_com + 3*body_rootid[b];
            auto add = [&](const float* point, const float* force, const float* torque, const float sg) __attribute__((always_inline)) {
              const float off[3] = {point[0] - com[0], point[1] - com[1], point[2] - com[2]};
              float cr[3]; cross3(cr, off, force);
              F[0] += sg * (torque[0] + cr[0]); F[1] += sg * (torque[1] + cr[1]); F[2] += sg * (torque[2] + cr[2]);
              F[3] += sg * force[0]; F[4] += sg * force[1]; F[5] += sg * force[2];
            };
            if (xf) { const float f[3] = {xf[6*b], xf[6*b+1], xf[6*b+2]}, t[3] = {xf[6*b+3], xf[6*b+4], xf[6*b+5]}; add(s_xipos + 3*b, f, t, 1.0f); }
            for (int k = 0; k < nblk; k++) {
              const int* hd = s_blki_i + k * BLKI_STRIDE;
              const int id = hd[1] & 0xffffff, rtype = (hd[1] >> 24) & 15;
              const float* bf = s_blkf + k * BLKF_STRIDE;
              if (rtype == RT_CONTACT) {
                const float* c = s_con + id * CON_STRIDE;
                const int g1 = CON_G1(c), g2 = CON_G2(c);
                const int b1 = geom_bodyid[g1], b2 = geom_bodyid[g2];
                if (b1 != b && b2 != b) continue;
                const float mu1 = fmaxf(geom_friction[3*g1], geom_friction[3*g2]), mu3 = fmaxf(geom_friction[3*g1+1], geom_friction[3*g2+1]);
                float cf[4];
                contact_frame_force(hd[0], bf + BF_F, mu1, mu3, cf);
                const float tors = cf[3];
                float Fw[3], Tw[3];
#pragma unroll
                for (int q = 0; q < 3; q++) { Fw[q] = c[4+q] * cf[0] + c[7+q] * cf[1] + c[10+q] * cf[2]; Tw[q] = c[4+q] * tors; }
                if (b2 == b) add(c + 1, Fw, Tw, 1.0f);
                if (b1 == b) add(c + 1, Fw, Tw, -1.0f);
              } else if (rtype == RT_WELD) {
                const int e = id & 0xffff, r = id >> 16;
                const int b1 = eq_obj1id[e], b2 = eq_obj2id[e];
                if (b1 != b && b2 != b) continue;
                const bool weld = M.I[M.o_eq_type + e] == MJH_EQ_WELD;
                const float* dat = eq_data + 11*e;
                const float f = bf[BF_F];
                const float z3[3] = {0, 0, 0};
                const bool first = b1 == b;
                float pw[3]; rotvec(pw, s_xmat + 9*b, weld ? (first ? dat + 3 : dat) : (first ? dat : dat + 3));
                const float pt[3] = {s_xpos[3*b] + pw[0], s_xpos[3*b+1] + pw[1], s_xpos[3*b+2] + pw[2]};
                if (r < 3) { float fv[3] = {0, 0, 0}; fv[r] = f; add(pt, fv, z3, first ? 1.0f : -1.0f); }
                else {
                  const float q1i[4] = {s_xquat[4*b1], -s_xquat[4*b1+1], -s_xquat[4*b1+2], -s_xquat[4*b1+3]}, rel[4] = {dat[6], dat[7], dat[8], dat[9]};
                  float q2r[4]; mulquat(q2r, s_xquat + 4*b2, rel);
                  float T[3];
#pragma unroll
                  for (int a = 0; a < 3; a++) {
                    const float w[4] = {0.0f, a == 0 ? 1.0f : 0.0f, a == 1 ? 1.0f : 0.0f, a == 2 ? 1.0f : 0.0f};
                    float u[4], vv[4]; mulquat(u, q1i, w); mulquat(vv, u, q2r);
                    T[a] = 0.5f * dat[10] * vv[1 + (r - 3)] * f;
                  }
                  add(pt, z3, T, first ? -1.0f : 1.0f);
                }
              }
            }
          }
#pragma unroll
          for (int q = 0; q < 6; q++) s_fext[6*b+q] = F[q];
        }
        WSYNC();
        if constexpr (REPORT) if (report) {
          const DReport& R = C->R;
          float* const rec = R.rec + (size_t)env * (size_t)R.maxcon * CREP_STRIDE;
          for (int c = lane; c < ncon; c += 64) *(float4*)(s_phi + 4 * c) = make_float4(0.0f, 0.0f, 0.0f, 0.0f);
          WSYNC();
          for (int k = lane; k < nblk; k += 64) {
            const int* hd = s_blki_i + k * BLKI_STRIDE;
            if (((hd[1] >> 24) & 15) != RT_CONTACT) continue;
            const int id = hd[1] & 0xffffff;
            if (id >= ncon) continue;
            const float* c = s_con + id * CON_STRIDE;
            const int g1 = CON_G1(c), g2 = CON_G2(c);
            const float mu1 = fmaxf(geom_friction[3*g1], geom_friction[3*g2]), mu3 = fmaxf(geom_friction[3*g1+1], geom_friction[3*g2+1]);
            float cf[4];
            contact_frame_force(hd[0], s_blkf + k * BLKF_STRIDE + BF_F, mu1, mu3, cf);
            *(float4*)(s_phi + 4 * id) = make_float4(cf[0], cf[1], cf[2], cf[3]);
          }
          WSYNC();
          for (int c = lane; c < ncon; c += 64) {
            const float4* r = (const float4*)(s_con + c * CON_STRIDE);
            const float4 r0 = r[0], r1 = r[1], r2 = r[2], r3 = r[3], f = *(const float4*)(s_phi + 4 * c);
            const int gw = __float_as_int(r3.y);
            float4* o = (float4*)(rec + (size_t)c * CREP_STRIDE);
            o[0] = r0; o[1] = r1; o[2] = r2;
            o[3] = make_float4(r3.x, f.x, f.y, f.z);
            o[4] = make_float4(f.w, __int_as_float(gw & 0xfff), __int_as_float((gw >> 12) & 0xfff), __int_as_float(gw >> 24));
          }
          if (lane == 0) R.ncon[env] = ncon;
          for (int i = lane; i < 6 * nbody; i += 64) R.cfrc[(size_t)env * (size_t)(6 * nbody) + i] = s_fext[i];
          WSYNC();
        }
        if (sensors) {
        if (lane == 0) { for (int k = 0; k < 6; k++) { s_cvel[k] = 0; s_cacc[k] = (k >= 3) ? -grav[k-3] : 0.0f; s_cfrc[k] = 0; } }
        WSYNC();
        for (int lev = 1; lev <= M.maxlevel; lev++) {
          for (int b = lane; b < nbody; b += 64) {
            if (body_level[b] != lev) continue;
            const int p = body_parentid[b];
            float cv[6], ca[6];
#pragma unroll
            for (int q = 0; q < 6; q++) { cv[q] = s_cvel[6*p+q]; ca[q] = s_cacc[6*p+q]; }
            int bda = body_dofadr[b];
            for (int j = 0; j < body_jntnum[b]; j++) {
              const int jt = jnt_type[body_jntadr[b] + j];
              if (jt == MJH_JNT_FREE) {
                for (int k = 0; k < 3; k++)
#pragma unroll
                  for (int q = 0; q < 6; q++) { s_cdofdot[6*(bda+k)+q] = 0; cv[q] += s_cdof[6*(bda+k)+q] * s_qvel[bda+k]; }
                bda += 3;
              }
              const int nd = (jt == MJH_JNT_FREE || jt == MJH_JNT_BALL) ? 3 : 1;
              float cvn[6];
#pragma unroll
              for (int q = 0; q < 6; q++) cvn[q] = cv[q];
              for (int k = 0; k < nd; k++) {
                float cd[6], cdd[6];
#pragma unroll
                for (int q = 0; q < 6; q++) cd[q] = s_cdof[6*(bda+k)+q];
                cross_motion(cdd, cv, cd);
                const float v = s_qvel[bda+k];
#pragma unroll
                for (int q = 0; q < 6; q++) { s_cdofdot[6*(bda+k)+q] = cdd[q]; cvn[q] += cd[q] * v; }
              }
#pragma unroll
              for (int q = 0; q < 6; q++) cv[q] = cvn[q];
              bda += nd;
            }
            for (int d = body_dofadr[b]; d < body_dofadr[b] + body_dofnum[b]; d++) {
              const float v = s_qvel[d], a = s_qacc[d];
#pragma unroll
              for (int q = 0; q < 6; q++) ca[q] += s_cdofdot[6*d+q] * v + s_cdof[6*d+q] * a;
            }
            float ci[10], f[6], t[6], t1[6];
#pragma unroll
            for (int k = 0; k < 10; k++) ci[k] = s_cinert[10*b+k];
            mul_inert_vec(f, ci, ca); mul_inert_vec(t, ci, cv); cross_force(t1, cv, t);
#pragma unroll
            for (int q = 0; q < 6; q++) { s_cvel[6*b+q] = cv[q]; s_cacc[6*b+q] = ca[q]; s_cfrc[6*b+q] = f[q] + t1[q] - s_fext[6*b+q]; }
          }
          WSYNC();
        }
        for (int si = lane; si < M.nsensor; si += 64) {
          const int site = M.I[M.o_sensor_objid + si], b = M.I[M.o_site_bodyid + site];
          float F[6] = {0, 0, 0, 0, 0, 0};
          for (int c = b; c < b + body_subtreesize[b]; c++)
#pragma unroll
            for (int q = 0; q < 6; q++) F[q] += s_cfrc[6*c+q];
          const float* com = s_com + 3*body_rootid[b];
          const float* sp = s_site + 12*site;
          const float off[3] = {sp[0] - com[0], sp[1] - com[1], sp[2] - com[2]};
          float cr[3]; cross3(cr, off, F + 3);
          const float tq[3] = {F[0] - cr[0], F[1] - cr[1], F[2] - cr[2]};
          const float* src = M.I[M.o_sensor_type + si] == MJH_SENS_FORCE ? F + 3 : tq;
          float* out = S.sensordata + ((size_t)env * M.nsensor + si) * 3;
#pragma unroll
          for (int k = 0; k < 3; k++) out[k] = sp[3+k] * src[0] + sp[6+k] * src[1] + sp[9+k] * src[2];
        }
        WSYNC();
        }
      }
      }
      if (ph & PH_STEP2) {
        bool badv = false;
        for (int i = lane; i < nv; i += 64) { float y = s_qacc[i]; badv |= !(y == y) || fabsf(y) > MJ_MAXVAL; }
        if (wave_any(badv)) {
          for (int i = lane; i < nq; i += 64) s_qpos[i] = S.initial_qpos[qrow + i];
          for (int i = lane; i < nv; i += 64) { s_qvel[i] = 0; s_qacc[i] = 0; s_ws[i] = 0; s_applied[i] = 0; s_tmpv2[i] = 0; s_smooth[i] = 0; }
          flags |= 4;
          WSYNC();
        }
        float* qint = s_qacc;
        if (M.has_damping && !(M.disableflags & MJH_DSBL_EULERDAMP)) {
          for (int i = lane; i < M.nM; i += 64) s_qLD[i] = qM_ro[i];
          for (int d = lane; d < nv; d += 64) s_tmpv[d] = dof_damping[d] * s_qacc[d];
          WSYNC();
          for (int d = lane; d < nv; d += 64) s_qLD[s_dofMadr_i[d]] += h * dof_damping[d];
          WSYNC();
          for (int t = 0; t < M.ntree; t++) if (tree_dofnum[t] >= MJH_WAVE_TREE_MIN) {
            factor_tree_wave(s_qLD, s_qLDinv, s_anc_i, s_dofMadr_i, tree_dofadr[t], tree_dofnum[t], M.nM, nv, lane);
            if (!level_solves) solve_tree_wave(s_tmpv, s_qLD, s_qLDinv, s_anc_i, s_dofMadr_i, tree_dofadr[t], tree_dofnum[t], M.nM, nv, lane);
          }
          if (short_rows) factor_trees_short(s_qLD, s_qLDinv, s_anc_i, s_dofMadr_i, tree_dofadr, tree_dofnum, M.ntree, M.nM, nv, lane);
          else for (int t = lane; t < M.ntree; t += 64) if (tree_dofnum[t] < MJH_WAVE_TREE_MIN) {
            factor_tree(s_qLD, s_qLDinv, s_dofpar_i, s_dofMadr_i, tree_dofadr[t], tree_dofnum[t]);
            if (!level_solves) solve_tree(s_tmpv, s_qLD, s_qLDinv, s_dofpar_i, s_dofMadr_i, tree_dofadr[t], tree_dofnum[t]);
          }
          WSYNC();
          if (level_solves) solve_trees_levels(s_tmpv, s_qLD, s_qLDinv, s_anc_i, s_dofMadr_i, nv, M.nM, lane);
          WSYNC();
          for (int d = lane; d < nv; d += 64) s_tmpv[d] = s_qacc[d] - h * s_tmpv[d];
          WSYNC();
          qint = s_tmpv;
        }
        for (int d = lane; d < nv; d += 64) {
          const int bd = dof_bodyid[d];
          const unsigned rb = (unsigned)(bd - sbase);
          const bool parked = rb < 32u && ((slotmask >> rb) & 1u);
          s_qvel[d] = parked ? 0.0f : s_qvel[d] + h * qint[d];
          if (parked) { s_qacc[d] = 0; s_ws[d] = 0; }
        }
        WSYNC();
        for (int j = lane; j < njnt; j += 64) {
          const int qa = jnt_qposadr[j], da = jnt_dofadr[j], jt = jnt_type[j];
          if (jt == MJH_JNT_FREE) {
            s_qpos[qa] += h * s_qvel[da]; s_qpos[qa+1] += h * s_qvel[da+1]; s_qpos[qa+2] += h * s_qvel[da+2];
            float q[4] = {s_qpos[qa+3], s_qpos[qa+4], s_qpos[qa+5], s_qpos[qa+6]}, w[3] = {s_qvel[da+3], s_qvel[da+4], s_qvel[da+5]};
            quat_integrate(q, w, h);
            s_qpos[qa+3] = q[0]; s_qpos[qa+4] = q[1]; s_qpos[qa+5] = q[2]; s_qpos[qa+6] = q[3];
          } else if (jt == MJH_JNT_BALL) {
            float q[4] = {s_qpos[qa], s_qpos[qa+1], s_qpos[qa+2], s_qpos[qa+3]}, w[3] = {s_qvel[da], s_qvel[da+1], s_qvel[da+2]};
            quat_integrate(q, w, h);
            s_qpos[qa] = q[0]; s_qpos[qa+1] = q[1]; s_qpos[qa+2] = q[2]; s_qpos[qa+3] = q[3];
          } else s_qpos[qa] += h * s_qvel[da];
        }
        time += M.timestep_d;
        WSYNC();
        if (lane == 0 && odom[9]) {
          const float* v = S.odom_vel + (size_t)env * 6;
          const float ax = odom[6] >= 0 ? s_qpos[odom[6]] : 0.0f, ay = odom[7] >= 0 ? s_qpos[odom[7]] : 0.0f, az = odom[8] >= 0 ? s_qpos[odom[8]] : 0.0f;
          const float sx = sinf(ax), cx = cosf(ax), sy = sinf(ay), cy = cosf(ay), sz = sinf(az), cz = cosf(az);
          if (odom[0] >= 0) s_qvel[odom[0]] = v[0]*cy*cz + v[1]*(sx*sy*cz - cx*sz) + v[2]*(cx*sy*cz + sx*sz);
          if (odom[1] >= 0) s_qvel[odom[1]] = v[0]*cy*sz + v[1]*(sx*sy*sz + cx*cz) + v[2]*(cx*sy*sz - sx*cz);
          if (odom[2] >= 0) s_qvel[odom[2]] = -v[0]*sy + v[1]*sx*cy + v[2]*cx*cy;
          for (int k = 0; k < 3; k++) if (odom[3+k] >= 0) s_qvel[odom[3+k]] = v[3+k];
        }
        WSYNC();
      }
    }
  }
  if constexpr (LOOP) { if (++step < nsteps) goto step_again; }

  PROF(14);
  if ((ph & (PH_FKONLY | PH_MULM)) || (xflags & XF_NOSTORE)) return;
  for (int i = lane; i < nq; i += 64) S.qpos[qrow + i] = s_qpos[i];
  for (int i = lane; i < nv; i += 64) {
    S.qvel[vrow + i] = s_qvel[i]; S.qacc_ws[vrow + i] = s_ws[i];
// ... 104 lines not shown
```

Before: 16.82 million.

## Pack per-geom contact parameters into aligned records and tag global address space loads

Result: no change. 16.88 million (median of 6 runs) (+0.4%).

```diff
diff --git a/mujoco_sim_amd/csrc/dev_convex.h b/mujoco_sim_amd/csrc/dev_convex.h
--- a/mujoco_sim_amd/csrc/dev_convex.h
+++ b/mujoco_sim_amd/csrc/dev_convex.h
@@ -66,20 +66,22 @@
     if (den > MJ_MINVAL) { const float inv = 1.0f / den; pl[0] = w0*inv; pl[1] = w1*inv; pl[2] = w2*inv; }
   }
 }
+template <bool GV = false>
 DEV void mesh_support_wave(const bool want, const float* vert, const int nvert, const float* dl, float* pl, const int lane) {
   unsigned long long req = __ballot(want);
   const unsigned long long va = (unsigned long long)vert;
   const int valo = (int)(unsigned)va, vahi = (int)(unsigned)(va >> 32);
   while (req) {
     constexpr int NB = 4;
-    int L[NB], nv[NB]; const float* vp[NB]; float d0[NB], d1[NB], d2[NB]; bool on[NB];
+    using VP = std::conditional_t<GV, const MJH_GLOBAL_AS float*, const float*>;
+    int L[NB], nv[NB]; VP vp[NB]; float d0[NB], d1[NB], d2[NB]; bool on[NB];
 #pragma unroll
     for (int u = 0; u < NB; u++) {
       on[u] = req != 0;
       L[u] = on[u] ? __ffsll((long long)req) - 1 : 0;
       if (on[u]) req &= req - 1;
       const unsigned lo = (unsigned)__builtin_amdgcn_readlane(valo, L[u]), hi = (unsigned)__builtin_amdgcn_readlane(vahi, L[u]);
-      vp[u] = (const float*)(((unsigned long long)hi << 32) | lo);
+      vp[u] = (VP)(((unsigned long long)hi << 32) | lo);
       nv[u] = on[u] ? __builtin_amdgcn_readlane(nvert, L[u]) : 0;
       d0[u] = readlane_f(dl[0], L[u]); d1[u] = readlane_f(dl[1], L[u]); d2[u] = readlane_f(dl[2], L[u]);
     }
@@ -126,16 +128,16 @@
     if (dp > bd) { bd = dp; pl[0] = x; pl[1] = y; pl[2] = z; }
   }
 }
-template <bool PRISM = false>
+template <bool PRISM = false, bool GV = false>
 DEV void mpr_support_wave(const CvxGeom& g1, const CvxGeom& g2, const float* dir, MprPt& p, const bool act, const int lane, const HfPrism* h = nullptr) {
   const float nd[3] = {-dir[0], -dir[1], -dir[2]};
   float dl1[3], dl2[3], pl1[3], pl2[3], a[3], b[3];
   rotvecT(dl1, g1.mat, dir); rotvecT(dl2, g2.mat, nd);
   if constexpr (PRISM) prism_support_local(*h, dl1, pl1); else cvx_support_local(g1, dl1, pl1);
   cvx_support_local(g2, dl2, pl2);
-  if constexpr (!PRISM) mesh_support_wave(act && g1.type == MJH_GEOM_MESH, g1.vert, g1.nvert, dl1, pl1, lane);
+  if constexpr (!PRISM) mesh_support_wave<GV>(act && g1.type == MJH_GEOM_MESH, g1.vert, g1.nvert, dl1, pl1, lane);
   if constexpr (PRISM) { if (g2.type == MJH_GEOM_MESH) mesh_support_lane(g2.vert, g2.nvert, dl2, pl2); }
-  else mesh_support_wave(act && g2.type == MJH_GEOM_MESH, g2.vert, g2.nvert, dl2, pl2, lane);
+  else mesh_support_wave<GV>(act && g2.type == MJH_GEOM_MESH, g2.vert, g2.nvert, dl2, pl2, lane);
   rotvec(a, g1.mat, pl1); rotvec(b, g2.mat, pl2);
 #pragma unroll
   for (int k = 0; k < 3; k++) {
@@ -144,7 +146,7 @@
   }
 }
 
-template <bool PRISM = false>
+template <bool PRISM = false, bool GV = false>
 DEV int c_convex_wave(CvxGeom& g1, CvxGeom& g2, float margin, float* st, const bool act, const int lane, const HfPrism* h = nullptr) {
   g1.pad = g2.pad = 0.5f * margin;
   MprPt p0, p1, p2, p3, p4;
@@ -159,7 +161,7 @@
   bool live = act;
   int res = 0;
   while (__ballot(live) != 0) {
-    mpr_support_wave<PRISM>(g1, g2, n, p4, live, lane, h);
+    mpr_support_wave<PRISM, GV>(g1, g2, n, p4, live, lane, h);
     if (live) {
     const float d4 = dot3(p4.v, n);
     if (phase == PH_FIRST) {
diff --git a/mujoco_sim_amd/csrc/dev_math.h b/mujoco_sim_amd/csrc/dev_math.h
--- a/mujoco_sim_amd/csrc/dev_math.h
+++ b/mujoco_sim_amd/csrc/dev_math.h
@@ -2,6 +2,8 @@
 #include <hip/hip_runtime.h>
 
 #define DEV __device__ __forceinline__
+#define MJH_GLOBAL_AS __attribute__((address_space(1)))
+typedef float mjh_f4 __attribute__((ext_vector_type(4)));
 #define HDEV __host__ __device__ __forceinline__
 #if !defined(__HIP_DEVICE_COMPILE__)
 static inline float rsqrtf(float x) { return 1.0f / sqrtf(x); }
diff --git a/mujoco_sim_amd/csrc/dev_types.h b/mujoco_sim_amd/csrc/dev_types.h
--- a/mujoco_sim_amd/csrc/dev_types.h
+++ b/mujoco_sim_amd/csrc/dev_types.h
@@ -99,7 +99,9 @@
 #define CREP_DIM 19
 struct DReport { int on, maxcon; int* ncon; float* rec; float* cfrc; };
 
-struct DConst { DModel M; Lay L; DHField H; DWpre W; DReport R; };
+#define GREC_STRIDE 16
+struct DRecords { int o_geom; };
+struct DConst { DModel M; Lay L; DHField H; DWpre W; DReport R; DRecords X; };
 
 enum { PH_STEP1 = 1, PH_INV = 2, PH_STEP2 = 4, PH_NOINT = 8, PH_FKONLY = 16, PH_MULM = 32, PH_RESET = 64,
        PH_PRE = 128, PH_POST = 256 };
diff --git a/mujoco_sim_amd/csrc/engine.hip b/mujoco_sim_amd/csrc/engine.hip
--- a/mujoco_sim_amd/csrc/engine.hip
+++ b/mujoco_sim_amd/csrc/engine.hip
@@ -65,6 +65,7 @@
   Lay L{};
   int lds_bytes = 0, lds_bytes_pre = 0;
   DHField H{};
+  DRecords X{};
   bool report = false; DReport R{};
   int2* csel_tab = nullptr; int2* csel_host = nullptr; int csel_cap = 0; hipEvent_t csel_up = nullptr; std::vector<int> csel_have; float* csel_io = nullptr; size_t csel_io_words = 0;
   DWpre W{};
@@ -236,7 +237,7 @@
   return 1;
 }
 
-struct HostPack { DModel M{}; Lay L{}; DHField H{}; DWpre W{}; bool report = false; std::vector<int> I; std::vector<float> F; int o_controlled = 0, o_odom = 0, lds_bytes = 0, lds_bytes_pre = 0, lds_bytes_wpre = 0; long long gstride = 0; };
+struct HostPack { DModel M{}; Lay L{}; DHField H{}; DWpre W{}; DRecords X{}; bool report = false; std::vector<int> I; std::vector<float> F; int o_controlled = 0, o_odom = 0, lds_bytes = 0, lds_bytes_pre = 0, lds_bytes_wpre = 0; long long gstride = 0; };
 #define MJH_WINDOW_MAXCON 128
 static int g_window_solver = getenv("MJH_WINDOW") ? (atoi(getenv("MJH_WINDOW")) != 0) : 1;
 extern "C" void mjh_set_window_solver(int on) { g_window_solver = on ? 1 : 0; }
@@ -331,6 +332,19 @@
       H.o_hfield_size = addF(m->hfield_size, 4 * (size_t)m->nhfield); H.o_hfield_data = addF(m->hfield_data, (size_t)m->nhfielddata);
     }
   }
+  {
+    while (F.size() % GREC_STRIDE) F.push_back(0);
+    hp.X.o_geom = (int)F.size();
+    auto asf = [](int v) { float f; std::memcpy(&f, &v, sizeof f); return f; };
+    for (int g = 0; g < ng; g++) {
+      const int b = m->geom_bodyid[g], t = m->body_treeid[b];
+      F.push_back(asf(b)); F.push_back(asf(t)); F.push_back(asf(t >= 0 ? (m->tree_dofadr[t] | (m->tree_dofnum[t] << 16)) : 0xffff)); F.push_back(asf(m->geom_condim[g]));
+      F.push_back((float)m->geom_friction[3*g]); F.push_back((float)m->geom_friction[3*g+1]); F.push_back((float)m->geom_solmix[g]);
+      F.push_back((float)m->geom_solref[2*g]); F.push_back((float)m->geom_solref[2*g+1]);
+      for (int q = 0; q < 5; q++) F.push_back((float)m->geom_solimp[5*g+q]);
+      F.push_back((float)m->geom_margin[g]); F.push_back((float)m->geom_gap[g]);
+    }
+  }
   M.group_max = m->ntree <= 64 ? 16 : 4;
   for (int t = 0; t < m->ntree; t++) if (m->tree_dofnum[t] > 8) M.group_max = 4;
 #undef PI
@@ -539,7 +553,7 @@
   e->model = m; e->nenv = nenv; e->device = device; e->stream = (hipStream_t)stream;
 
   HostPack hp; derive_fitting(m, hp);
-  e->M = hp.M; e->L = hp.L; e->H = hp.H; e->W = hp.W; e->report = hp.report; e->lds_bytes = hp.lds_bytes; e->lds_bytes_pre = hp.lds_bytes_wpre; e->o_controlled = hp.o_controlled; e->o_odom = hp.o_odom;
+  e->M = hp.M; e->L = hp.L; e->H = hp.H; e->W = hp.W; e->X = hp.X; e->report = hp.report; e->lds_bytes = hp.lds_bytes; e->lds_bytes_pre = hp.lds_bytes_wpre; e->o_controlled = hp.o_controlled; e->o_odom = hp.o_odom;
   DModel& M = e->M; std::vector<int>& I = hp.I; std::vector<float>& F = hp.F;
   e->hI = I;
   if (dev_alloc(e, &e->dI, I.size(), false) || dev_alloc(e, &e->dF, F.size(), false)) { mjh_destroy(e); return MJH_ERR_NO_DEVICE; }
@@ -554,7 +568,7 @@
     if (dev_alloc(e, &R.ncon, (size_t)nenv) || dev_alloc(e, &R.rec, (size_t)nenv * R.maxcon * CREP_STRIDE) || dev_alloc(e, &R.cfrc, (size_t)nenv * 6 * e->M.nbody)) { mjh_destroy(e); return MJH_ERR_NO_DEVICE; }
   }
   {
-    DConst hc; hc.M = e->M; hc.L = e->L; hc.H = e->H; hc.W = e->W; hc.R = e->R;
+    DConst hc; hc.M = e->M; hc.L = e->L; hc.H = e->H; hc.W = e->W; hc.R = e->R; hc.X = e->X;
     if (dev_alloc(e, &e->dC, 1, false)) { mjh_destroy(e); return MJH_ERR_NO_DEVICE; }
     HIPCHK(hipMemcpyAsync(e->dC, &hc, sizeof hc, hipMemcpyHostToDevice, e->stream));
     HIPCHK(hipStreamSynchronize(e->stream));
diff --git a/mujoco_sim_amd/csrc/step_kernel.h b/mujoco_sim_amd/csrc/step_kernel.h
--- a/mujoco_sim_amd/csrc/step_kernel.h
+++ b/mujoco_sim_amd/csrc/step_kernel.h
@@ -39,21 +39,22 @@
   return s0 + y * (s1 - s0);
 }
 
-template <class T> struct Tab {
+template <class T, bool GLB = false> struct Tab {
   const T* base; int off;
-  DEV T operator[](int i) const { return base[off + i]; }
-  DEV const T* operator+(int k) const { return base + off + k; }
+  DEV T operator[](int i) const { if constexpr (GLB) return ((const MJH_GLOBAL_AS T*)base)[off + i]; else return base[off + i]; }
+  DEV const T* operator+(int k) const { if constexpr (GLB) return (const T*)((const MJH_GLOBAL_AS T*)base + off + k); else return base + off + k; }
 };
-template <bool LAZY, class T, int DModel::*OFF> struct XTab {
+template <bool LAZY, class T, int DModel::*OFF, bool GLB = false> struct XTab {
   const DModel* m; const T* base; int off;
   DEV explicit XTab(const DModel& M) : m(&M), base(nullptr), off(0) { if constexpr (!LAZY) { base = tb(); off = M.*OFF; } }
   DEV const T* tb() const { if constexpr (T(1.5) == T(1)) return (const T*)m->I; else return (const T*)m->F; }
+  DEV const MJH_GLOBAL_AS T* tg() const { return (const MJH_GLOBAL_AS T*)tb(); }
 #ifdef MJH_TAB_PROBE_L2
   DEV T operator[](int i) const { if constexpr (LAZY) return *(volatile const T*)(tb() + (m->*OFF + i)); else return base[off + i]; }
 #else
-  DEV T operator[](int i) const { if constexpr (LAZY) return tb()[m->*OFF + i]; else return base[off + i]; }
+  DEV T operator[](int i) const { if constexpr (LAZY && GLB) return tg()[m->*OFF + i]; else if constexpr (LAZY) return tb()[m->*OFF + i]; else return base[off + i]; }
 #endif
-  DEV const T* operator+(int k) const { if constexpr (LAZY) return tb() + (m->*OFF + k); else return base + off + k; }
+  DEV const T* operator+(int k) const { if constexpr (LAZY && GLB) return (const T*)(tg() + (m->*OFF + k)); else if constexpr (LAZY) return tb() + (m->*OFF + k); else return base + off + k; }
 };
 
 template <bool LAZY, int Lay::*OFF> struct XArr {
@@ -858,10 +859,16 @@
 #ifndef MJH_LAZY_TABLES
 #define MJH_LAZY_TABLES (WPRE != 0 || (!DIAGM && NROW <= 4 && EXTRA))
 #endif
-#define IT(n) const XTab<MJH_LAZY_TABLES, int, &DModel::o_##n> n(M);
+#ifndef MJH_GLOBAL_TABLES
+#define MJH_GLOBAL_TABLES MJH_LAZY_TABLES
+#endif
+#define MTI(i) (MJH_GLOBAL_TABLES ? ((const MJH_GLOBAL_AS int*)M.I)[i] : M.I[i])
+#define MTF(i) (MJH_GLOBAL_TABLES ? ((const MJH_GLOBAL_AS float*)M.F)[i] : M.F[i])
+#define MTFP(a, b) (MJH_GLOBAL_TABLES ? (const float*)((const MJH_GLOBAL_AS float*)M.F + (a) + (b)) : M.F + (a) + (b))
+#define IT(n) const XTab<MJH_LAZY_TABLES, int, &DModel::o_##n, MJH_GLOBAL_TABLES> n(M);
   MJH_INT_TABLES(IT)
 #undef IT
-#define FT(n) const XTab<MJH_LAZY_TABLES, float, &DModel::o_##n> n(M);
+#define FT(n) const XTab<MJH_LAZY_TABLES, float, &DModel::o_##n, MJH_GLOBAL_TABLES> n(M);
   MJH_FLT_TABLES(FT)
 #undef FT
   float* const gs = NROW == 8 ? S.gscratch + (size_t)env * (size_t)S.gstride : nullptr;
@@ -872,6 +879,11 @@
 #define MJH_COLLIDE_LANES 1
 #endif
   constexpr bool COLLIDE_LANES = MJH_COLLIDE_LANES != 0 && WPRE != 0;
+#ifndef MJH_GEOM_RECORDS
+#define MJH_GEOM_RECORDS 1
+#endif
+  constexpr bool RECORDS = MJH_GEOM_RECORDS != 0 && WPRE != 0;
+  const auto grec = [&](int g) __attribute__((always_inline)) { return (const MJH_GLOBAL_AS mjh_f4*)((const MJH_GLOBAL_AS float*)M.F + C->X.o_geom) + (GREC_STRIDE / 4) * g; };
   constexpr bool REPORT = EXTRA && !DIAGM && WPRE == 0;
 #define LA(n) const XArr<MJH_LAZY_LDS, &Lay::n> s_##n(lds, L);
   MJH_LDS_SMALL(LA)
@@ -996,8 +1008,8 @@
           s_qpos[qa+3] = xquat[0]; s_qpos[qa+4] = xquat[1]; s_qpos[qa+5] = xquat[2]; s_qpos[qa+6] = xquat[3];
           s_xanchor[3*ja] = xpos[0]; s_xanchor[3*ja+1] = xpos[1]; s_xanchor[3*ja+2] = xpos[2];
           s_xaxis[3*ja] = 0; s_xaxis[3*ja+1] = 0; s_xaxis[3*ja+2] = 1;
-        } else if (EXTRA && M.nmocap > 0 && M.I[M.o_body_mocapid + b] >= 0) {
-          const float* mp = S.mocap + ((size_t)env * M.nmocap + M.I[M.o_body_mocapid + b]) * 7;
+        } else if (EXTRA && M.nmocap > 0 && MTI(M.o_body_mocapid + b) >= 0) {
+          const float* mp = S.mocap + ((size_t)env * M.nmocap + MTI(M.o_body_mocapid + b)) * 7;
           xpos[0] = mp[0]; xpos[1] = mp[1]; xpos[2] = mp[2]; xquat[0] = mp[3]; xquat[1] = mp[4]; xquat[2] = mp[5]; xquat[3] = mp[6];
         } else {
           const int p = body_parentid[b];
@@ -1056,10 +1068,10 @@
     }
     if (EXTRA && M.nsite > 0) {
       for (int si = lane; si < M.nsite; si += 64) {
-        const int b = M.I[M.o_site_bodyid + si];
+        const int b = MTI(M.o_site_bodyid + si);
         float t[3], q[4], mat[9];
-        rotvec(t, s_xmat + 9*b, M.F + M.o_site_pos + 3*si);
-        mulquat(q, s_xquat + 4*b, M.F + M.o_site_quat + 4*si); quat2mat(mat, q);
+        rotvec(t, s_xmat + 9*b, MTFP(M.o_site_pos, 3*si));
+        mulquat(q, s_xquat + 4*b, MTFP(M.o_site_quat, 4*si)); quat2mat(mat, q);
 #pragma unroll
         for (int k = 0; k < 3; k++) s_site[12*si+k] = s_xpos[3*b+k] + t[k];
 #pragma unroll
@@ -1182,19 +1194,19 @@
     if (!post && !(M.disableflags & (MJH_DSBL_CONTACT | MJH_DSBL_CONSTRAINT))) {
       int conbase = 0;
       auto hfield_pair = [&](const auto ipu) __attribute__((always_inline)) {
-        const Tab<int> geom_dataid{M.I, M.o_geom_dataid}, mesh_vertadr{M.I, M.o_mesh_vertadr}, mesh_vertnum{M.I, M.o_mesh_vertnum};
+        const Tab<int, MJH_GLOBAL_TABLES> geom_dataid{M.I, M.o_geom_dataid}, mesh_vertadr{M.I, M.o_mesh_vertadr}, mesh_vertnum{M.I, M.o_mesh_vertnum};
         const DHField& H = C->H;
         const int g1 = pair_geom1[ipu], g2 = pair_geom2[ipu], t2 = geom_type[g2];
         float* const stp = s_stage + pair_stageadr[ipu] * RAW_STRIDE;
         const int hid = geom_dataid[g1];
-        const int hnr = M.I[H.o_hfield_nrow + hid], hnc = M.I[H.o_hfield_ncol + hid];
-        const float* const hdat = M.F + H.o_hfield_data + M.I[H.o_hfield_adr + hid];
-        const float hsx = M.F[H.o_hfield_size + 4*hid], hsy = M.F[H.o_hfield_size + 4*hid + 1], hsz = M.F[H.o_hfield_size + 4*hid + 2], hsb = M.F[H.o_hfield_size + 4*hid + 3];
+        const int hnr = MTI(H.o_hfield_nrow + hid), hnc = MTI(H.o_hfield_ncol + hid);
+        const float* const hdat = MTFP(H.o_hfield_data, MTI(H.o_hfield_adr + hid));
+        const float hsx = MTF(H.o_hfield_size + 4*hid), hsy = MTF(H.o_hfield_size + 4*hid + 1), hsz = MTF(H.o_hfield_size + 4*hid + 2), hsb = MTF(H.o_hfield_size + 4*hid + 3);
         const float hmargin = fmaxf(geom_margin[g1], geom_margin[g2]);
         CvxGeom P1, P2;
         P1.type = MJH_GEOM_HFIELD; P1.vert = nullptr; P1.nvert = 0; P1.pad = P2.pad = 0;
         P2.type = t2; P2.vert = nullptr; P2.nvert = 0;
-        if (t2 == MJH_GEOM_MESH) { const int id = geom_dataid[g2]; P2.vert = M.F + M.o_mesh_vert + 3 * mesh_vertadr[id]; P2.nvert = mesh_vertnum[id]; }
+        if (t2 == MJH_GEOM_MESH) { const int id = geom_dataid[g2]; P2.vert = Tab<float, MJH_GLOBAL_TABLES>{M.F, M.o_mesh_vert} + 3 * mesh_vertadr[id]; P2.nvert = mesh_vertnum[id]; }
         float lp[3];
 #pragma unroll
         for (int k = 0; k < 9; k++) { P1.mat[k] = s_gmat[9*g1+k]; P2.mat[k] = s_gmat[9*g2+k]; }
@@ -1227,7 +1239,7 @@
 #pragma unroll
           for (int q = 0; q < RAW_STRIDE; q++) rbuf[q] = 0;
           bool got = false;
-          if (wave_any(act)) got = c_convex_wave<true>(P1, P2, hmargin, rbuf, act, lane, &hp) != 0 && act;
+          if (wave_any(act)) got = c_convex_wave<true, MJH_GLOBAL_TABLES>(P1, P2, hmargin, rbuf, act, lane, &hp) != 0 && act;
           const unsigned long long gm = __ballot(got);
           const int idx = cnt + __popcll(gm & ((1ull << lane) - 1ull));
           if (got && idx < MJH_HFIELD_MAXCON) {
@@ -1274,13 +1286,13 @@
             else if (t1 == MJH_GEOM_SPHERE && t2 == MJH_GEOM_BOX) n = c_sphere_box(p1, z1[0], p2, m2, z2, margin, st);
             else if (t1 == MJH_GEOM_PLANE && t2 == MJH_GEOM_ELLIPSOID) n = c_plane_ellipsoid(p1, m1, p2, m2, z2, margin, st);
             else if (EXTRA && t2 == MJH_GEOM_MESH && t1 == MJH_GEOM_PLANE) {
-              const Tab<int> geom_dataid{M.I, M.o_geom_dataid}, mesh_vertadr{M.I, M.o_mesh_vertadr}, mesh_vertnum{M.I, M.o_mesh_vertnum};
-              const Tab<float> mesh_vert{M.F, M.o_mesh_vert};
+              const Tab<int, MJH_GLOBAL_TABLES> geom_dataid{M.I, M.o_geom_dataid}, mesh_vertadr{M.I, M.o_mesh_vertadr}, mesh_vertnum{M.I, M.o_mesh_vertnum};
+              const Tab<float, MJH_GLOBAL_TABLES> mesh_vert{M.F, M.o_mesh_vert};
               const int id = geom_dataid[g2];
               n = c_plane_mesh(p1, m1, p2, m2, mesh_vert + 3 * mesh_vertadr[id], mesh_vertnum[id], margin, st);
             } else if (EXTRA && pair_is_convex(t1, t2)) {
-              const Tab<int> geom_dataid{M.I, M.o_geom_dataid}, mesh_vertadr{M.I, M.o_mesh_vertadr}, mesh_vertnum{M.I, M.o_mesh_vertnum};
-              const Tab<float> mesh_vert{M.F, M.o_mesh_vert};
+              const Tab<int, MJH_GLOBAL_TABLES> geom_dataid{M.I, M.o_geom_dataid}, mesh_vertadr{M.I, M.o_mesh_vertadr}, mesh_vertnum{M.I, M.o_mesh_vertnum};
+              const Tab<float, MJH_GLOBAL_TABLES> mesh_vert{M.F, M.o_mesh_vert};
               cvx = true;
               G1.type = t1; G2.type = t2; G1.vert = G2.vert = nullptr; G1.nvert = G2.nvert = 0;
               if (t1 == MJH_GEOM_MESH) { const int id = geom_dataid[g1]; G1.vert = mesh_vert + 3 * mesh_vertadr[id]; G1.nvert = mesh_vertnum[id]; }
@@ -1292,7 +1304,7 @@
             } else if (HF && t1 == MJH_GEOM_HFIELD) hf = true;
           }
         }
-        if constexpr (EXTRA) { if (wave_any(cvx)) { const int nc = c_convex_wave(G1, G2, margin, st, cvx, lane); if (cvx) n = nc; } }
+        if constexpr (EXTRA) { if (wave_any(cvx)) { const int nc = c_convex_wave<false, MJH_GLOBAL_TABLES>(G1, G2, margin, st, cvx, lane); if (cvx) n = nc; } }
         if constexpr (HF) {
           unsigned long long req = __ballot(hf);
           while (req) {
@@ -1411,7 +1423,7 @@
       const int w4 = rowW >> 2;
       if (!(M.disableflags & MJH_DSBL_EQUALITY))
         for (int e = 0; e < M.neq; e++) if (eq_active[e]) {
-          const int et = (EXTRA && M.has_weld) ? M.I[M.o_eq_type + e] : MJH_EQ_JOINT;
+          const int et = (EXTRA && M.has_weld) ? MTI(M.o_eq_type + e) : MJH_EQ_JOINT;
           const int nr = et == MJH_EQ_WELD ? 6 : (et == MJH_EQ_CONNECT ? 3 : 1);
           if (lane < nr) put_block(nblk + lane, BK_SINGLE, 1, 1, 0, (nblk + lane) * w4, et == MJH_EQ_JOINT ? e : (e | (lane << 16)), et == MJH_EQ_JOINT ? RT_EQ : RT_WELD, 0);
           nblk += nr; nbrow += nr; nefc += nr;
@@ -1470,6 +1482,7 @@
       if (jb >= nb) continue;
       const int id = hd[1] & 0xffffff, rtype = (hd[1] >> 24) & 15, side = (hd[1] >> 28) & 1;
       int t1 = -1, t2 = -1;
+      int tw1 = -1, tw2 = 0;
       if (rtype == RT_EQ) {
         const int j1 = eq_obj1id[id], j2 = eq_obj2id[id];
         const float* dat = eq_data + 11*id;
@@ -1489,7 +1502,7 @@
       else if (EXTRA && rtype == RT_WELD) {
         const int e = id & 0xffff, r = id >> 16;
         const int b1 = eq_obj1id[e], b2 = eq_obj2id[e];
-        const bool weld = M.I[M.o_eq_type + e] == MJH_EQ_WELD;
+        const bool weld = MTI(M.o_eq_type + e) == MJH_EQ_WELD;
         const float* dat = eq_data + 11*e;
         t1 = body_treeid[b1]; t2 = body_treeid[b2];
         if (t1 < 0) { t1 = t2; t2 = -1; }
@@ -1524,13 +1537,21 @@
       else {
         const float* c = s_con + id * CON_STRIDE;
         const int g1 = CON_G1(c), g2 = CON_G2(c);
-        const int b1 = geom_bodyid[g1], b2 = geom_bodyid[g2];
-        t1 = body_treeid[b1]; t2 = body_treeid[b2];
+        int b1, b2; float fr10, fr11, fr20, fr21;
+        if constexpr (RECORDS) {
+          const MJH_GLOBAL_AS mjh_f4* r1 = grec(g1); const MJH_GLOBAL_AS mjh_f4* r2 = grec(g2);
+          const mjh_f4 h1 = r1[0], h2 = r2[0], p1 = r1[1], p2 = r2[1];
+          b1 = __float_as_int(h1.x); b2 = __float_as_int(h2.x); t1 = __float_as_int(h1.y); t2 = __float_as_int(h2.y);
+          tw1 = t1 < 0 ? __float_as_int(h2.z) : __float_as_int(h1.z); tw2 = __float_as_int(h2.z);
+          fr10 = p1.x; fr11 = p1.y; fr20 = p2.x; fr21 = p2.y;
+        } else { b1 = geom_bodyid[g1]; b2 = geom_bodyid[g2]; t1 = body_treeid[b1]; t2 = body_treeid[b2]; }
         const int t1raw = t1, t2raw = t2;
         if (t1 < 0) { t1 = t2; t2 = -1; }
         if (t2 == t1) t2 = -1;
         const float* dir = c + 4 + 3 * (jb < 3 ? jb : 0);
-        const float musc = jb == 0 ? 1.0f : (jb < 3 ? fmaxf(geom_friction[3*g1], geom_friction[3*g2]) : fmaxf(geom_friction[3*g1+1], geom_friction[3*g2+1]));
+        float musc;
+        if constexpr (RECORDS) musc = jb == 0 ? 1.0f : (jb < 3 ? fmaxf(fr10, fr20) : fmaxf(fr11, fr21));
+        else musc = jb == 0 ? 1.0f : (jb < 3 ? fmaxf(geom_friction[3*g1], geom_friction[3*g2]) : fmaxf(geom_friction[3*g1+1], geom_friction[3*g2+1]));
 #pragma unroll
         for (int sd = 0; sd < 2; sd++) {
           const int bd = sd ? b2 : b1; const float ss = (sd ? 1.0f : -1.0f) * musc;
@@ -1565,6 +1586,7 @@
       }
       if (jb == 0) {
         if (EXTRA && t1 < 0) { hd[2] = 0xffff; hd[3] = 0xffff; }
+        else if (RECORDS && tw1 >= 0) { hd[2] = tw1; hd[3] = t2 >= 0 ? tw2 : 0xffff; }
         else { hd[2] = tree_dofadr[t1] | (tree_dofnum[t1] << 16); hd[3] = t2 >= 0 ? (tree_dofadr[t2] | (tree_dofnum[t2] << 16)) : 0xffff; }
       }
     }
@@ -1604,7 +1626,7 @@
       } else if (EXTRA && rtype == RT_WELD) {
         const int e = id & 0xffff, r = id >> 16;
         const int b1 = eq_obj1id[e], b2 = eq_obj2id[e];
-        const bool weld = M.I[M.o_eq_type + e] == MJH_EQ_WELD;
+        const bool weld = MTI(M.o_eq_type + e) == MJH_EQ_WELD;
         const float* dat = eq_data + 11*e;
         if (r < 3) {
           float p1[3], p2[3];
@@ -1623,8 +1645,24 @@
       } else {
         const float* c = s_con + id * CON_STRIDE;
         const int g1 = CON_G1(c), g2 = CON_G2(c), dim = CON_DIM(c);
+        pos = c[0]; margin = c[CON_MARGIN];
+        if constexpr (RECORDS) {
+          const MJH_GLOBAL_AS mjh_f4* r1 = grec(g1); const MJH_GLOBAL_AS mjh_f4* r2 = grec(g2);
+          const mjh_f4 h1 = r1[0], h2 = r2[0], p1 = r1[1], p2 = r2[1], q1 = r1[2], q2 = r2[2], u1 = r1[3], u2 = r2[3];
+          const int b1 = __float_as_int(h1.x), b2 = __float_as_int(h2.x);
+          const float sr1[2] = {p1.w, q1.x}, sr2[2] = {p2.w, q2.x}, si1[5] = {q1.y, q1.z, q1.w, u1.x, u1.y}, si2[5] = {q2.y, q2.z, q2.w, u2.x, u2.y};
+          const float f0 = fmaxf(p1.x, p2.x), f1 = fmaxf(p1.y, p2.y);
+          mu1 = f0; mu3 = f1;
+          const float tran = p_binv(2*b1) + p_binv(2*b2);
+          if (dim == 1) diagA = tran;
+          else { diagA = tran + f0*f0*tran; const float mu0 = f0 * rsqrtf(M.impratio); rscale = 2 * mu0 * mu0; }
+          const float a = p1.z, bq = p2.z;
+          const float mix = (a >= MJ_MINVAL && bq >= MJ_MINVAL) ? a / (a + bq) : ((a < MJ_MINVAL && bq < MJ_MINVAL) ? 0.5f : (a < MJ_MINVAL ? 0.0f : 1.0f));
+          sr[0] = mix*sr1[0] + (1-mix)*sr2[0]; sr[1] = mix*sr1[1] + (1-mix)*sr2[1];
+#pragma unroll
+          for (int q = 0; q < 5; q++) si[q] = mix*si1[q] + (1-mix)*si2[q];
+        } else {
         const int b1 = geom_bodyid[g1], b2 = geom_bodyid[g2];
-        pos = c[0]; margin = c[CON_MARGIN];
         const float f0 = fmaxf(geom_friction[3*g1], geom_friction[3*g2]), f1 = fmaxf(geom_friction[3*g1+1], geom_friction[3*g2+1]);
         mu1 = f0; mu3 = f1;
         const float tran = p_binv(2*b1) + p_binv(2*b2);
@@ -1635,6 +1673,7 @@
         sr[0] = mix*geom_solref[2*g1] + (1-mix)*geom_solref[2*g2]; sr[1] = mix*geom_solref[2*g1+1] + (1-mix)*geom_solref[2*g2+1];
 #pragma unroll
         for (int q = 0; q < 5; q++) si[q] = mix*geom_solimp[5*g1+q] + (1-mix)*geom_solimp[5*g2+q];
+        }
       }
       const float imp = get_impedance(si, pos, margin);
       float R = fmaxf(MJ_MINVAL, (1 - imp) * diagA / imp);
@@ -2725,7 +2764,7 @@
                 const int e = id & 0xffff, r = id >> 16;
                 const int b1 = eq_obj1id[e], b2 = eq_obj2id[e];
                 if (b1 != b && b2 != b) continue;
-                const bool weld = M.I[M.o_eq_type + e] == MJH_EQ_WELD;
+                const bool weld = MTI(M.o_eq_type + e) == MJH_EQ_WELD;
                 const float* dat = eq_data + 11*e;
                 const float f = bf[BF_F];
                 const float z3[3] = {0, 0, 0};
@@ -2834,7 +2873,7 @@
           WSYNC();
         }
         for (int si = lane; si < M.nsensor; si += 64) {
-          const int site = M.I[M.o_sensor_objid + si], b = M.I[M.o_site_bodyid + site];
+          const int site = MTI(M.o_sensor_objid + si), b = MTI(M.o_site_bodyid + site);
           float F[6] = {0, 0, 0, 0, 0, 0};
           for (int c = b; c < b + body_subtreesize[b]; c++)
 #pragma unroll
@@ -2844,7 +2883,7 @@
           const float off[3] = {sp[0] - com[0], sp[1] - com[1], sp[2] - com[2]};
           float cr[3]; cross3(cr, off, F + 3);
           const float tq[3] = {F[0] - cr[0], F[1] - cr[1], F[2] - cr[2]};
-          const float* src = M.I[M.o_sensor_type + si] == MJH_SENS_FORCE ? F + 3 : tq;
+          const float* src = MTI(M.o_sensor_type + si) == MJH_SENS_FORCE ? F + 3 : tq;
           float* out = S.sensordata + ((size_t)env * M.nsensor + si) * 3;
 #pragma unroll
           for (int k = 0; k < 3; k++) out[k] = sp[3+k] * src[0] + sp[6+k] * src[1] + sp[9+k] * src[2];
```
